# lh3/bfc

Hardware: AMD Instinct MI355X
Metric: M k-mers/s counted (bloom+htab) on 150 bp reads (higher is better)
Workload: dtype u64

## Files before the change

### bfc_amd/_lib.py

```python
import ctypes as C
import os

HERE = os.path.dirname(os.path.abspath(__file__))
SO = os.environ.get("BFC_GPU_LIB") or os.path.join(HERE, "libbfc_gpu.so")

u64p = C.POINTER(C.c_uint64)
u32p = C.POINTER(C.c_uint32)
f32p = C.POINTER(C.c_float)


class BfcOpt(C.Structure):
    _fields_ = [("chunk_size", C.c_int), ("n_threads", C.c_int), ("no_mt_io", C.c_int), ("q", C.c_int), ("k", C.c_int),
                ("filter_mode", C.c_int), ("refine_ec", C.c_int), ("no_qual", C.c_int), ("min_frac", C.c_float),
                ("l_pre", C.c_int), ("bf_shift", C.c_int), ("n_hashes", C.c_int), ("discard", C.c_int),
                ("max_end_ext", C.c_int), ("win_multi_ec", C.c_int), ("min_cov", C.c_int),
                ("w_ec", C.c_int), ("w_ec_high", C.c_int), ("w_absent", C.c_int), ("w_absent_high", C.c_int),
                ("max_path_diff", C.c_int), ("max_heap", C.c_int)]


class BfcBf(C.Structure):
    _fields_ = [("n_shift", C.c_int), ("n_hashes", C.c_int), ("b", C.POINTER(C.c_uint8))]


class BfcKmer(C.Structure):
# ... 5 lines not shown
                ("filter_mode", C.c_int), ("device", C.c_int), ("max_batch_pos", C.c_uint64),
                ("region_shift", C.c_int), ("tab_cshift", C.c_int), ("debug_seen", C.c_int), ("track_order", C.c_int), ("rank", C.c_int), ("n_ranks", C.c_int), ("table_layout", C.c_int)]


SYMBOLS = {
    "bfc_bf_init": (C.POINTER(BfcBf), [C.c_int, C.c_int]),
    "bfc_bf_destroy": (None, [C.POINTER(BfcBf)]),
    "bfc_bf_insert": (C.c_int, [C.POINTER(BfcBf), C.c_uint64]),
    "bfc_bf_get": (C.c_int, [C.POINTER(BfcBf), C.c_uint64]),
    "bfc_ch_init": (C.c_void_p, [C.c_int, C.c_int]),
    "bfc_ch_destroy": (None, [C.c_void_p]),
    "bfc_ch_insert": (C.c_int, [C.c_void_p, u64p, C.c_int, C.c_int]),
    "bfc_ch_get": (C.c_int, [C.c_void_p, u64p]),
    "bfc_ch_count": (C.c_uint64, [C.c_void_p]),
    "bfc_ch_hist": (C.c_int, [C.c_void_p, u64p, u64p]),
    "bfc_ch_dump": (C.c_int, [C.c_void_p, C.c_char_p]),
    "bfc_ch_restore": (C.c_void_p, [C.c_char_p]),
    "bfc_ch_get_k": (C.c_int, [C.c_void_p]),
    "bfc_ch_kmer_occ": (C.c_int, [C.c_void_p, C.POINTER(BfcKmer)]),
    "bfc_count": (C.c_void_p, [C.c_char_p, C.POINTER(BfcOpt)]),
    "bfc_correct": (None, [C.c_char_p, C.POINTER(BfcOpt), C.c_void_p]),
    "bfcg_params_default": (None, [C.POINTER(BfcgParams)]),
    "bfcg_create": (C.c_void_p, [C.POINTER(BfcgParams)]),
    "bfcg_destroy": (None, [C.c_void_p]),
    "bfcg_last_error": (C.c_char_p, []),
    "bfcg_build_id": (C.c_char_p, []),
    "bfcg_device_count": (C.c_int, []),
    "bfcg_reset": (C.c_int, [C.c_void_p]),
    "bfcg_count_batch_dev": (C.c_int, [C.c_void_p, C.c_void_p, C.c_void_p, C.c_uint64]),
    "bfcg_count_batch_host": (C.c_int, [C.c_void_p, C.c_void_p, C.c_void_p, C.c_uint64]),
    "bfcg_plane_words": (C.c_uint64, [C.c_uint64]),
    "bfcg_pack_planes": (None, [C.c_void_p, C.c_void_p, C.c_uint64, C.c_uint64, C.c_uint64, C.c_int, C.c_void_p, C.c_uint64]),
    "bfcg_count_batch_planes": (C.c_int, [C.c_void_p, C.c_void_p, C.c_uint64, C.c_uint64, C.c_uint64, C.c_int]),
    "bfcg_sync": (C.c_int, [C.c_void_p]),
    "bfcg_mg_info": (C.c_int, [C.c_void_p, C.POINTER(C.c_int)]),
    "bfcg_batch_limit": (C.c_uint64, [C.c_void_p]),
    "bfcg_mg_scatter": (C.c_int, [C.c_void_p, C.c_void_p, C.c_void_p, C.c_uint64, C.c_void_p, u32p]),
    "bfcg_mg_process": (C.c_int, [C.c_void_p, C.c_void_p, u32p]),
    "bfcg_mg_allow_onepass": (None, [C.c_void_p, C.c_int]),
    "bfcg_group_unique_id": (C.c_int, [C.c_void_p]),
    "bfcg_group_create": (C.c_void_p, [C.POINTER(BfcgParams), C.c_int, C.c_int, C.c_int, C.POINTER(C.c_int), C.c_void_p, C.c_int]),
    "bfcg_group_destroy": (None, [C.c_void_p]),
    "bfcg_group_info": (C.c_int, [C.c_void_p, C.POINTER(C.c_int)]),
    "bfcg_group_slab_mode": (C.c_int, [C.c_void_p]),
    "bfcg_group_lazy_batches": (C.c_uint64, [C.c_void_p]),
    "bfcg_group_exchange_bytes": (C.c_int, [C.c_void_p, u64p]),
    "bfcg_group_ctx": (C.c_void_p, [C.c_void_p, C.c_int]),
    "bfcg_group_reset": (C.c_int, [C.c_void_p]),
    "bfcg_group_count_batch_dev": (C.c_int, [C.c_void_p, C.POINTER(C.c_void_p), C.POINTER(C.c_void_p), u64p]),
    "bfcg_group_count_batch_host": (C.c_int, [C.c_void_p, C.c_void_p, C.c_void_p, C.c_uint64]),
    "bfcg_group_sync": (C.c_int, [C.c_void_p]),
    "bfcg_group_stats": (C.c_int, [C.c_void_p, u64p]),
    "bfcg_group_progress": (C.c_int, [C.c_void_p, u64p, u64p, u64p, C.c_int]),
    "bfcg_group_export_table": (C.c_void_p, [C.c_void_p]),
    "bfcg_group_export_bloom": (C.POINTER(BfcBf), [C.c_void_p, C.c_int]),
    "bfcg_group_export_bloom_resident": (C.POINTER(BfcBf), [C.c_void_p, C.c_int]),
    "bfcg_trim_create": (C.c_void_p, [C.c_int, C.POINTER(BfcBf), C.c_int, C.c_uint64, C.c_uint64]),
    "bfcg_trim_destroy": (None, [C.c_void_p]),
    "bfcg_trim_batch": (C.c_int, [C.c_void_p, C.c_void_p, C.c_void_p, C.c_uint64, u64p, C.c_uint64, C.c_float, C.POINTER(C.c_int32), C.POINTER(C.c_int32)]),
    "bfcg_trim_last_ms": (C.c_float, [C.c_void_p]),
    "bfcg_trim_adopted": (C.c_int, [C.c_void_p]),
    "bfcg_trim_dev_seq": (C.c_void_p, [C.c_void_p]),
    "bfcg_stream_batches": (C.c_uint64, [C.c_void_p]),
    "bfc_ch_union": (C.c_void_p, [C.POINTER(C.c_void_p), C.c_int]),
    "bfc_ingest_digest": (C.c_int, [C.c_char_p, C.c_uint64, C.c_uint64, C.c_int, u64p]),
    "bfc_ingest_planes_digest": (C.c_int, [C.c_char_p, C.c_uint64, C.c_uint64, C.c_int, C.c_int, C.c_int, u64p]),
    "bfc_pgz_digest": (C.c_int, [C.c_char_p, C.c_int, C.c_uint64, C.c_uint64, u64p]),
    "bfcg_kcov_create": (C.c_void_p, [C.c_void_p, C.c_int, C.c_uint64]),
    "bfcg_kcov_attach": (C.c_void_p, [C.c_void_p, C.c_uint64]),
    "bfcg_kcov_destroy": (None, [C.c_void_p]),
    "bfcg_kcov_batch": (C.c_int, [C.c_void_p, C.c_void_p, C.c_void_p, C.c_uint64, C.c_int, C.c_void_p]),
    "bfcg_kcov_last_ms": (C.c_float, [C.c_void_p]),
    "bfcg_kcov_dev_seq": (C.c_void_p, [C.c_void_p]),
    "bfcg_kcov_dev_out": (C.c_void_p, [C.c_void_p]),
    "bfcg_dev_alloc": (C.c_void_p, [C.c_void_p, C.c_uint64]),
    "bfcg_dev_free": (None, [C.c_void_p, C.c_void_p]),
    "bfcg_h2d": (C.c_int, [C.c_void_p, C.c_void_p, C.c_void_p, C.c_uint64]),
    "bfcg_d2h": (C.c_int, [C.c_void_p, C.c_void_p, C.c_void_p, C.c_uint64]),
    "bfcg_host_alloc": (C.c_void_p, [C.c_uint64]),
    "bfcg_host_free": (None, [C.c_void_p]),
    "bfcg_stats": (C.c_int, [C.c_void_p, u64p]),
    "bfcg_progress": (C.c_int, [C.c_void_p, u64p, u64p, u64p, C.c_int]),
    "bfcg_partition_info": (C.c_int, [C.c_void_p, u64p]),
    "bfcg_s1wc_launches": (C.c_uint64, []),
    "bfcg_table_info": (C.c_int, [C.c_void_p, C.POINTER(C.c_int)]),
    "bfcg_last_batch_ms": (C.c_int, [C.c_void_p, f32p]),
    "bfcg_stage_ms": (C.c_int, [C.c_void_p, C.POINTER(C.c_double), u64p, C.c_int]),
    "bfcg_bloom_to_host": (C.c_int, [C.c_void_p, C.c_int, C.c_void_p]),
    "bfcg_export_bloom": (C.POINTER(BfcBf), [C.c_void_p, C.c_int]),
    "bfcg_export_bloom_resident": (C.POINTER(BfcBf), [C.c_void_p, C.c_int]),
    "bfcg_resident_drop": (None, [C.c_void_p]),
    "bfcg_export_table": (C.c_void_p, [C.c_void_p]),
    "bfcg_export_table_resident": (C.c_void_p, [C.c_void_p]),
    "bfc_ch_get_lpre": (C.c_int, [C.c_void_p]),
    "bfc_ch_export_sorted": (C.c_uint64, [C.c_void_p, u32p, u64p]),
    "bfcg_ec_create": (C.c_void_p, [C.c_void_p, C.POINTER(BfcOpt), C.c_int, C.c_uint64, C.c_uint64]),
    "bfcg_ec_attach": (C.c_void_p, [C.c_void_p, C.POINTER(BfcOpt), C.c_uint64, C.c_uint64]),
    "bfcg_ec_batch": (C.c_int, [C.c_void_p, C.c_void_p, C.c_void_p, C.c_uint64, u64p, C.c_uint64, u32p, u32p]),
    "bfcg_ec_destroy": (None, [C.c_void_p]),
    "bfcg_ec_last_ms": (C.c_float, [C.c_void_p]),
    "bfcg_ec_host_reads": (C.c_uint64, [C.c_void_p]),
    "bfcg_ec_last_lookups": (C.c_uint64, [C.c_void_p]),
    "bfcg_ec_retry_reads": (C.c_uint64, [C.c_void_p]),
    "bfcg_ec_adopted": (C.c_int, [C.c_void_p]),
    "bfcg_ec1_host": (C.c_int, [C.c_void_p, C.POINTER(BfcOpt), C.c_int, C.c_void_p, C.c_void_p, u32p, u32p]),
    "bfcg_ec_batch_refine": (C.c_int, [C.c_void_p, C.c_void_p, C.c_void_p, C.c_uint64, u64p, C.c_uint64, u32p, u32p, u32p, u32p]),
    "bfcg_ec1_host_refine": (C.c_int, [C.c_void_p, C.POINTER(BfcOpt), C.c_int, C.c_void_p, C.c_void_p, C.c_uint32, C.c_uint32, u32p, u32p]),
    "bfcg_ec_parse_stats": (C.c_int, [C.c_char_p, u32p, u32p]),
    "bfcg_kmers_create": (C.c_void_p, [C.c_void_p, C.c_int]),
    "bfcg_kmers_attach": (C.c_void_p, [C.c_void_p]),
    "bfcg_kmers_destroy": (None, [C.c_void_p]),
    "bfcg_kmers_info": (C.c_int, [C.c_void_p, C.POINTER(C.c_int)]),
    "bfcg_kmers_hist": (C.c_int, [C.c_void_p, u64p, u64p]),
    "bfcg_kmers_sub_sizes": (C.c_int, [C.c_void_p, u32p]),
    "bfcg_kmers_hist_sizes": (C.c_int, [C.c_void_p, u64p, u64p, u32p]),
    "bfcg_kmers_list": (C.c_int, [C.c_void_p, C.c_int, C.c_int, C.c_uint32, C.c_uint32, C.c_void_p, C.c_void_p, C.c_uint64, u64p]),
    "bfcg_kmers_last_ms": (C.c_float, [C.c_void_p]),
    "bfcg_kmer_decode_host": (C.c_int, [C.c_int, C.c_int, C.c_uint32, C.c_uint64, u64p]),
    "bfcg_kmer_2str": (None, [C.c_int, u64p, C.c_char_p]),
    "bfcg_kmers_format": (C.c_uint64, [C.c_int, C.c_void_p, C.c_void_p, C.c_uint64, C.c_void_p]),
    "bfcg_kmers_format_sizes": (C.c_uint64, [C.c_void_p, C.c_uint64, C.c_void_p]),
    "bfcg_kmers_lookup": (C.c_int, [C.c_void_p, C.c_void_p, C.c_uint64, C.c_void_p, u64p]),
    "bfcg_kmers_profile": (C.c_int, [C.c_void_p, C.c_void_p, C.c_void_p, C.c_uint64, C.c_void_p]),
    "bfcg_kmer_from_str": (C.c_int, [C.c_int, C.c_char_p, u64p]),
    "bfcg_kmer_occ_host": (C.c_int, [C.c_void_p, u64p]),
    "bfcg_kmers_occ_host": (None, [C.c_void_p, C.c_void_p, C.c_uint64, C.c_void_p]),
    "bfcg_kmers_parse": (C.c_uint64, [C.c_int, C.c_char_p, C.c_uint64, C.c_void_p, C.c_uint64, u64p]),
    "bfcg_lookup_format": (C.c_uint64, [C.c_char_p, C.c_uint64, C.c_void_p, C.c_uint64, C.c_void_p]),
    "bfcg_profile_format": (C.c_uint64, [C.c_void_p, C.c_uint64, C.c_void_p]),
    "bfcg_kmers_read_stats": (C.c_int, [C.c_void_p, C.c_void_p, C.c_void_p, C.c_uint64, C.c_void_p, C.c_uint64, C.c_int, C.c_void_p]),
    "bfcg_read_stats_host": (C.c_int, [C.c_void_p, C.c_void_p, C.c_uint64, C.c_void_p, C.c_uint64, C.c_int, C.c_void_p]),
    "bfcg_read_stats_format": (C.c_uint64, [C.c_void_p, C.c_uint64, C.c_void_p]),
    "bfcg_kmers_joint_hist": (C.c_int, [C.c_void_p, C.c_void_p, u64p, u64p]),
    "bfcg_kmers_list_vs": (C.c_int, [C.c_void_p, C.c_void_p, C.c_int, C.c_int, C.c_int, C.c_int, C.c_uint32, C.c_uint32, C.c_void_p, C.c_void_p, C.c_void_p, C.c_uint64, u64p]),
    "bfcg_kmers_union": (C.c_void_p, [C.c_void_p, C.c_void_p]),
    "bfcg_kmers_export": (C.c_void_p, [C.c_void_p, u64p]),
    "bfcg_kmers_format_vs": (C.c_uint64, [C.c_int, C.c_void_p, C.c_void_p, C.c_void_p, C.c_uint64, C.c_void_p]),
    "bfcg_kmers_neighbors": (C.c_int, [C.c_void_p, C.c_void_p, C.c_uint64, C.c_void_p]),
    "bfcg_kmers_graph_census": (C.c_int, [C.c_void_p, C.c_int, u64p]),
    "bfcg_kmers_list_graph": (C.c_int, [C.c_void_p, C.c_int, C.c_uint32, C.c_uint32, C.c_uint32, C.c_void_p, C.c_void_p, C.c_void_p, C.c_uint64, u64p]),
    "bfcg_kmers_extend": (C.c_int, [C.c_void_p, C.c_void_p, C.c_uint64, C.c_int, C.c_int, C.c_void_p, C.c_void_p]),
    "bfcg_kmer_revcomp": (C.c_int, [C.c_int, u64p, u64p]),
    "bfcg_neighbors_host": (C.c_int, [C.c_void_p, C.c_void_p, C.c_uint64, C.c_void_p]),
    "bfcg_graph_census_host": (C.c_int, [C.c_void_p, C.c_int, u64p]),
    "bfcg_graph_nb_host": (C.c_int64, [C.c_void_p, C.c_int, C.c_void_p, C.c_void_p]),
    "bfcg_extend_host": (C.c_int, [C.c_void_p, C.c_void_p, C.c_uint64, C.c_int, C.c_int, C.c_void_p, C.c_void_p]),
    "bfcg_kmers_unitigs": (C.c_int, [C.c_void_p, C.c_int, C.c_void_p, C.c_uint64, C.c_void_p, C.c_void_p, C.c_void_p, C.c_void_p, C.c_uint64, u64p]),
    "bfcg_unitigs_host": (C.c_int, [C.c_void_p, C.c_int, C.c_void_p, C.c_uint64, C.c_void_p, C.c_void_p, C.c_void_p, C.c_void_p, C.c_uint64, u64p]),
    "bfcg_kmers_clip": (C.c_void_p, [C.c_void_p, C.c_int, C.c_int, C.c_int, C.c_int, C.c_int, C.c_void_p, C.POINTER(C.c_int)]),
    "bfcg_clip_host": (C.c_void_p, [C.c_void_p, C.c_int, C.c_int, C.c_int, C.c_int, C.c_int, C.c_void_p, C.POINTER(C.c_int)]),
    "bfcg_kmers_pop": (C.c_void_p, [C.c_void_p, C.c_int, C.c_int, C.c_int, C.c_int, C.c_int, C.c_void_p, C.POINTER(C.c_int)]),
    "bfcg_pop_host": (C.c_void_p, [C.c_void_p, C.c_int, C.c_int, C.c_int, C.c_int, C.c_int, C.c_void_p, C.POINTER(C.c_int)]),
    "bfcg_hash_positions": (C.c_int, [C.c_void_p, C.c_void_p, C.c_void_p, C.c_uint64, u64p]),
    "bfcg_seen_flags": (C.c_int, [C.c_void_p, C.c_void_p, C.c_uint64]),
}

HOST_SYMBOLS = {
    "bfc_ch_alloc_raw": (C.c_void_p, [C.c_int, C.c_int, C.c_int]),
    "bfc_ch_raw_slots": (u64p, [C.c_void_p]),
    "bfc_ch_raw_cshift": (C.c_int, [C.c_void_p]),
    "bfc_ch_raw_recount": (None, [C.c_void_p]),
}

_lib = None


# ... 25 lines not shown
```

### bfc_amd/api.py

```python
import ctypes as C
import math

import numpy as np

from . import _lib
from ._lib import BfcOpt, BfcgParams, BfcKmer, u64p, u32p, f32p

STAT_NAMES = {0: "n_kmers", 1: "n_high", 2: "n_seen", 3: "n_keys", 4: "tab_ovf", 5: "err_pool", 6: "slow_buckets", 7: "crowded_regions", 8: "tab_cshift", 9: "n_batches"}


class BfcGpuError(RuntimeError):
    pass


def bfc_opt_init():
    o = BfcOpt()
    o.chunk_size = 100000000
    o.n_threads = 1
    o.q = 20
    o.k = 33
    o.l_pre = 20
    o.bf_shift = 33
    o.n_hashes = 4
    o.min_frac = 0.9
# ... 354 lines not shown
        return self

    def _ck(self, rc):
        if rc != 0:
            raise BfcGpuError(self.L.bfcg_last_error().decode())

    def close(self):
        if self.ctx and not getattr(self, "_borrowed", False):
            self.L.bfcg_destroy(self.ctx)
        self.ctx = None

    def __del__(self):
        try:
            self.close()
        except Exception:
            pass

    def reset(self):
        self._ck(self.L.bfcg_reset(self.ctx))

    def count_host(self, seq_stream, qual_stream=None):
        seq_stream = np.ascontiguousarray(seq_stream, dtype=np.uint8)
        q = np.ascontiguousarray(qual_stream, dtype=np.uint8) if qual_stream is not None else None
        self._ck(self.L.bfcg_count_batch_host(self.ctx, seq_stream.ctypes.data, q.ctypes.data if q is not None else None, len(seq_stream)))

    def count_planes(self, planes, first_pos, n_pos, has_qual=True):
        planes = np.ascontiguousarray(planes, dtype=np.uint32)
        assert planes.ndim == 2 and planes.shape[0] == 4
        self._ck(self.L.bfcg_count_batch_planes(self.ctx, planes.ctypes.data, planes.shape[1], first_pos, n_pos, 1 if has_qual else 0))

    def count_dev(self, d_seq, d_qual, n_pos):
        self._ck(self.L.bfcg_count_batch_dev(self.ctx, d_seq, d_qual, n_pos))

    def mg_info(self):
        out = (C.c_int * 4)()
        self.L.bfcg_mg_info(self.ctx, out)
        return dict(nb1=out[0], nb_loc=out[1], rec_bytes=out[2], n_ranks=out[3])

    def batch_limit(self):
        return int(self.L.bfcg_batch_limit(self.ctx))

    def mg_scatter(self, d_seq, d_qual, n_pos, d_send):
        counts = np.zeros(self.mg_info()["nb1"], dtype=np.uint32)
        self._ck(self.L.bfcg_mg_scatter(self.ctx, d_seq, d_qual, n_pos, d_send, counts.ctypes.data_as(u32p)))
        return counts

    def mg_process(self, d_recv, seg_cnt):
        seg_cnt = np.ascontiguousarray(seg_cnt, dtype=np.uint32)
        self._ck(self.L.bfcg_mg_process(self.ctx, d_recv, seg_cnt.ctypes.data_as(u32p)))

    def dev_alloc(self, nbytes):
        p = self.L.bfcg_dev_alloc(self.ctx, nbytes)
        if not p:
            raise BfcGpuError(self.L.bfcg_last_error().decode())
        return p

    def dev_free(self, p):
        self.L.bfcg_dev_free(self.ctx, p)

    def h2d(self, dptr, arr):
        arr = np.ascontiguousarray(arr)
        self._ck(self.L.bfcg_h2d(self.ctx, dptr, arr.ctypes.data, arr.nbytes))

    def sync(self):
        self._ck(self.L.bfcg_sync(self.ctx))

    def stats(self):
        out = np.zeros(16, dtype=np.uint64)
        self._ck(self.L.bfcg_stats(self.ctx, out.ctypes.data_as(u64p)))
        d = {STAT_NAMES[i]: int(out[i]) for i in STAT_NAMES}
        d["stream_batches"] = int(self.L.bfcg_stream_batches(self.ctx))
        d["phase_cycles"] = [int(out[i]) for i in range(10, 16)]
        return d

    def table_info(self):
        out = (C.c_int * 4)()
        self.L.bfcg_table_info(self.ctx, out)
        return dict(segments=bool(out[0]), seg_shift=out[1], tab_cshift=out[2], seg_growths=out[3])

    def partition_info(self):
        out = (C.c_uint64 * 2)()
        self.L.bfcg_partition_info(self.ctx, out)
        return dict(one_pass=bool(out[0] & 1), level2_one_pass=bool(out[0] & 2), replayed_batches=int(out[1]))

    def s1wc_launches(self):
        return int(self.L.bfcg_s1wc_launches())

    def last_batch_ms(self):
        out = np.zeros(6, dtype=np.float32)
        self.L.bfcg_last_batch_ms(self.ctx, out.ctypes.data_as(f32p))
        return dict(hist1=float(out[0]), scatter1=float(out[1]), level2=float(out[2]), bloom=float(out[3]), commit=float(out[4]), total=float(out[5]))

    def stage_ms(self, reset=False):
        out = (C.c_double * 6)()
        n = C.c_uint64()
        self._ck(self.L.bfcg_stage_ms(self.ctx, out, C.byref(n), int(reset)))
        return dict(hist1=out[0], scatter1=out[1], level2=out[2], bloom=out[3], commit=out[4], total=out[5]), int(n.value)

    def bloom_bytes(self, which=0):
        out = np.empty((1 << (self.bf_shift - 3)) // self.n_ranks, dtype=np.uint8)
        self._ck(self.L.bfcg_bloom_to_host(self.ctx, which, out.ctypes.data))
        return out

    def export_bloom(self, which=0, resident=False):
        p = (self.L.bfcg_export_bloom_resident if resident else self.L.bfcg_export_bloom)(self.ctx, which)
        if not p:
            raise BfcGpuError(self.L.bfcg_last_error().decode())
        return HostBloom(p)

    def export_table(self):
        p = self.L.bfcg_export_table(self.ctx)
        if not p:
            raise BfcGpuError(self.L.bfcg_last_error().decode())
        return HostTable(p)

    def hash_positions(self, seq_stream, qual_stream=None):
        seq_stream = np.ascontiguousarray(seq_stream, dtype=np.uint8)
        q = np.ascontiguousarray(qual_stream, dtype=np.uint8) if qual_stream is not None else None
        out = np.zeros((len(seq_stream), 3), dtype=np.uint64)
        self._ck(self.L.bfcg_hash_positions(self.ctx, seq_stream.ctypes.data, q.ctypes.data if q is not None else None, len(seq_stream), out.ctypes.data_as(u64p)))
        return out

    def seen_flags(self, n_pos):
        out = np.zeros(n_pos, dtype=np.uint8)
        self._ck(self.L.bfcg_seen_flags(self.ctx, out.ctypes.data, n_pos))
        return out


class GpuGroup:

    def __init__(self, k, bf_shift, devices, max_batch_pos, n_ranks=None, first_rank=0, uid=None, transport=0, q=20, n_hashes=4, l_pre=20,
                 filter_mode=0, track_order=False, table_layout=0, region_shift=0, tab_cshift=0):
        self.L = _lib.load()
        p = BfcgParams()
        self.L.bfcg_params_default(C.byref(p))
        p.k, p.q, p.bf_shift, p.n_hashes, p.l_pre, p.filter_mode = k, q, bf_shift, n_hashes, l_pre, filter_mode
        p.max_batch_pos, p.region_shift, p.tab_cshift, p.track_order, p.table_layout = int(max_batch_pos), region_shift, tab_cshift, int(track_order), int(table_layout)
        self.params, self.k, self.bf_shift = p, k, bf_shift
        self.devices = list(devices)
        self.n_local = len(self.devices)
        self.n_ranks = n_ranks if n_ranks is not None else self.n_local
        dv = (C.c_int * self.n_local)(*self.devices)
        self._uid = (C.c_uint8 * 128).from_buffer_copy(bytes(uid)) if uid is not None else None
        self.g = self.L.bfcg_group_create(C.byref(p), self.n_ranks, first_rank, self.n_local, dv, self._uid, transport)
        if not self.g:
            raise BfcGpuError("bfcg_group_create failed: " + self.L.bfcg_last_error().decode())

    @staticmethod
    def unique_id():
        L = _lib.load()
        buf = (C.c_uint8 * 128)()
        if L.bfcg_group_unique_id(buf) != 0:
            raise BfcGpuError(L.bfcg_last_error().decode())
        return bytes(buf)

    def _ck(self, rc):
        if rc != 0:
            raise BfcGpuError(self.L.bfcg_last_error().decode())

    def close(self):
        if self.g:
            self.L.bfcg_group_destroy(self.g)
            self.g = None

    def __del__(self):
        try:
# ... 522 lines not shown
```

### bfc_amd/csrc/bfcg_bloom3.hip

```cpp
#include <hip/hip_runtime.h>
#include <stdint.h>
#include <stdlib.h>
#include "kmer_dev.h"
#include "bfcg_internal.h"
#include "bfcg_dev.h"

using namespace bfcg;

#define B3_UND 0x40000000u
#define B3_SEEN16 0x8000u
#define B3_COLD_NR 8
#define B3_WALK_U 4
template <int BT, int PF, bool COLD>
__global__ __launch_bounds__(BT, PF <= 2 ? 8 : 6) void k_bloom3(KParams P, BloomArgs A)
{
	extern __shared__ __attribute__((aligned(16))) unsigned char smem[];
	__shared__ uint32_t s_list_n, s_ovf, s_pool_off, s_emit_n, s_fs_used, s_wb_n, s_pad3[2];
	const uint32_t f = blockIdx.x;
	const bool ho_log = A.ho_stride != 0;
	if (batch_poisoned(A)) { if (ho_log && threadIdx.x == 0) A.ho_mark[f] = A.ho_cur[f]; return; }
	uint32_t rs, n;
	region_list(A, f, rs, n);
	if (n == 0) { if (threadIdx.x == 0) { if (ho_log) A.ho_mark[f] = A.ho_cur[f]; else if (A.agg_cnt) A.agg_cnt[f] = 0; } return; }
	uint32_t ho_cur0 = 0;
	unsigned long long *ho_base;
	if (ho_log) {
		ho_cur0 = A.ho_cur[f];
		if (ho_cur0 + n > A.ho_stride) {
			if (threadIdx.x == 0) { atomicAdd(&A.stats[(size_t)(f & (ST_SLOTS - 1)) * ST_N + ST_ERR_POOL], 1ULL); A.ho_mark[f] = ho_cur0; }
			return;
		}
		ho_base = A.ho + (uint64_t)f * A.ho_stride + ho_cur0;
	} else ho_base = reinterpret_cast<unsigned long long *>(A.stream_out) + rs;
	A.stats += (size_t)(f & (ST_SLOTS - 1)) * ST_N;
	const uint32_t region_dw = 16u << P.R;
	unsigned char *sp = smem;
	unsigned int *region = reinterpret_cast<unsigned int *>(sp); sp += (size_t)region_dw * 4;
	const uint32_t nblk = 1u << P.R;
	unsigned int *bcnt = reinterpret_cast<unsigned int *>(sp), *boff = bcnt + nblk;
	if (COLD) sp += (size_t)(2 * nblk + 4) * 4;
	unsigned int *fs = reinterpret_cast<unsigned int *>(sp); if (!COLD) sp += (size_t)P.fs_cap * 4;
	unsigned int *la = reinterpret_cast<unsigned int *>(sp); sp += (size_t)P.list_cap * 4;
	unsigned int *lb = reinterpret_cast<unsigned int *>(sp); sp += (size_t)P.list_cap * 4;
	unsigned short *lc = reinterpret_cast<unsigned short *>(sp); sp += (size_t)P.list_cap * 2;
	unsigned short *ord = reinterpret_cast<unsigned short *>(sp);
	const uint32_t fs_mask = P.fs_cap - 1;
	const uint32_t *recs = A.recs + (uint64_t)rs * 3;
	unsigned int *g_region = reinterpret_cast<unsigned int *>(A.bloom) + (uint64_t)f * region_dw;
	const uint32_t imp = (P.f_base + f) >> P.F2;
	const Dec3 D = dec3_geom(P);
	const int tid = threadIdx.x, lane = tid & 63;
	const uint32_t mask_a = (1u << D.a) - 1u, imp_sh = D.n ? imp << D.lo : 0u, sh_up = D.lo + D.n;
#ifdef BFCG_MEASURE
	const bool timing = BFCG_ABL(P, 64) && tid == 0;
	long long tq[7] = {0, 0, 0, 0, 0, 0, 0};
	long long tc[7] = {0, 0, 0, 0, 0, 0, 0};
	if (timing) tq[0] = clock64();
#define B3_TC(i) do { if (timing) tc[i] = clock64(); } while (0)
#else
#define B3_TC(i) do { } while (0)
#endif
	auto addr3 = [&](uint32_t d0, uint32_t d1) -> uint32_t {
		const uint32_t y0d = d0 & mask_a, upper = y0d >> D.up;
		const uint32_t y0lo = D.n ? (y0d & D.lowmask) | imp_sh | (upper << sh_up) : y0d;
		const uint32_t y1lo = __builtin_amdgcn_alignbit(d1, d0, D.a) & D.mk32;
		const uint32_t hh = upper | (((y0lo - y1lo) ^ y1lo) << D.sh_x);
		uint32_t h2 = (hh >> 9) & 511u;
		h2 |= (uint32_t)((h2 & 31u) == 0);
		return (y0d & D.rmask) | ((hh & 511u) << 8) | (h2 << 17);
	};
	auto entry3 = [&](uint32_t d0, uint32_t d1) -> unsigned long long {
		const unsigned long long AA = d0 | ((unsigned long long)d1 << 32);
		const unsigned long long y1 = (AA >> D.a) & ((1ULL << P.k) - 1);
		const uint32_t y0d = d0 & mask_a;
		const unsigned long long id = (unsigned long long)((y0d & D.rmask) | ((y0d >> D.up) << D.R)) | (y1 << D.sh_y1);
		return (id << 1) | (unsigned long long)((d1 >> D.sh_flag) & 1u);
	};
	RecW<3> cur[PF], nxt[PF];
#pragma unroll
	for (int u = 0; u < PF; ++u) {
		const uint32_t i = tid + u * BT;
		cur[u].d[0] = cur[u].d[1] = cur[u].d[2] = 0; nxt[u] = cur[u];
		if (i < n) cur[u] = rec_load<3>(recs + (uint64_t)i * 3);
		if (i + BT * PF < n) nxt[u] = rec_load<3>(recs + (uint64_t)(i + BT * PF) * 3);
	}
	{
		const uint4 *src = reinterpret_cast<const uint4 *>(g_region);
		uint4 *dst = reinterpret_cast<uint4 *>(region);
		for (uint32_t i = tid; i < region_dw / 4; i += BT) dst[i] = src[i];
		if constexpr (COLD) { for (uint32_t i = tid; i < 2 * nblk + 4; i += BT) bcnt[i] = 0; }
		else {
			uint4 *f4 = reinterpret_cast<uint4 *>(fs);
			for (uint32_t i = tid; i < P.fs_cap / 4; i += BT) f4[i] = make_uint4(FS32_EMPTY, FS32_EMPTY, FS32_EMPTY, FS32_EMPTY);
		}
		if (tid == 0) { s_list_n = 0; s_emit_n = 0; s_ovf = 0; s_fs_used = 0; s_wb_n = 0; }
	}
	__syncthreads();
#ifdef BFCG_MEASURE
	if (timing) tq[1] = clock64();
#endif
	volatile uint32_t *v_ovf = &s_ovf;

	for (uint32_t base = 0; base < n; base += BT * PF) {
		uint32_t pk[PF], um[PF];
#pragma unroll
		for (int u = 0; u < PF; ++u) {
			pk[u] = 0; um[u] = 0;
			if (base + u * BT + (uint32_t)(tid & ~63) < n) {
				pk[u] = addr3(cur[u].d[0], cur[u].d[1]);
				const B3Pos b = b3_positions((pk[u] >> 8) & 511u, pk[u] >> 17);
				const uint32_t bl64 = (pk[u] & 255u) << 6;
// ... 621 lines not shown
```

### bfc_amd/csrc/bfcg_ctx.hip

```cpp
#include <hip/hip_runtime.h>
#include <stdint.h>
#include <stdio.h>
#include <stdlib.h>
#include <string.h>
#include <stdarg.h>
#include <sys/mman.h>
#include <time.h>
#include <vector>
#include <thread>
#include "bfc_gpu.h"
#include "bfcg_internal.h"
#include "bfc_host.h"

using namespace bfcg;

static thread_local char g_err[512] = "";
enum { HO_MAX_PAGES = BFCG_HO_MAX_PAGES };
enum { OP_FLAG_WORDS = 12, OP_STICKY = 8 };
static double dbg_now(void) { struct timespec ts; clock_gettime(CLOCK_MONOTONIC, &ts); return ts.tv_sec + 1e-9 * ts.tv_nsec; }
static inline void set_seg_shift(KParams &P, int s, int blk_max) { P.seg_shift = s; P.seg_blk = s < blk_max ? s : blk_max; }
int bfcg::fail(const char *fmt, ...)
{
	va_list ap; va_start(ap, fmt); vsnprintf(g_err, sizeof(g_err), fmt, ap); va_end(ap);
	fprintf(stderr, "[E::bfcg] %s\n", g_err);
	return -1;
}

struct bfcg_ctx {
	bfcg_params_t prm;
	KParams P;
	BatchBufs B;
	hipStream_t st;
	hipStream_t stA;
	hipStream_t stC;
	hipEvent_t evt[2][7];
	hipEvent_t evA[2], evB[2], evCopy;
	uint32_t *rows1[2], *chunk1[2], *start1[2]; uint64_t *recs1[2];
	uint8_t *d_seq2[2], *d_qual2[2];
	uint32_t *d_planes[2];
	uint64_t plane_cap;
	int cur, pend;
	int used[2];
	uint8_t *d_seq, *d_qual;
	unsigned long long *h_stats;
	unsigned long long *h_snap[2];
	uint64_t call_no, slot_call[2];
	int call_depth;
	uint64_t final_call, call_keys[64];
	uint64_t n_batches;
	float last_ms[6];
	double sum_ms[6]; uint64_t n_timed;
	int rw;
	uint64_t bloom_bytes;
	int n_ranks, rank, log2n;
	uint32_t *d_seg, *h_seg;
	size_t seg_words;
	uint64_t recv_cap;
	uint64_t keys_last, grow[2];
	uint64_t crowded_last;
	int stream_mode;
	uint32_t *stream_out; uint64_t n_stream_batches;
	double seen_per_pos;
	int cold;
	uint64_t seen_last, pos_final, slot_pos[2];
	int pipeline;
	int seg_ok;
	int seg_total_max;
	int seg_blk_max;
	int b3_ok;
	uint32_t fs_cap_w, list_cap_w;
	uint32_t list_cap_cw;
	uint32_t list_cap_c;
	int seg_init_shift;
	int seg_escaped;
	uint64_t n_seg_grow;
	int onepass_ok, onepass;
	uint32_t *op_cursor[2], *op_seg[2], *op_flags, *h_flags[2];
	int unfinished, unfinished_mg;
	uint32_t *h_rows[2]; int rows_slot;
	uint32_t op_cap; uint64_t op_min_pos;
	uint32_t *cnt2; uint32_t cap2; uint64_t recs2_n;
	struct opq_t { const uint8_t *seq, *qual; uint64_t n_pos; int slot; const void *recv; int mg; } opq[4]; int n_opq;
	int mg_op2_ok, mg_op2, mg_op2_allowed; uint32_t *mg_seg[4];
	int mg_slab_ok; int mg_seg_slab[4];
	uint64_t n_replayed;
	int reused;
	int seg_no_grow;
	int seg_cap_shift;
	unsigned long long *ho, *ho_keys, *h_ho_keys[2]; uint32_t *ho_cur, *ho_mark; uint32_t ho_stride; int ho_K;
	int ho_pending;
	uint64_t ho_page_call[HO_MAX_PAGES];
	int slot_commit[2]; uint64_t slot_page_call[2][HO_MAX_PAGES];
	int slot_all_committed[2];
	uint64_t keys_known;
	int commit_absorbed;
	uint64_t keys_per_batch; int n_commits, ho_window;
	unsigned long long *seg_spare; int seg_spare_shift;
};

extern "C" const char *bfcg_last_error(void) { return g_err; }
extern "C" void bfcg_set_error(const char *msg) { fail("%s", msg); }

extern "C" int bfcg_device_count(void)
{
	int ndev = 0;
	if (hipGetDeviceCount(&ndev) != hipSuccess) { (void)hipGetLastError(); return 0; }
	return ndev;
}

extern "C" void bfcg_params_default(bfcg_params_t *p)
{
	memset(p, 0, sizeof(*p));
	p->k = 33; p->q = 20; p->bf_shift = 33; p->n_hashes = 4; p->l_pre = 20;
	p->max_batch_pos = 1ULL << 27;
}

static int clamp_lpre(int k, int l_pre)
{
	if (k * 2 - l_pre > BFC_CH_KEYBITS) l_pre = k * 2 - BFC_CH_KEYBITS;
	if (l_pre > BFC_CH_MAXPRE) l_pre = BFC_CH_MAXPRE;
	return l_pre;
}

extern "C" bfcg_ctx_t *bfcg_create(const bfcg_params_t *prm)
{
	int ndev = 0;
	const bool timing = getenv("BFC_GPU_TIMING") != 0;
	const double t_c0 = dbg_now();
	if (hipGetDeviceCount(&ndev) != hipSuccess || ndev == 0) { fail("no HIP device available: the counting path has no CPU fallback"); return NULL; }
	const double t_c1 = dbg_now();
	if (prm->device < 0 || prm->device >= ndev) { fail("device %d out of range (%d devices)", prm->device, ndev); return NULL; }
	if (prm->k < 1 || prm->k > 63) { fail("k=%d outside [1,63] (bfc.h:8, htab.c:23)", prm->k); return NULL; }
	if (prm->bf_shift < 9 + 0 || prm->bf_shift > 37) { fail("bf_shift=%d outside [9,37] (bbf.c:9, bfc.h:9)", prm->bf_shift); return NULL; }
	if (prm->n_hashes < 1 || prm->n_hashes > 12) { fail("n_hashes=%d outside [1,12]", prm->n_hashes); return NULL; }
	if (prm->max_batch_pos == 0 || prm->max_batch_pos >= (1ULL << 32)) { fail("max_batch_pos must be in [1, 2^32)"); return NULL; }
	const int n_ranks = prm->n_ranks > 0 ? prm->n_ranks : 1;
	int log2n = 0; while ((1 << log2n) < n_ranks) ++log2n;
	if ((1 << log2n) != n_ranks || n_ranks > 64 || prm->rank < 0 || prm->rank >= n_ranks) { fail("n_ranks=%d must be a power of two <= 64 and 0 <= rank=%d < n_ranks", n_ranks, prm->rank); return NULL; }
	if (n_ranks > 1 && prm->max_batch_pos >= (1ULL << (32 - log2n))) { fail("with %d ranks a batch holds < 2^%d positions", n_ranks, 32 - log2n); return NULL; }
	BFCG_CKN((void)0, hipSetDevice(prm->device));

	bfcg_ctx_t *c = (bfcg_ctx_t *)calloc(1, sizeof(bfcg_ctx_t));
	if (!c) { fail("out of host memory"); return NULL; }
	c->prm = *prm;
	KParams &P = c->P;
	P.k = prm->k; P.q = prm->q; P.bf_shift = prm->bf_shift; P.n_hashes = prm->n_hashes; P.filter_mode = prm->filter_mode;
	P.l_pre = clamp_lpre(prm->k, prm->l_pre);
	if (!prm->filter_mode && 2 * prm->k < P.l_pre) {
		fail("k=%d is too small for l_pre=%d: the count table needs 2k >= l_pre (htab.c:45-58)", prm->k, P.l_pre); bfcg_destroy(c); return NULL;
	}
	{
		const char *e;
		P.R = prm->region_shift > 0 ? prm->region_shift : ((e = getenv("BFCG_R")) ? atoi(e) : 8);
		if (P.R > 10) P.R = 10;
		if (P.R < 4) P.R = 4;
		if (P.R > P.bf_shift - 9) P.R = P.bf_shift - 9;
		while (P.bf_shift - 9 - P.R > 20 && P.R < 10) ++P.R;
		P.F = P.bf_shift - 9 - P.R;
		if (P.F <= 8) { P.F1 = P.F; P.F2 = 0; }
		else { P.F2 = (P.F + 1) / 2; if (P.F2 > 10) P.F2 = 10; P.F1 = P.F - P.F2; }
		if (P.F2 > 0 && (e = getenv("BFCG_F1"))) {
			const int f1 = atoi(e);
			if (f1 >= 1 && f1 <= 10 && P.F - f1 >= 1 && P.F - f1 <= 10 && f1 >= log2n) { P.F1 = f1; P.F2 = P.F - f1; }
		}
		if (P.F1 > 10) { fail("bf_shift=%d needs more than two scatter levels at region_shift=%d", P.bf_shift, P.R); bfcg_destroy(c); return NULL; }
		if (n_ranks > 1 && P.F2 == 0) {
			if (P.F <= log2n) { fail("bf_shift=%d gives %d bloom regions: too few for %d ranks", P.bf_shift, 1 << P.F, n_ranks); bfcg_destroy(c); return NULL; }
			P.F1 = (P.F + 1) / 2 > log2n ? (P.F + 1) / 2 : log2n; P.F2 = P.F - P.F1;
		}
#ifdef BFCG_MEASURE
		P.ablate = (e = getenv("BFCG_ABLATE")) ? atoi(e) : 0;
#else
		P.ablate = 0;
		if ((e = getenv("BFCG_ABLATE")) && atoi(e)) fprintf(stderr, "[W::bfcg] BFCG_ABLATE=%s ignored: this library was built without -DBFCG_MEASURE\n", e);
#endif
// ... 87 lines not shown
	c->recv_cap = n_ranks > 1 ? B.max_kmers + B.max_kmers / 4 + (1u << 20) : B.max_kmers;
	BFCG_CKN(bfcg_destroy(c), hipStreamCreate(&c->st)); BFCG_CKN(bfcg_destroy(c), hipStreamCreate(&c->stA)); BFCG_CKN(bfcg_destroy(c), hipStreamCreate(&c->stC));
	for (int b = 0; b < 2; ++b) {
		for (int i = 0; i < 7; ++i) BFCG_CKN(bfcg_destroy(c), hipEventCreate(&c->evt[b][i]));
		BFCG_CKN(bfcg_destroy(c), hipEventCreateWithFlags(&c->evA[b], hipEventDisableTiming)); BFCG_CKN(bfcg_destroy(c), hipEventCreateWithFlags(&c->evB[b], hipEventDisableTiming));
	}
	BFCG_CKN(bfcg_destroy(c), hipEventCreateWithFlags(&c->evCopy, hipEventDisableTiming));
	{
		const uint64_t tile = (uint64_t)bfcg_tile_of_rw(c->rw / 4), tile1 = (uint64_t)bfcg_tile1_of_rw(c->rw / 4);
		const uint64_t tiles1 = (prm->max_batch_pos + tile1 - 1) / tile1, chunks1 = (tiles1 + BFCG_SCAN_CH - 1) / BFCG_SCAN_CH;
		const uint64_t rows2 = (c->recv_cap + c->recv_cap / 8) / tile + (uint64_t)nb1 * 16 + 8;
		for (int b = 0; b < 2; ++b) {
			BFCG_CKN(bfcg_destroy(c), hipMalloc(&c->rows1[b], sizeof(uint32_t) * tiles1 * nb1));
			BFCG_CKN(bfcg_destroy(c), hipMalloc(&c->chunk1[b], sizeof(uint32_t) * chunks1 * nb1));
			BFCG_CKN(bfcg_destroy(c), hipMalloc(&c->start1[b], sizeof(uint32_t) * (nb1 + 1) * 2));
		}
		B.rows1 = c->rows1[0]; B.chunk1 = c->chunk1[0]; B.start1 = c->start1[0]; B.row_base = B.start1 + nb1 + 1;
		if (P.F2 > 0) {
			BFCG_CKN(bfcg_destroy(c), hipMalloc(&B.rows2, sizeof(uint32_t) * rows2 * (1u << P.F2)));
			BFCG_CKN(bfcg_destroy(c), hipMalloc(&B.start2, sizeof(uint32_t) * (nfine + 1)));
		}
	}
	{
		const char *e = getenv("BFCG_ONEPASS");
		c->onepass_ok = n_ranks == 1 && P.F2 > 0 && !(e && atoi(e) == 0);
		uint64_t cap = (B.max_kmers + B.max_kmers / 8) / ((uint64_t)nb1 * 8) + 1;
		while (cap * nb1 * 8 > 0xffffffffULL) --cap;
		if (cap >= 1024) cap &= ~31ULL;
		else if (cap >= 8) cap &= ~3ULL;
		c->op_cap = (uint32_t)cap;
		c->op_min_pos = (e = getenv("BFCG_ONEPASS_MIN_TILES")) ? (uint64_t)atoi(e) * 4096 : (uint64_t)nb1 * 8 * 1024;
	}
	const uint64_t recs1_n = c->onepass_ok ? (uint64_t)c->op_cap * nb1 * 8 + (uint64_t)bfcg_tile1_of_rw(c->rw / 4) + 64 : B.max_kmers;
	BFCG_CKN(bfcg_destroy(c), hipMalloc(&c->recs1[0], recs1_n * c->rw));
	if (n_ranks == 1 && !c->pipeline) c->recs1[1] = c->recs1[0];
	else BFCG_CKN(bfcg_destroy(c), hipMalloc(&c->recs1[1], recs1_n * c->rw));
	{
		const char *e = getenv("BFCG_ONEPASS");
		c->mg_op2_ok = P.F2 > 0 && !(e && atoi(e) == 0);
	}
	{ const char *e = getenv("BFCG_MG_SLABS"); c->mg_slab_ok = P.F2 > 0 && !(e && atoi(e) == 0); }
	if (c->onepass_ok || c->mg_slab_ok) {
		for (int b = 0; b < 2; ++b) {
			BFCG_CKN(bfcg_destroy(c), hipMalloc(&c->op_cursor[b], sizeof(uint32_t) * (8 * nb1 * 32 + 32)));
			BFCG_CKN(bfcg_destroy(c), hipMalloc(&c->op_seg[b], sizeof(uint32_t) * ((size_t)25 * nb1 + 8)));
		}
	}
	if (c->mg_slab_ok) for (int b = 0; b < 2; ++b) BFCG_CKN(bfcg_destroy(c), hipHostMalloc(&c->h_rows[b], sizeof(uint32_t) * ((size_t)8 * nb1 + 2 * (size_t)n_ranks)));
	if (c->onepass_ok || c->mg_op2_ok || c->mg_slab_ok) {
		for (int b = 0; b < 2; ++b) BFCG_CKN(bfcg_destroy(c), hipHostMalloc(&c->h_flags[b], 4 * sizeof(uint32_t)));
		BFCG_CKN(bfcg_destroy(c), hipMalloc(&c->op_flags, OP_FLAG_WORDS * sizeof(uint32_t)));
		BFCG_CKN(bfcg_destroy(c), hipMemset(c->op_flags, 0, OP_FLAG_WORDS * sizeof(uint32_t)));
	}
	if (c->mg_op2_ok) for (int i = 0; i < 4; ++i) c->mg_seg[i] = (uint32_t *)malloc(sizeof(uint32_t) * (size_t)n_ranks * (size_t)(nb1 >> log2n) * 8);
	B.recs1 = c->recs1[0];
	c->recs2_n = c->recv_cap;
	if (c->onepass_ok || c->mg_op2_ok || c->mg_slab_ok) {
		const char *e = getenv("BFCG_ONEPASS2");
		const uint64_t cap2 = (B.max_kmers + B.max_kmers / 8) / (uint64_t)nfine + 64, n2 = cap2 * (uint64_t)nfine + 8192;
		if (!(e && atoi(e) == 0) && n2 < 0xffffffffULL) {
			c->cap2 = (uint32_t)cap2; c->recs2_n = n2 > c->recv_cap ? n2 : c->recv_cap;
			BFCG_CKN(bfcg_destroy(c), hipMalloc(&c->cnt2, sizeof(uint32_t) * (size_t)nfine));
		} else { c->mg_op2_ok = 0; BFCG_CKN(bfcg_destroy(c), hipMalloc(&c->cnt2, sizeof(uint32_t) * (size_t)nfine)); }
		B.cnt_live = c->cnt2;
	}
	if (P.F2 > 0) BFCG_CKN(bfcg_destroy(c), hipMalloc(&B.recs2, c->recs2_n * c->rw));
	c->seg_words = (size_t)25 * nb1 + 8;
	{ BFCG_CKN(bfcg_destroy(c), hipMalloc(&c->d_seg, sizeof(uint32_t) * 2 * c->seg_words)); BFCG_CKN(bfcg_destroy(c), hipHostMalloc(&c->h_seg, sizeof(uint32_t) * 2 * c->seg_words)); }
	BFCG_CKN(bfcg_destroy(c), hipMalloc(&B.bloom, c->bloom_bytes));
	P.f_base = (uint32_t)c->rank * (uint32_t)nfine;
	if (c->seg_ok) {
		int sh = prm->tab_cshift > 0 ? prm->tab_cshift + 3 : 6;
		if (prm->tab_cshift <= 0) while (((uint64_t)nfine << sh) < prm->max_batch_pos / 4 && sh < BFCG_SEG_MAX_SHIFT) ++sh;
		if (sh > BFCG_SEG_MAX_SHIFT) sh = BFCG_SEG_MAX_SHIFT;
		c->seg_init_shift = sh;
		{ const char *e = getenv("BFCG_SEG_BLOCK"); c->seg_blk_max = e && atoi(e) >= 3 && atoi(e) <= BFCG_SEG_MAX_SHIFT ? atoi(e) : 12; }
		{ const char *e = getenv("BFCG_SEG_TOTAL"); c->seg_total_max = e && atoi(e) >= c->seg_blk_max && atoi(e) <= BFCG_SEG_TOTAL_MAX ? atoi(e) : BFCG_SEG_TOTAL_MAX; }
		if (c->seg_total_max > c->seg_blk_max + 15) c->seg_total_max = c->seg_blk_max + 15;
		P.seg = 1; set_seg_shift(P, sh, c->seg_blk_max); c->seg_cap_shift = sh;
		BFCG_CKN(bfcg_destroy(c), set_seg_lds_attr());
		BFCG_CKN(bfcg_destroy(c), hipMalloc(&B.seg_tab, ((uint64_t)nfine << sh) * 8));
		{
			const char *e = getenv("BFCG_COMMIT_K");
			int K = e ? atoi(e) : 4;
			if (K < 1) K = 1;
			if (K > HO_MAX_PAGES) K = HO_MAX_PAGES;
			if (!c->cap2) K = 1;
			size_t free_b = 0, total_b = 0;
			const uint64_t page = (uint64_t)nfine * (c->cap2 ? c->cap2 : 1) * 8;
			if (hipMemGetInfo(&free_b, &total_b) == hipSuccess) while (K > 1 && page * (uint64_t)K > (uint64_t)free_b / 3) --K;
			c->ho_K = K;
			c->ho_stride = c->cap2 ? (uint32_t)K * c->cap2 : 0u;
			uint64_t entries = (uint64_t)nfine * c->ho_stride;
			if (entries < c->recs2_n) entries = c->recs2_n;
			BFCG_CKN(bfcg_destroy(c), hipMalloc(&c->ho, (entries + 4096) * 8));
			BFCG_CKN(bfcg_destroy(c), hipMalloc(&c->ho_cur, sizeof(uint32_t) * (size_t)nfine));
			BFCG_CKN(bfcg_destroy(c), hipMalloc(&c->ho_mark, sizeof(uint32_t) * (size_t)nfine * HO_MAX_PAGES));
			BFCG_CKN(bfcg_destroy(c), hipMalloc(&c->ho_keys, sizeof(unsigned long long) * ST_SLOTS * HO_MAX_PAGES));
			for (int b = 0; b < 2; ++b) BFCG_CKN(bfcg_destroy(c), hipHostMalloc(&c->h_ho_keys[b], sizeof(unsigned long long) * ST_SLOTS * HO_MAX_PAGES));
		}
	}
	if (P.filter_mode) BFCG_CKN(bfcg_destroy(c), hipMalloc(&B.bloom_hi, c->bloom_bytes));
	else if (!c->seg_ok) BFCG_CKN(bfcg_destroy(c), hipMalloc(&B.table, 8ULL << (P.l_pre + P.tab_cshift)));
	if (P.track) { BFCG_CKN(bfcg_destroy(c), hipMalloc(&B.tab_first, 8ULL << (P.l_pre + P.tab_cshift))); BFCG_CKN(bfcg_destroy(c), hipMalloc(&B.sub_last, 8ULL << P.l_pre)); }
	BFCG_CKN(bfcg_destroy(c), hipMalloc(&B.stats, sizeof(unsigned long long) * ST_N * (ST_SLOTS + 1)));
	{ uint64_t cap = prm->max_batch_pos / 2; if (cap < (1u << 20)) cap = 1u << 20; if (cap > (1u << 28)) cap = 1u << 28; B.tab_ovf_cap = (uint32_t)cap; }
	BFCG_CKN(bfcg_destroy(c), hipMalloc(&B.tab_ovf, (uint64_t)B.tab_ovf_cap * 40));
	B.pool_slices = 256;
	{
		const uint64_t pool_words = (uint64_t)B.pool_slices + (uint64_t)B.pool_slices * ((uint64_t)1024 << P.R);
		BFCG_CKN(bfcg_destroy(c), hipMalloc(&B.pool, pool_words * 8));
		BFCG_CKN(bfcg_destroy(c), hipMemset(B.pool, 0, (size_t)B.pool_slices * 8));
	}
	if (prm->debug_seen) BFCG_CKN(bfcg_destroy(c), hipMalloc(&B.seen_out, prm->max_batch_pos));
	if (!P.filter_mode) {
		if (!c->seg_ok) BFCG_CKN(bfcg_destroy(c), hipMalloc(&B.agg_out, (uint64_t)nfine * P.ag_cap * (P.track ? 32 : 24)));
		BFCG_CKN(bfcg_destroy(c), hipMalloc(&B.agg_cnt, sizeof(uint32_t) * nfine));
	}
	for (int b = 0; b < 2; ++b) { BFCG_CKN(bfcg_destroy(c), hipMalloc(&c->d_seq2[b], prm->max_batch_pos)); BFCG_CKN(bfcg_destroy(c), hipMalloc(&c->d_qual2[b], prm->max_batch_pos + 64)); }
	c->d_seq = c->d_seq2[0]; c->d_qual = c->d_qual2[0];
	BFCG_CKN(bfcg_destroy(c), hipHostMalloc(&c->h_stats, sizeof(unsigned long long) * ST_N * (ST_SLOTS + 2)));
	for (int b = 0; b < 2; ++b) BFCG_CKN(bfcg_destroy(c), hipHostMalloc(&c->h_snap[b], sizeof(unsigned long long) * ST_N * (ST_SLOTS + 1)));
	const double t_c2 = dbg_now();
	BFCG_CKN(bfcg_destroy(c), set_bloom_lds_attr(P));
	BFCG_CKN(bfcg_destroy(c), set_scatter1wc_lds_attr());
	const double t_c3 = dbg_now();
	if (bfcg_reset(c) != 0) { bfcg_destroy(c); return NULL; }
	if (timing) fprintf(stderr, "[T::bfcg_create] HIP runtime up %.3f s, device buffers %.3f s, kernel attributes %.3f s, filter and table cleared %.3f s\n", t_c1 - t_c0, t_c2 - t_c1, t_c3 - t_c2, dbg_now() - t_c3);
	return c;
}

extern "C" void bfcg_destroy(bfcg_ctx_t *c)
{
	if (!c) return;
	(void)hipSetDevice(c->prm.device);
	(void)hipDeviceSynchronize();
	for (int b = 0; b < 2; ++b) { (void)hipFree(c->rows1[b]); (void)hipFree(c->chunk1[b]); (void)hipFree(c->start1[b]); if (b == 0 || c->recs1[1] != c->recs1[0]) (void)hipFree(c->recs1[b]); (void)hipFree(c->d_seq2[b]); (void)hipFree(c->d_qual2[b]); (void)hipFree(c->d_planes[b]); }
	(void)hipFree(c->B.rows2); (void)hipFree(c->B.start2); (void)hipFree(c->B.recs2);
	(void)hipFree(c->B.bloom); (void)hipFree(c->B.bloom_hi); (void)hipFree(c->B.table); (void)hipFree(c->B.stats); (void)hipFree(c->B.tab_first); (void)hipFree(c->B.sub_last);
	(void)hipFree(c->stream_out); (void)hipFree(c->B.seg_tab); (void)hipFree(c->seg_spare);
	(void)hipFree(c->ho); (void)hipFree(c->ho_cur); (void)hipFree(c->ho_mark); (void)hipFree(c->ho_keys);
	for (int b = 0; b < 2; ++b) if (c->h_ho_keys[b]) (void)hipHostFree(c->h_ho_keys[b]);
	for (int b = 0; b < 2; ++b) { (void)hipFree(c->op_cursor[b]); (void)hipFree(c->op_seg[b]); if (c->h_flags[b]) (void)hipHostFree(c->h_flags[b]); if (c->h_rows[b]) (void)hipHostFree(c->h_rows[b]); }
	(void)hipFree(c->op_flags); (void)hipFree(c->cnt2); for (int i = 0; i < 4; ++i) free(c->mg_seg[i]);
	(void)hipFree(c->B.tab_ovf); (void)hipFree(c->B.pool); (void)hipFree(c->B.seen_out); (void)hipFree(c->B.agg_out); (void)hipFree(c->B.agg_cnt);
	for (void *h : {(void *)c->h_stats, (void *)c->h_snap[0], (void *)c->h_snap[1]}) if (h) (void)hipHostFree(h); (void)hipFree(c->d_seg); if (c->h_seg) (void)hipHostFree(c->h_seg);
	for (int b = 0; b < 2; ++b) for (hipEvent_t e : {c->evt[b][0], c->evt[b][1], c->evt[b][2], c->evt[b][3], c->evt[b][4], c->evt[b][5], c->evt[b][6], c->evA[b], c->evB[b]}) if (e) (void)hipEventDestroy(e);
	if (c->evCopy) (void)hipEventDestroy(c->evCopy);
	for (hipStream_t st : {c->st, c->stA, c->stC}) if (st) (void)hipStreamDestroy(st);
	free(c);
}

static inline uint64_t nfine(const bfcg_ctx_t *c) { return ((uint64_t)1 << c->P.F) >> c->log2n; }
static int batch_fits(const bfcg_ctx_t *c, uint64_t n_pos)
{
	if (n_pos > c->prm.max_batch_pos) return fail("batch of %llu positions exceeds max_batch_pos=%llu", (unsigned long long)n_pos, (unsigned long long)c->prm.max_batch_pos);
	return 0;
}

static int drain(bfcg_ctx_t *c);
static int replay_poisoned(bfcg_ctx_t *c);
static int enqueue_batch(bfcg_ctx_t *c, const uint8_t *d_seq, const uint8_t *d_qual, uint64_t n_pos, int wait_copy, int no_kstats);
static int ensure_agg(bfcg_ctx_t *c);
static int same_block_offset(bfcg_ctx_t *c, int b, const uint8_t *d_seq, const uint8_t **d_qual, uint64_t n_pos, hipStream_t s);
static int commit_pending_pages(bfcg_ctx_t *c, int b);
static void absorb_pages(bfcg_ctx_t *c, int b);
static int handover_begin(bfcg_ctx_t *c, BatchBufs &Bt, int b, int slabs, uint64_t call);
static int handover_end(bfcg_ctx_t *c, const BatchBufs &Bt, int b);

static void warm_tables(const bfcg_ctx_t *c, KParams &Pt)
{
	Pt.b3_warm = 0; Pt.b3_cold = 0;
	if (Pt.b3 && c->cold && c->list_cap_c) { Pt.list_cap = c->list_cap_c; Pt.b3_cold = 1; Pt.dedupe = 0; }
	else if (Pt.b3 && !Pt.dedupe && !c->cold && c->list_cap_cw && c->list_cap_cw >= c->list_cap_w) { Pt.list_cap = c->list_cap_cw; Pt.b3_warm = 1; Pt.b3_cold = 1; }
	else if (Pt.b3 && !Pt.dedupe && !c->cold && c->list_cap_w) { Pt.fs_cap = c->fs_cap_w; Pt.list_cap = c->list_cap_w; Pt.b3_warm = 1; }
}
static int dedupe_hint(const bfcg_ctx_t *c) { return (c->n_batches == 0 || (c->cold && c->seen_per_pos < 0.15)) && !getenv("BFCG_NO_DEDUPE"); }

extern "C" int bfcg_reset(bfcg_ctx_t *c)
{
	const double t_dbg = dbg_now();
	struct dbg_guard { double t; ~dbg_guard() { if (getenv("BFCG_DEBUG")) fprintf(stderr, "[D::reset] %.3f ms\n", (dbg_now() - t) * 1e3); } } dg{t_dbg};
	BFCG_CK(hipSetDevice(c->prm.device));
	if (c->pend && drain(c) != 0) return -1;
	BFCG_CK(hipMemsetAsync(c->B.stats, 0, sizeof(unsigned long long) * ST_N * (ST_SLOTS + 1), c->st));
	if (c->op_flags) BFCG_CK(hipMemsetAsync(c->op_flags, 0, OP_FLAG_WORDS * sizeof(uint32_t), c->st));
	BFCG_CK(hipEventRecord(c->evCopy, c->st));
	BFCG_CK(hipStreamWaitEvent(c->stA, c->evCopy, 0));
	BFCG_CK(hipMemsetAsync(c->B.bloom, 0, c->bloom_bytes, c->st));
	if (c->B.bloom_hi) BFCG_CK(hipMemsetAsync(c->B.bloom_hi, 0, c->bloom_bytes, c->st));
	if (c->seg_ok) {
		const uint64_t nf = nfine(c);
		if (c->seg_escaped || !c->B.seg_tab) {
			BFCG_CK(hipStreamSynchronize(c->st));
			if (c->B.table) { BFCG_CK(hipFree(c->B.table)); c->B.table = 0; }
			if (c->B.seg_tab) { BFCG_CK(hipFree(c->B.seg_tab)); c->B.seg_tab = 0; }
			set_seg_shift(c->P, c->seg_init_shift, c->seg_blk_max); c->seg_cap_shift = c->seg_init_shift;
			BFCG_CK(hipMalloc(&c->B.seg_tab, (nf << c->P.seg_shift) * 8));
		} else {
			set_seg_shift(c->P, c->seg_init_shift, c->seg_blk_max);
			if (c->n_batches && c->seg_spare && c->seg_spare_shift < c->seg_cap_shift && ((nf << c->seg_cap_shift) * 8) <= (16ULL << 30)) {
				BFCG_CK(hipStreamSynchronize(c->st));
				BFCG_CK(hipFree(c->seg_spare)); c->seg_spare = 0;
				if (hipMalloc(&c->seg_spare, (nf << c->seg_cap_shift) * 8) != hipSuccess) { (void)hipGetLastError(); c->seg_spare = 0; }
				c->seg_spare_shift = c->seg_cap_shift;
			}
		}
		if (c->n_batches) c->reused = 1;
		c->P.seg = 1; c->P.b3 = c->b3_ok; c->seg_escaped = 0;
		BFCG_CK(hipMemsetAsync(c->ho_cur, 0, sizeof(uint32_t) * (size_t)nf, c->st));
		c->ho_pending = 0; c->slot_commit[0] = c->slot_commit[1] = 0; c->slot_all_committed[0] = c->slot_all_committed[1] = 0; c->keys_known = 0; c->commit_absorbed = 0;
		c->keys_per_batch = 0; c->n_commits = 0; c->ho_window = 1;
		BFCG_CK(hipMemsetAsync(c->B.seg_tab, 0, (nf << c->P.seg_shift) * 8, c->st));
	}
	if (c->B.table) BFCG_CK(hipMemsetAsync(c->B.table, 0, 8ULL << (c->P.l_pre + c->P.tab_cshift), c->st));
	if (c->B.tab_first) { BFCG_CK(hipMemsetAsync(c->B.tab_first, 0xff, 8ULL << (c->P.l_pre + c->P.tab_cshift), c->st)); BFCG_CK(hipMemsetAsync(c->B.sub_last, 0, 8ULL << c->P.l_pre, c->st)); }
	c->n_batches = 0;
	c->keys_last = 0; c->grow[0] = c->grow[1] = 0;
	c->crowded_last = 0; c->stream_mode = c->P.seg ? 1 : 0;
	c->cold = 1; c->seen_last = c->pos_final = 0; c->seg_no_grow = 0;
	c->onepass = c->onepass_ok; c->mg_op2 = c->mg_op2_ok; c->n_opq = 0;
	c->call_no = c->final_call = 0; c->call_depth = 0; memset(c->call_keys, 0, sizeof(c->call_keys));
	return 0;
}

static void fold_slots(bfcg_ctx_t *c, const unsigned long long *raw)
{
	for (int i = 0; i < ST_N; ++i) {
		unsigned long long s = 0;
		for (int j = 0; j < ST_SLOTS; ++j) s += raw[(size_t)j * ST_N + i];
		c->h_stats[i] = s;
	}
	c->h_stats[ST_TAB_OVF] = raw[(size_t)ST_SLOTS * ST_N];
}
static int fetch_stats(bfcg_ctx_t *c)
{
	unsigned long long *raw = c->h_stats + ST_N;
	BFCG_CK(hipMemcpyAsync(raw, c->B.stats, sizeof(unsigned long long) * ST_N * (ST_SLOTS + 1), hipMemcpyDeviceToHost, c->st));
	BFCG_CK(hipStreamSynchronize(c->st));
	fold_slots(c, raw);
	return 0;
}
static void fold_snapshot(bfcg_ctx_t *c, int b)
{
	fold_slots(c, c->h_snap[b]);
	absorb_pages(c, b);
	if (c->slot_all_committed[b]) {
		c->final_call = c->slot_call[b]; c->call_keys[c->slot_call[b] & 63] = c->h_stats[ST_KEYS];
		if (c->h_stats[ST_KEYS] > c->keys_known && c->h_stats[ST_KEYS] - c->keys_known > c->keys_per_batch) c->keys_per_batch = c->h_stats[ST_KEYS] - c->keys_known;
		c->keys_known = c->h_stats[ST_KEYS]; c->commit_absorbed = 1;
	}
	c->pos_final += c->slot_pos[b]; c->slot_pos[b] = 0;
}

static int table_maintain(bfcg_ctx_t *c);
static int seg_maintain(bfcg_ctx_t *c);
static int seg_target_shift(const bfcg_ctx_t *c);
static int seg_to_legacy(bfcg_ctx_t *c, int for_export = 0);
static void note_growth(bfcg_ctx_t *c);
static int finalise_previous(bfcg_ctx_t *c, int b);
static int table_target_cshift(const bfcg_ctx_t *c);
static int use_stream(bfcg_ctx_t *c);

static int batch_times(bfcg_ctx_t *c, int b)
{
	for (int i = 0; i < 3; ++i) BFCG_CK(hipEventSynchronize(c->evt[b][i]));
	for (int i = 0; i < 5; ++i) BFCG_CK(hipEventElapsedTime(&c->last_ms[i], c->evt[b][i == 2 ? 6 : i], c->evt[b][i + 1]));
	c->last_ms[5] = c->last_ms[0] + c->last_ms[1] + c->last_ms[2] + c->last_ms[3] + c->last_ms[4];
	for (int i = 0; i < 6; ++i) c->sum_ms[i] += c->last_ms[i];
	++c->n_timed;
	return 0;
}
static int check_health(bfcg_ctx_t *c)
{
	if (c->h_stats[ST_ERR_POOL]) return fail("first-setter pool exhausted in %llu bloom regions: batch too large for max_batch_pos", (unsigned long long)c->h_stats[ST_ERR_POOL]);
	if (c->P.seg) return seg_maintain(c);
	if (c->B.table) return table_maintain(c);
	return 0;
}
static int drain(bfcg_ctx_t *c)
{
	if (!c->pend) return 0;
	BFCG_CK(hipStreamSynchronize(c->stA));
	BFCG_CK(hipStreamSynchronize(c->st));
	BFCG_CK(hipGetLastError());
	c->pend = 0;
	if (batch_times(c, c->cur ^ 1) != 0) return -1;
	absorb_pages(c, c->cur); absorb_pages(c, c->cur ^ 1);
	if (c->n_opq) {
		uint32_t sticky = 0;
		BFCG_CK(hipMemcpy(&sticky, c->op_flags + OP_STICKY, sizeof(sticky), hipMemcpyDeviceToHost));
		if (sticky) return replay_poisoned(c);
		c->n_opq = 0;
	}
	if (c->P.seg && c->ho_pending) {
		if (commit_pending_pages(c, 0) != 0) return -1;
		BFCG_CK(hipStreamSynchronize(c->st));
		BFCG_CK(hipGetLastError());
		absorb_pages(c, 0);
	}
	if (fetch_stats(c) != 0) return -1;
	c->keys_known = c->h_stats[ST_KEYS]; c->commit_absorbed = 1;
	c->final_call = c->call_no; c->call_keys[c->call_no & 63] = c->h_stats[ST_KEYS];
	c->pos_final += c->slot_pos[0] + c->slot_pos[1]; c->slot_pos[0] = c->slot_pos[1] = 0;
	note_growth(c);
	return check_health(c);
}

extern "C" int bfcg_sync(bfcg_ctx_t *c) { return drain(c); }

static int replay_poisoned(bfcg_ctx_t *c)
{
	const int n = c->n_opq;
	bfcg_ctx::opq_t q[4];
	for (int i = 0; i < n; ++i) q[i] = c->opq[i];
	c->n_opq = 0; c->onepass = 0; c->mg_op2 = 0;
	if (getenv("BFCG_DEBUG")) {
		uint32_t fl[OP_FLAG_WORDS];
		BFCG_CK(hipMemcpy(fl, c->op_flags, sizeof(fl), hipMemcpyDeviceToHost));
		fprintf(stderr, "[D::replay] %d batches; flags (level-1 slab, -, region slab, -) of slot 0: %u %u %u %u, slot 1: %u %u %u %u, sticky %u\n", n, fl[0], fl[1], fl[2], fl[3], fl[4], fl[5], fl[6], fl[7], fl[OP_STICKY]);
	}
	BFCG_CK(hipMemset(c->op_flags, 0, OP_FLAG_WORDS * sizeof(uint32_t)));
	if (fetch_stats(c) != 0) return -1;
	c->n_batches -= (uint64_t)n;
	std::vector<uint32_t> seg;
	for (int i = 0; i < n; ++i) if (q[i].mg) --c->call_no;
	for (int i = 0; i < n; ++i) {
		if (q[i].mg) {
			const int slab = c->mg_seg_slab[q[i].mg - 1];
			const size_t w = (size_t)c->n_ranks * (size_t)((1 << c->P.F1) >> c->log2n) * (slab ? 8 : 1);
			seg.assign(c->mg_seg[q[i].mg - 1], c->mg_seg[q[i].mg - 1] + w);
			if (mg_process(c, q[i].recv, seg.data(), slab ? c->op_cap : 0u, 0, 0) != 0) return -1;
		} else if (enqueue_batch(c, q[i].seq, q[i].qual, q[i].n_pos, 0, 1) != 0) return -1;
		if (drain(c) != 0) return -1;
		++c->n_replayed;
	}
	return 0;
}

static uint64_t growth_forecast(const bfcg_ctx_t *c) { return c->grow[0] < c->grow[1] ? c->grow[0] : c->grow[1]; }
static void note_growth(bfcg_ctx_t *c)
{
	const uint64_t keys = c->h_stats[ST_KEYS];
	{
		const uint64_t ds = c->h_stats[ST_SEEN] - c->seen_last, np = c->pos_final;
		if (np) { c->cold = ds * 5 < np * 2; c->seen_per_pos = (double)ds / (double)np; }
		c->seen_last = c->h_stats[ST_SEEN]; c->pos_final = 0;
	}
	if (!c->P.seg || c->commit_absorbed) {
		c->grow[1] = c->grow[0]; c->grow[0] = keys > c->keys_last ? keys - c->keys_last : 0; c->keys_last = keys;
		c->commit_absorbed = 0;
	}
	const uint64_t crowded = c->h_stats[ST_CROWDED];
	if (!c->stream_mode && c->B.table && !c->P.track && c->P.n_hashes == 4 && c->P.bloom_bt == 512 && !getenv("BFCG_NO_STREAM") && (crowded - c->crowded_last) * 2 > nfine(c)) c->stream_mode = 1;
	c->crowded_last = crowded;
}
static int table_target_cshift(const bfcg_ctx_t *c)
{
	const KParams &P = c->P;
	const uint64_t need = c->h_stats[ST_KEYS] + c->h_stats[ST_TAB_OVF], g = growth_forecast(c);
	int t = P.tab_cshift;
	if ((need + g) * 2 > (1ULL << (P.l_pre + t)))
		while ((need + 2 * g) * 2 > (1ULL << (P.l_pre + t)) && P.l_pre + t < 36) ++t;
	if (c->h_stats[ST_TAB_OVF] && t == P.tab_cshift) ++t;
	if (t > P.tab_cshift) {
		size_t free_b = 0, total_b = 0;
		if (hipMemGetInfo(&free_b, &total_b) == hipSuccess) {
			const uint64_t margin = 2ULL << 30;
			while (t > P.tab_cshift && (8ULL << (P.l_pre + t)) + margin > (uint64_t)free_b) --t;
			if (t == P.tab_cshift && !c->h_stats[ST_TAB_OVF] && need * 5 <= (4ULL << (P.l_pre + t))) return t;
			if (t == P.tab_cshift) return t + 1;
		}
	}
	return t;
}

static int table_maintain(bfcg_ctx_t *c)
{
	KParams &P = c->P; BatchBufs &B = c->B;
	for (;;) {
		const uint64_t ovf = c->h_stats[ST_TAB_OVF];
		const int target = table_target_cshift(c);
		if (ovf == 0 && target == P.tab_cshift) return 0;
		if (ovf > B.tab_ovf_cap) return fail("count table overflow list exhausted (%llu parked k-mers)", (unsigned long long)ovf);
		if (P.l_pre + target > 36) return fail("count table cannot grow beyond 2^36 slots");
		{
			size_t free_b = 0, total_b = 0;
			if (hipMemGetInfo(&free_b, &total_b) == hipSuccess && (8ULL << (P.l_pre + target)) + (1ULL << 30) > (uint64_t)free_b)
				return fail("count table of %llu keys cannot grow to 2^%d slots: %.1f GiB of device memory free", (unsigned long long)c->h_stats[ST_KEYS], P.l_pre + target, free_b / 1073741824.0);
		}
		int old_cshift = P.tab_cshift;
		unsigned long long *nt = 0;
		P.tab_cshift = target;
		unsigned long long *nf = 0;
		BFCG_CK(hipMalloc(&nt, 8ULL << (P.l_pre + P.tab_cshift)));
		BFCG_CK(hipMemsetAsync(nt, 0, 8ULL << (P.l_pre + P.tab_cshift), c->st));
		if (B.tab_first) { BFCG_CK(hipMalloc(&nf, 8ULL << (P.l_pre + P.tab_cshift))); BFCG_CK(hipMemsetAsync(nf, 0xff, 8ULL << (P.l_pre + P.tab_cshift), c->st)); }
		run_table_rehash(P, B.table, old_cshift, nt, B.tab_first, nf, c->st);
		BFCG_CK(hipStreamSynchronize(c->st));
		BFCG_CK(hipFree(B.table));
		B.table = nt;
		if (B.tab_first) { BFCG_CK(hipFree(B.tab_first)); B.tab_first = nf; }
		if (ovf) {
			uint64_t *tmp = 0;
			BFCG_CK(hipMalloc(&tmp, ovf * 40));
			BFCG_CK(hipMemcpyAsync(tmp, B.tab_ovf, ovf * 40, hipMemcpyDeviceToDevice, c->st));
			BFCG_CK(hipMemsetAsync(&B.stats[(size_t)ST_SLOTS * ST_N], 0, 8, c->st));
			run_table_replay(P, B.table, tmp, ovf, B.stats, B.tab_ovf, B.tab_ovf_cap, B.tab_first, B.sub_last, c->st);
			if (fetch_stats(c) != 0) return -1;
			BFCG_CK(hipFree(tmp));
		} else c->h_stats[ST_TAB_OVF] = 0;
	}
}


static int seg_target_shift(const bfcg_ctx_t *c)
{
	const KParams &P = c->P;
	const uint64_t nf = nfine(c);
	const uint64_t need = c->h_stats[ST_KEYS] + c->h_stats[ST_TAB_OVF], g = c->ho_K > 1 ? c->keys_per_batch : c->grow[0] > c->grow[1] ? c->grow[0] : c->grow[1];
	int t = P.seg_shift;
	const double full = c->seg_no_grow ? 0.85 : 0.62;
	while ((double)(need + (c->seg_no_grow ? 0 : g)) > full * (double)(nf << t)) ++t;
	if (c->h_stats[ST_TAB_OVF] && t == P.seg_shift) ++t;
	if (t != P.seg_shift && getenv("BFCG_DEBUG")) fprintf(stderr, "[D::seg_target] shift %d -> %d: keys %llu parked %llu forecast %llu slots %llu\n", P.seg_shift, t,
		(unsigned long long)c->h_stats[ST_KEYS], (unsigned long long)c->h_stats[ST_TAB_OVF], (unsigned long long)g, (unsigned long long)(nf << P.seg_shift));
	return t;
}

static int seg_maintain(bfcg_ctx_t *c)
{
	KParams &P = c->P; BatchBufs &B = c->B;
	const uint64_t nf = nfine(c);
	const double t_dbg = dbg_now();
	struct dbg_guard { double t; int s0; const int *s1; ~dbg_guard() { if (getenv("BFCG_DEBUG") && *s1 != s0) fprintf(stderr, "[D::seg_maintain] shift %d -> %d: %.3f ms\n", s0, *s1, (dbg_now() - t) * 1e3); } } dg{t_dbg, P.seg_shift, &P.seg_shift};
	for (;;) {
		const uint64_t ovf = c->h_stats[ST_TAB_OVF];
		const int target = seg_target_shift(c);
		if (ovf == 0 && target == P.seg_shift) return 0;
		if (ovf > B.tab_ovf_cap) return fail("count table overflow list exhausted (%llu parked k-mers)", (unsigned long long)ovf);
		{
			size_t free_b = 0, total_b = 0;
			const bool no_room = hipMemGetInfo(&free_b, &total_b) == hipSuccess && ((nf << target) * 8) + (1ULL << 30) > (uint64_t)free_b + (c->seg_spare && c->seg_spare_shift >= target ? (nf << c->seg_spare_shift) * 8 : 0);
			if (no_room || target > c->seg_total_max) {
				if (ovf == 0 && (double)c->h_stats[ST_KEYS] < 0.85 * (double)(nf << P.seg_shift)) { c->seg_no_grow = 1; return 0; }
				if (target > c->seg_total_max) return seg_to_legacy(c);
				if (seg_to_legacy(c) == 0) return 0;
				return fail("count table of %llu keys cannot grow to 2^%d slots per region: %.1f GiB of device memory free", (unsigned long long)c->h_stats[ST_KEYS], target, free_b / 1073741824.0);
			}
		}
		const int old_shift = P.seg_shift, old_blk = P.seg_blk;
		unsigned long long *nt = 0;
		int nt_shift = target;
		set_seg_shift(P, target, c->seg_blk_max);
		if (c->seg_spare && c->seg_spare_shift >= target) { nt = c->seg_spare; nt_shift = c->seg_spare_shift; c->seg_spare = 0; }
		else {
			if (c->seg_spare) { BFCG_CK(hipFree(c->seg_spare)); c->seg_spare = 0; }
			BFCG_CK(hipMalloc(&nt, (nf << target) * 8));
		}
		run_seg_rehash(P, B.seg_tab, old_shift, old_blk, nt, (uint32_t)nf, c->st);
		BFCG_CK(hipStreamSynchronize(c->st));
		BFCG_CK(hipGetLastError());
		if (((nf << nt_shift) * 8) <= (16ULL << 30)) {
			if (c->seg_cap_shift < nt_shift && c->reused) { BFCG_CK(hipFree(B.seg_tab)); c->seg_spare = 0; if (hipMalloc(&c->seg_spare, (nf << nt_shift) * 8) != hipSuccess) { (void)hipGetLastError(); c->seg_spare = 0; } c->seg_spare_shift = nt_shift; }
			else { c->seg_spare = B.seg_tab; c->seg_spare_shift = c->seg_cap_shift; }
		} else BFCG_CK(hipFree(B.seg_tab));
		B.seg_tab = nt; c->seg_cap_shift = nt_shift;
		++c->n_seg_grow;
		if (ovf) {
			uint64_t *tmp = 0;
			BFCG_CK(hipMalloc(&tmp, ovf * 40));
			BFCG_CK(hipMemcpyAsync(tmp, B.tab_ovf, ovf * 40, hipMemcpyDeviceToDevice, c->st));
			BFCG_CK(hipMemsetAsync(&B.stats[(size_t)ST_SLOTS * ST_N], 0, 8, c->st));
			run_seg_replay(P, B.seg_tab, tmp, ovf, B.stats, B.tab_ovf, B.tab_ovf_cap, c->st);
			if (fetch_stats(c) != 0) return -1;
			BFCG_CK(hipFree(tmp));
		} else c->h_stats[ST_TAB_OVF] = 0;
	}
}

static int seg_to_legacy(bfcg_ctx_t *c, int for_export)
{
	KParams &P = c->P; BatchBufs &B = c->B;
	const uint64_t nf = nfine(c);
	const uint64_t keys = c->h_stats[ST_KEYS];
	if (c->seg_spare) { BFCG_CK(hipFree(c->seg_spare)); c->seg_spare = 0; }
	if (!for_export && !P.filter_mode && !B.agg_out) BFCG_CK(hipMalloc(&B.agg_out, nf * P.ag_cap * (P.track ? 32 : 24)));
	int cs = c->prm.tab_cshift > 0 ? c->prm.tab_cshift : 2;
	const uint64_t want = for_export ? keys + keys * 3 / 4 : 2 * keys + (c->prm.max_batch_pos / 4);
	while ((1ULL << (P.l_pre + cs)) < want && P.l_pre + cs < 36) ++cs;
	{
		size_t free_b = 0, total_b = 0;
		if (hipMemGetInfo(&free_b, &total_b) == hipSuccess)
			while (cs > 1 && (8ULL << (P.l_pre + cs)) + (2ULL << 30) > (uint64_t)free_b) --cs;
	}
	P.tab_cshift = cs;
	BFCG_CK(hipMalloc(&B.table, 8ULL << (P.l_pre + cs)));
	BFCG_CK(hipMemsetAsync(B.table, 0, 8ULL << (P.l_pre + cs), c->st));
	BFCG_CK(hipMemset2DAsync(B.stats + ST_KEYS, sizeof(unsigned long long) * ST_N, 0, sizeof(unsigned long long), ST_SLOTS, c->st));
	run_seg_to_table(P, B.seg_tab, (uint32_t)nf, B.table, B.stats, B.tab_ovf, B.tab_ovf_cap, c->st);
	BFCG_CK(hipStreamSynchronize(c->st));
	BFCG_CK(hipGetLastError());
	BFCG_CK(hipFree(B.seg_tab));
	B.seg_tab = 0;
	P.seg = 0; P.b3 = 0; c->seg_escaped = 1;
	BFCG_CK(set_bloom_lds_attr(P));
	if (fetch_stats(c) != 0) return -1;
	c->keys_last = c->h_stats[ST_KEYS];
	if (for_export && c->h_stats[ST_TAB_OVF] == 0) return 0;
	return table_maintain(c);
}

extern "C" int bfcg_partition_info(bfcg_ctx_t *c, uint64_t out[2]) { out[0] = (uint64_t)((c->onepass ? 1 : 0) | ((c->onepass || (c->mg_op2 && c->mg_op2_allowed)) && c->cap2 ? 2 : 0)); out[1] = c->n_replayed; return 0; }
extern "C" void bfcg_mg_allow_onepass(bfcg_ctx_t *c, int on) { c->mg_op2_allowed = on != 0; }

extern "C" int bfcg_table_info(bfcg_ctx_t *c, int out[4])
{
	out[0] = c->P.seg; out[1] = c->P.seg ? c->P.seg_shift : 0; out[2] = c->P.seg ? 0 : c->P.tab_cshift; out[3] = (int)c->n_seg_grow;
	return 0;
}


static KParams batch_params(const bfcg_ctx_t *c, int no_kstats, int onepass1)
{
	KParams Pt = c->P;
	Pt.no_kstats = no_kstats;
	Pt.dedupe = dedupe_hint(c);
	warm_tables(c, Pt);
	if (onepass1) {
		const char *e = getenv("BFCG_L2_BIG");
		const int want = e ? atoi(e) : 0;
		Pt.l2_big = c->cap2 && want > 0 && Pt.F2 >= (want == 1 ? 9 : 10) && scatter2_big_ok(Pt);
	}
	return Pt;
}

static int batch_bufs(bfcg_ctx_t *c, BatchBufs &Bt)
{
	if (ensure_agg(c) != 0 || use_stream(c) != 0) return -1;
	Bt = c->B;
	Bt.batch_hi = (unsigned long long)(c->n_batches + 1) << 32;
	Bt.stream = c->stream_mode; Bt.stream_out = c->stream_out;
	return 0;
}

struct StageB {
	const uint64_t *in1; const uint32_t *seg_beg, *seg_end; int n_seg, segs_per_bucket; const uint32_t *row_base, *bucket_start; uint64_t rec_bound;
	int slabs;
	int queued;
	uint64_t call, pos;
	const uint8_t *seq, *qual;
	const void *recv; const uint32_t *sizes; int sizes_slab;
	int finalise;
};

static int opq_push(bfcg_ctx_t *c, int b, const StageB &w)
{
	if (c->n_opq == 4) return fail("internal: one-pass queue overflow");
	int mg = 0;
	if (w.recv) {
		const size_t words = (size_t)c->n_ranks * (size_t)((1 << c->P.F1) >> c->log2n) * (w.sizes_slab ? 8 : 1);
		for (;; ++mg) { int used = 0; for (int i = 0; i < c->n_opq; ++i) used |= c->opq[i].mg == mg + 1; if (!used) break; }
		if (w.sizes) memcpy(c->mg_seg[mg], w.sizes, sizeof(uint32_t) * words); else memset(c->mg_seg[mg], 0, sizeof(uint32_t) * words);
		c->mg_seg_slab[mg++] = w.sizes_slab;
	}
	c->opq[c->n_opq++] = bfcg_ctx::opq_t{w.seq, w.qual, w.pos, b, w.recv, mg};
	return 0;
}

static int enqueue_stage_b(bfcg_ctx_t *c, int b, BatchBufs &Bt, const KParams &Pt, const StageB &w)
{
	if (handover_begin(c, Bt, b, w.slabs, w.call) != 0) return -1;
	run_stage_b(Pt, Bt, w.in1, w.seg_beg, w.seg_end, w.n_seg, w.segs_per_bucket, w.row_base, w.bucket_start, w.rec_bound, c->st, c->evt[b]);
	if (handover_end(c, Bt, b) != 0) return -1;
	if (w.queued) {
		BFCG_CK(hipMemcpyAsync(c->h_flags[b] + 1, c->op_flags + OP_STICKY, sizeof(uint32_t), hipMemcpyDeviceToHost, c->st));
		if (opq_push(c, b, w) != 0) return -1;
	}
	BFCG_CK(hipMemcpyAsync(c->h_snap[b], c->B.stats, sizeof(unsigned long long) * ST_N * (ST_SLOTS + 1), hipMemcpyDeviceToHost, c->st));
	c->slot_call[b] = c->call_no = w.call; c->slot_pos[b] = w.pos;
	BFCG_CK(hipEventRecord(c->evB[b], c->st));
	BFCG_CK(hipGetLastError());
	c->used[b] = 1;
	++c->n_batches;
	return w.finalise ? finalise_previous(c, b) : 0;
}

static int mg_stage_b(bfcg_ctx_t *c, int b, const void *d_recv, const uint32_t *d, int n_seg, int spb, uint64_t rec_bound, const uint32_t *sizes, int sizes_slab, int finalise)
{
	BatchBufs Bt;
	if (batch_bufs(c, Bt) != 0) return -1;
	const int op2_run = c->mg_op2 && c->mg_op2_allowed && c->cap2;
	const int op2 = op2_run && rec_bound >= 8 * nfine(c);
	if (op2_run) Bt.op_sticky = c->op_flags + OP_STICKY;
	if (op2) {
		Bt.cnt2 = c->cnt2; Bt.cap2 = c->cap2; Bt.op_flags = c->op_flags + 4 * b;
		BFCG_CK(hipMemsetAsync(Bt.op_flags, 0, 4 * sizeof(uint32_t), c->st));
	}
	const StageB w = {(const uint64_t *)d_recv, d, d + n_seg, n_seg, spb, d + 2 * n_seg, d + 3 * n_seg + 1, rec_bound, op2, op2_run, c->call_no + 1, rec_bound, nullptr, nullptr, d_recv, sizes, sizes_slab, finalise};
	return enqueue_stage_b(c, b, Bt, batch_params(c, 0, 0), w);
}


extern "C" int bfcg_mg_info(bfcg_ctx_t *c, int out[4])
{
	out[0] = 1 << c->P.F1; out[1] = (1 << c->P.F1) >> c->log2n; out[2] = c->rw; out[3] = c->n_ranks;
	return 0;
}

static int mg_scatter2(bfcg_ctx_t *c, const uint8_t *d_seq, const uint8_t *d_qual, uint64_t n_pos, void *d_send, uint32_t *counts, int no_kstats);
extern "C" int bfcg_mg_scatter(bfcg_ctx_t *c, const uint8_t *d_seq, const uint8_t *d_qual, uint64_t n_pos, void *d_send, uint32_t *counts) { return mg_scatter2(c, d_seq, d_qual, n_pos, d_send, counts, 0); }
int bfcg::mg_scatter_again(bfcg_ctx_t *c, const uint8_t *d_seq, const uint8_t *d_qual, uint64_t n_pos, void *d_send, uint32_t *counts) { return mg_scatter2(c, d_seq, d_qual, n_pos, d_send, counts, 1); }
static inline hipStream_t mg_stage_a_stream(bfcg_ctx_t *c) { return c->n_ranks == 1 && !c->pipeline ? c->st : c->stA; }
static int mg_stage_a_begin(bfcg_ctx_t *c, int b, hipStream_t sA, const uint8_t *d_seq, const uint8_t **d_qual, uint64_t n_pos)
{
	if (batch_fits(c, n_pos) != 0) return -1;
	BFCG_CK(hipSetDevice(c->prm.device));
	if (n_pos == 0) {
		for (int i = 0; i < 3; ++i) BFCG_CK(hipEventRecord(c->evt[b][i], sA));
		return 1;
	}
	return same_block_offset(c, b, d_seq, d_qual, n_pos, sA);
}
static BatchBufs mg_slab_bufs(const bfcg_ctx_t *c, int b, uint32_t own_delta)
{
	const uint32_t nb_loc = (1u << c->P.F1) >> c->log2n;
	BatchBufs Bt = c->B;
	Bt.op_cursor = c->op_cursor[b]; Bt.op_seg = c->op_seg[b]; Bt.op_flags = c->op_flags + 4 * b; Bt.op_cap = c->op_cap; Bt.cap2 = c->cap2;
	Bt.op_own_lo = (uint32_t)c->rank * nb_loc; Bt.op_own_n = nb_loc; Bt.op_own_delta = own_delta;
	return Bt;
}
static int mg_scatter2(bfcg_ctx_t *c, const uint8_t *d_seq, const uint8_t *d_qual, uint64_t n_pos, void *d_send, uint32_t *counts, int no_kstats)
{
	const int nb1 = 1 << c->P.F1, b = c->cur;
	const hipStream_t sA = mg_stage_a_stream(c);
	const int begun = mg_stage_a_begin(c, b, sA, d_seq, &d_qual, n_pos);
	if (begun == 1) memset(counts, 0, sizeof(uint32_t) * nb1);
	if (begun) return begun < 0 ? -1 : 0;
	BatchBufs Bt = c->B;
	Bt.rows1 = c->rows1[b]; Bt.chunk1 = c->chunk1[b]; Bt.start1 = c->start1[b]; Bt.row_base = Bt.start1 + nb1 + 1;
	KParams Pa = c->P;
	Pa.no_kstats = no_kstats;
	run_stage_a(Pa, Bt, d_seq, d_qual, (int64_t)n_pos, (uint64_t *)d_send, sA, c->evt[b]);
	BFCG_CK(hipGetLastError());
	uint32_t *tmp = (uint32_t *)malloc(sizeof(uint32_t) * (nb1 + 1));
	hipError_t e = hipMemcpyAsync(tmp, Bt.start1, sizeof(uint32_t) * (nb1 + 1), hipMemcpyDeviceToHost, sA);
	if (e == hipSuccess) e = hipStreamSynchronize(sA);
	if (e != hipSuccess) { free(tmp); return fail("reading the level-1 bucket starts failed: %s", hipGetErrorString(e)); }
	for (int i = 0; i < nb1; ++i) counts[i] = tmp[i + 1] - tmp[i];
	free(tmp);
	return 0;
}

int bfcg::mg_slab_info(bfcg_ctx_t *c, uint32_t out[2]) { out[0] = c->op_cap; out[1] = (uint32_t)(c->mg_slab_ok && c->op_cursor[0] != 0); return 0; }
int bfcg::mg_scatter_slabs(bfcg_ctx_t *c, const uint8_t *d_seq, const uint8_t *d_qual, uint64_t n_pos, void *d_send, uint32_t own_delta, uint32_t *fills, int *overflow)
{
	const int nb1 = 1 << c->P.F1, b = c->cur;
// ... 68 lines not shown
					const uint64_t at = ((uint64_t)((size_t)s * nb_loc + k) * 8 + x) * slab_cap;
					const uint32_t fill = seg_cnt[((size_t)s * nb_loc + k) * 8 + x];
					if (fill > slab_cap || at + fill > 0xffffffffULL) return fail("slab of %u records holds %u", slab_cap, fill);
					seg_beg[seg] = (uint32_t)at; seg_end[seg] = (uint32_t)at + fill; off += fill;
				}
	} else
	for (int s = 0; s < N; ++s)
		for (int k = 0; k < nb_loc; ++k) {
			int seg = k * N + s;
			seg_beg[seg] = (uint32_t)off; off += seg_cnt[s * nb_loc + k]; seg_end[seg] = (uint32_t)off;
		}
	if (off > c->recv_cap) return fail("received %llu records for this rank's buckets, capacity %llu", (unsigned long long)off, (unsigned long long)c->recv_cap);
	const uint32_t tile2 = (uint32_t)bfcg_tile_of_rw(c->rw / 4);
	for (int seg = 0; seg < n_seg; ++seg) { row_base[seg] = (uint32_t)rows; rows += (seg_end[seg] - seg_beg[seg] + tile2 - 1) / tile2; }
	row_base[n_seg] = (uint32_t)rows;
	for (int k = 0; k < nb_loc; ++k) {
		bucket_start[k] = (uint32_t)tot;
		for (int s = 0; s < spb; ++s) tot += seg_end[k * spb + s] - seg_beg[k * spb + s];
	}
	bucket_start[nb_loc] = (uint32_t)tot;
	uint32_t *d = c->d_seg + (size_t)b * c->seg_words;
	for (int i = 0; i < n_wait; ++i) BFCG_CK(hipStreamWaitEvent(c->st, wait[i], 0));
	BFCG_CK(hipEventRecord(c->evt[b][6], c->st));
	BFCG_CK(hipMemcpyAsync(d, seg_beg, sizeof(uint32_t) * words, hipMemcpyHostToDevice, c->st));
	if (c->B.seen_out) BFCG_CK(hipMemsetAsync(c->B.seen_out, 0, c->prm.max_batch_pos, c->st));
	return mg_stage_b(c, b, d_recv, d, n_seg, spb, off, seg_cnt, slab_cap != 0, 1);
}

int bfcg::mg_async_ok(bfcg_ctx_t *c) { return c->mg_slab_ok && !c->B.seen_out && !c->P.track && c->h_rows[0] != 0 && (c->n_ranks == 1 || (uint64_t)8 * (1u << c->P.F1) * c->op_cap <= c->recv_cap); }
int bfcg::mg_process_slabs_dev(bfcg_ctx_t *c, const void *d_recv, const uint32_t *d_rows_in, uint32_t slab_cap, uint64_t rec_bound, int s_lo, int s_hi, hipEvent_t *wait, int n_wait)
{
	const int N = c->n_ranks, nb_loc = (1 << c->P.F1) >> c->log2n, spb = N * 8, n_seg = nb_loc * spb, b = c->cur;
	BFCG_CK(hipSetDevice(c->prm.device));
	const size_t words = (size_t)3 * n_seg + 1 + nb_loc + 1;
	if (words > c->seg_words) return fail("internal: %zu segment words, room for %zu", words, c->seg_words);
	if (!slab_cap || !mg_async_ok(c)) return fail("internal: mg_process_slabs_dev needs slabs and no debug_seen");
	if (rec_bound > c->recv_cap) rec_bound = c->recv_cap;
	uint32_t *d = c->d_seg + (size_t)b * c->seg_words;
	for (int i = 0; i < n_wait; ++i) BFCG_CK(hipStreamWaitEvent(c->st, wait[i], 0));
	BFCG_CK(hipEventRecord(c->evt[b][6], c->st));
	run_seg_setup_mg(c->P, c->rw / 4, d_rows_in, (uint32_t)(nb_loc * 8 + 2), N, s_lo, s_hi, slab_cap, d, nullptr, c->st);
	const int n_q = c->n_opq;
	if (mg_stage_b(c, b, d_recv, d, n_seg, spb, rec_bound, nullptr, 1, 0) != 0) return -1;
	c->unfinished_mg = c->n_opq > n_q ? c->opq[n_q].mg : 0;
	c->unfinished = 1;
	return 0;
}
int bfcg::mg_process_finish(bfcg_ctx_t *c, const uint32_t *fills)
{
	if (!c->unfinished) return fail("internal: no stage B waits for its sizes");
	const int N = c->n_ranks, nb_loc = (1 << c->P.F1) >> c->log2n, b = c->cur;
	c->unfinished = 0;
	uint64_t tot = 0;
	for (size_t i = 0; i < (size_t)N * nb_loc * 8; ++i) tot += fills[i];
	c->slot_pos[b] = tot;
	if (c->unfinished_mg) {
		memcpy(c->mg_seg[c->unfinished_mg - 1], fills, sizeof(uint32_t) * (size_t)N * nb_loc * 8);
		for (int i = 0; i < c->n_opq; ++i) if (c->opq[i].mg == c->unfinished_mg) c->opq[i].n_pos = tot;
		c->unfinished_mg = 0;
	}
	return finalise_previous(c, b);
}

static int use_stream(bfcg_ctx_t *c)
{
	if (c->stream_mode) {
		if (!c->P.seg && !c->stream_out) BFCG_CK(hipMalloc(&c->stream_out, c->recs2_n * (uint64_t)c->rw));
		++c->n_stream_batches;
	}
	return 0;
}

static int finalise_previous(bfcg_ctx_t *c, int b)
{
	if (c->pend) {
		const int pb = b ^ 1;
		BFCG_CK(hipEventSynchronize(c->evB[pb]));
		if (batch_times(c, pb) != 0) return -1;
		if (c->n_opq && c->opq[0].slot == pb) {
			if (c->h_flags[pb][1]) { c->pend = 1; c->cur = b ^ 1; return drain(c); }
			for (int i = 1; i < c->n_opq; ++i) c->opq[i - 1] = c->opq[i];
			--c->n_opq;
		}
		fold_snapshot(c, pb);
		note_growth(c);
		if (c->h_stats[ST_ERR_POOL] || c->h_stats[ST_TAB_OVF] || (c->P.seg ? seg_target_shift(c) != c->P.seg_shift : (c->B.table && table_target_cshift(c) != c->P.tab_cshift))) {
			c->pend = 1; c->cur = b ^ 1;
			return drain(c);
		}
	}
	c->pend = 1; c->cur = b ^ 1;
	return 0;
}


static int commit_pending_pages(bfcg_ctx_t *c, int b)
{
	if (!c->ho_pending) return 0;
	const uint32_t nf = (uint32_t)nfine(c);
	BatchBufs Bt = c->B;
	Bt.ho = c->ho; Bt.ho_stride = c->ho_stride; Bt.ho_cur = c->ho_cur; Bt.ho_mark = c->ho_mark; Bt.ho_mark_stride = nf; Bt.ho_keys = c->ho_keys;
	BFCG_CK(hipMemsetAsync(c->ho_keys, 0, sizeof(unsigned long long) * ST_SLOTS * (size_t)c->ho_pending, c->st));
	run_commit_pages(c->P, Bt, nf, (uint32_t)c->ho_pending, c->st);
	BFCG_CK(hipMemcpyAsync(c->h_ho_keys[b], c->ho_keys, sizeof(unsigned long long) * ST_SLOTS * (size_t)c->ho_pending, hipMemcpyDeviceToHost, c->st));
	c->slot_commit[b] = c->ho_pending;
	memcpy(c->slot_page_call[b], c->ho_page_call, sizeof(uint64_t) * (size_t)c->ho_pending);
	c->ho_pending = 0;
	return 0;
}
static int handover_begin(bfcg_ctx_t *c, BatchBufs &Bt, int b, int slabs, uint64_t call)
{
	c->slot_commit[b] = 0; c->slot_all_committed[b] = 1;
	if (!c->P.seg) return 0;
	const uint32_t nf = (uint32_t)nfine(c);
	Bt.stream_out = (uint32_t *)c->ho;
	Bt.ho = c->ho; Bt.ho_cur = c->ho_cur; Bt.ho_mark = c->ho_mark; Bt.ho_mark_stride = nf; Bt.ho_keys = c->ho_keys;
	if (!slabs || c->ho_stride == 0 || Bt.seen_out) {
		if (commit_pending_pages(c, b) != 0) return -1;
		Bt.ho_stride = 0; Bt.ho_page = 0; Bt.ho_commit = 1; Bt.ho_keys = nullptr;
		return 0;
	}
	if (c->ho_pending == 0) {
		int w = 1;
		if (c->ho_K > 1 && c->n_commits > 0) {
			const double room = 0.85 * (double)((uint64_t)nf << c->P.seg_shift) - (double)c->keys_known, g = 1.1 * (double)(c->keys_per_batch ? c->keys_per_batch : 1);
			w = room <= g ? 1 : room / g >= (double)c->ho_K ? c->ho_K : (int)(room / g);
		}
		c->ho_window = w;
		if (getenv("BFCG_DEBUG")) fprintf(stderr, "[D::window] %d batches: keys %llu, largest page of the last commit %llu, slots %llu, commits so far %d\n", w,
			(unsigned long long)c->keys_known, (unsigned long long)c->keys_per_batch, (unsigned long long)((uint64_t)nf << c->P.seg_shift), c->n_commits);
	}
	Bt.ho_stride = c->ho_stride; Bt.ho_page = (uint32_t)c->ho_pending;
	c->ho_page_call[c->ho_pending++] = call;
	Bt.ho_commit = c->ho_pending >= c->ho_window;
	if (Bt.ho_commit) BFCG_CK(hipMemsetAsync(c->ho_keys, 0, sizeof(unsigned long long) * ST_SLOTS * (size_t)c->ho_pending, c->st));
	else c->slot_all_committed[b] = 0;
	return 0;
}
static int handover_end(bfcg_ctx_t *c, const BatchBufs &Bt, int b)
{
	if (!c->P.seg || Bt.ho_stride == 0 || !Bt.ho_commit) return 0;
	BFCG_CK(hipMemcpyAsync(c->h_ho_keys[b], c->ho_keys, sizeof(unsigned long long) * ST_SLOTS * (size_t)c->ho_pending, hipMemcpyDeviceToHost, c->st));
	c->slot_commit[b] = c->ho_pending;
	memcpy(c->slot_page_call[b], c->ho_page_call, sizeof(uint64_t) * (size_t)c->ho_pending);
	c->ho_pending = 0;
	return 0;
}
static void absorb_pages(bfcg_ctx_t *c, int b)
{
	const int J = c->slot_commit[b];
	if (!J) return;
	uint64_t run = c->keys_known, most = 0;
	for (int j = 0; j < J; ++j) {
		const unsigned long long *row = c->h_ho_keys[b] + (size_t)j * ST_SLOTS;
		uint64_t d = 0;
		for (int i = 0; i < ST_SLOTS; ++i) d += row[i];
		run += d;
		if (d > most) most = d;
		c->call_keys[c->slot_page_call[b][j] & 63] = run;
	}
	c->keys_per_batch = most; ++c->n_commits;
	c->final_call = c->slot_page_call[b][J - 1];
	c->keys_known = run;
	c->slot_commit[b] = 0;
	c->commit_absorbed = 1;
}

static int same_block_offset(bfcg_ctx_t *c, int b, const uint8_t *d_seq, const uint8_t **d_qual, uint64_t n_pos, hipStream_t s)
{
	if (!*d_qual || ((((uintptr_t)d_seq) ^ ((uintptr_t)*d_qual)) & 15) == 0) return 0;
	uint8_t *dst = c->d_qual2[b] + (((uintptr_t)d_seq) & 15);
	BFCG_CK(hipMemcpyAsync(dst, *d_qual, n_pos, hipMemcpyDeviceToDevice, s));
	*d_qual = dst;
	return 0;
}

static int ensure_agg(bfcg_ctx_t *c)
{
	if (c->P.filter_mode || c->P.seg || c->B.agg_out) return 0;
	BFCG_CK(hipMalloc(&c->B.agg_out, nfine(c) * c->P.ag_cap * (c->P.track ? 32 : 24)));
	return 0;
}

static int enqueue_batch(bfcg_ctx_t *c, const uint8_t *d_seq, const uint8_t *d_qual, uint64_t n_pos, int wait_copy, int no_kstats)
{
	const int b = c->cur, nb1 = 1 << c->P.F1;
	BatchBufs Bt;
	if (batch_bufs(c, Bt) != 0) return -1;
	Bt.rows1 = c->rows1[b]; Bt.chunk1 = c->chunk1[b]; Bt.start1 = c->start1[b]; Bt.row_base = Bt.start1 + nb1 + 1; Bt.recs1 = c->recs1[b];
	hipStream_t sA = c->pipeline ? c->stA : c->st;
	if (c->used[b]) BFCG_CK(hipStreamWaitEvent(sA, c->evB[b], 0));
	if (!c->pipeline && wait_copy) BFCG_CK(hipStreamWaitEvent(sA, c->evCopy, 0));
	const int op_run = c->onepass && !no_kstats;
	const int op = op_run && n_pos >= c->op_min_pos;
	const KParams Pt = batch_params(c, no_kstats, op);
	StageB w = {};
	w.seq = d_seq; w.qual = d_qual;
	if (same_block_offset(c, b, d_seq, &d_qual, n_pos, sA) != 0) return -1;
	if (op_run) Bt.op_sticky = c->op_flags + OP_STICKY;
	if (op) {
		Bt.op_cursor = c->op_cursor[b]; Bt.op_seg = c->op_seg[b]; Bt.op_flags = c->op_flags + 4 * b; Bt.op_cap = c->op_cap;
		Bt.cnt2 = c->cnt2; Bt.cap2 = c->cap2;
		run_stage_a_onepass(Pt, Bt, d_seq, d_qual, (int64_t)n_pos, Bt.recs1, sA, c->evt[b]);
	} else run_stage_a(Pt, Bt, d_seq, d_qual, (int64_t)n_pos, Bt.recs1, sA, c->evt[b]);
	BFCG_CK(hipEventRecord(c->evA[b], sA));
	BFCG_CK(hipStreamWaitEvent(c->st, c->evA[b], 0));
	BFCG_CK(hipEventRecord(c->evt[b][6], c->st));
	if (c->B.seen_out) BFCG_CK(hipMemsetAsync(c->B.seen_out, 0, n_pos, c->st));
	w.in1 = Bt.recs1; w.segs_per_bucket = op ? 8 : 1; w.n_seg = nb1 * w.segs_per_bucket;
	if (op) {
		const uint32_t *sg = c->op_seg[b];
		w.seg_beg = sg; w.seg_end = sg + 8 * nb1; w.row_base = sg + 16 * nb1; w.bucket_start = sg + 24 * nb1 + 1; w.rec_bound = (uint64_t)8 * nb1 * c->op_cap;
	} else { w.seg_beg = Bt.start1; w.seg_end = Bt.start1 + 1; w.row_base = Bt.row_base; w.bucket_start = Bt.start1; w.rec_bound = n_pos; }
	w.slabs = op && Bt.cap2; w.queued = op_run; w.call = c->call_no; w.pos = n_pos; w.finalise = 1;
	return enqueue_stage_b(c, b, Bt, Pt, w);
}

static uint64_t split_limit(const bfcg_ctx_t *c);
static void split_rule(const bfcg_ctx_t *c, uint64_t *from, uint64_t *target_max)
{
	const uint64_t lim = split_limit(c);
	if (c->cold) { const char *e = getenv("BFCG_COLD_FRAC"); *target_max = e ? (uint64_t)((double)lim * atof(e)) : lim - lim / 10; *from = *target_max; }
	else {
		double unseen = 0.79 - c->seen_per_pos;
		if (unseen < 0.2) unseen = 0.2;
		double w = getenv("BFCG_NO_WARM_BATCHES") ? 1.0 : 0.6 / 0.95 / unseen;
		if (w < 1.0) w = 1.0;
		*target_max = (uint64_t)((double)lim * w); *from = *target_max + *target_max / 6;
	}
}
static uint64_t split_limit(const bfcg_ctx_t *c)
{
	const uint64_t nf = nfine(c);
	const uint32_t cap = c->P.b3 && c->cold && c->list_cap_c ? c->list_cap_c : c->P.list_cap;
	if (c->P.b3fm) return (uint64_t)((double)nf * (double)cap * 0.95 * 1.6);
	return (uint64_t)((double)nf * (double)cap * 0.95);
}
static uint64_t find_cut(const uint8_t *seq, int on_device, uint64_t lo, uint64_t hi)
{
	const uint64_t win = hi - lo < (1u << 20) ? hi - lo : (1u << 20);
	const uint8_t *p = seq + hi - win;
	uint8_t *tmp = 0;
	if (on_device) {
		tmp = (uint8_t *)malloc(win);
		if (hipMemcpy(tmp, p, win, hipMemcpyDeviceToHost) != hipSuccess) { free(tmp); return 0; }
		p = tmp;
	}
	uint64_t cut = 0;
	for (uint64_t i = win; i > 0; --i) if (!is_acgt(p[i - 1])) { cut = hi - win + i; break; }
	free(tmp);
	return cut > lo ? cut : 0;
}

extern "C" uint64_t bfcg_batch_limit(bfcg_ctx_t *c) { return split_limit(c); }
double bfcg::mg_warm_factor(bfcg_ctx_t *c)
{
	if (c->cold || getenv("BFCG_NO_WARM_BATCHES")) return 1.0;
	double unseen = 1.0 - c->seen_per_pos;
	if (unseen < 0.2) unseen = 0.2;
	const double w = 0.6 / unseen;
	return w < 1.0 ? 1.0 : w;
}



__global__ __launch_bounds__(256) void k_expand_planes(const uint32_t *__restrict__ pl, uint64_t pw, uint32_t bit_off, uint64_t n_pos, int has_qual,
                                                        uint8_t *__restrict__ seq, uint8_t *__restrict__ qual)
{
	const uint64_t i0 = ((uint64_t)blockIdx.x * 256 + threadIdx.x) * 16;
	if (i0 >= n_pos) return;
	const uint64_t s = i0 + bit_off, k = s >> 5;
	const uint32_t sh = (uint32_t)s & 31u;
	auto take = [&](int p) -> uint32_t {
		const uint32_t *w = pl + (uint64_t)p * pw + k;
		const unsigned long long v = (unsigned long long)w[0] | ((unsigned long long)w[1] << 32);
		return (uint32_t)(v >> sh) & 0xffffu;
	};
	const uint32_t m0 = take(0), m1 = take(1), mn = take(2), mq = has_qual ? take(3) : 0u;
	auto spread = [](uint32_t nib) -> uint32_t { return ((nib & 0xFu) * 0x00204081u) & 0x01010101u; };
	uint32_t sw[4], qw[4];
#pragma unroll
	for (int d = 0; d < 4; ++d) {
		const uint32_t c0 = spread(m0 >> (4 * d)), c1 = spread(m1 >> (4 * d)), nn = spread(mn >> (4 * d)) * 0xFFu, hq = spread(mq >> (4 * d));
		const uint32_t base = 0x41414141u + c0 * 2u + c1 * 6u + (c0 & c1) * 0x0bu;
		sw[d] = (base & ~nn) | (0x0a0a0a0au & nn);
		qw[d] = 0x80808080u - hq;
	}
	if (i0 + 16 <= n_pos) {
		*reinterpret_cast<uint4 *>(seq + i0) = make_uint4(sw[0], sw[1], sw[2], sw[3]);
		if (has_qual) *reinterpret_cast<uint4 *>(qual + i0) = make_uint4(qw[0], qw[1], qw[2], qw[3]);
	} else {
		for (uint64_t i = i0; i < n_pos; ++i) {
			const int j = (int)(i - i0);
			seq[i] = (uint8_t)(sw[j >> 2] >> (8 * (j & 3)));
			if (has_qual) qual[i] = (uint8_t)(qw[j >> 2] >> (8 * (j & 3)));
		}
	}
// ... 278 lines not shown
```

### bfc_amd/csrc/bfcg_dev.h

```cpp
#pragma once
#include <hip/hip_runtime.h>
#include <stdint.h>
#include "kmer_dev.h"
#include "bfcg_internal.h"

using namespace bfcg;

template <int RD> struct RecW { uint32_t d[RD]; };

template <int RD> __device__ __forceinline__ RecW<RD> rec_load(const uint32_t *p);
template <> __device__ __forceinline__ RecW<3> rec_load<3>(const uint32_t *p)
{ const uint3 v = *reinterpret_cast<const uint3 *>(p); RecW<3> r; r.d[0] = v.x; r.d[1] = v.y; r.d[2] = v.z; return r; }
template <> __device__ __forceinline__ RecW<4> rec_load<4>(const uint32_t *p)
{ const uint4 v = *reinterpret_cast<const uint4 *>(p); RecW<4> r; r.d[0] = v.x; r.d[1] = v.y; r.d[2] = v.z; r.d[3] = v.w; return r; }
template <> __device__ __forceinline__ RecW<5> rec_load<5>(const uint32_t *p)
{ RecW<5> r; r.d[0] = p[0]; r.d[1] = p[1]; r.d[2] = p[2]; r.d[3] = p[3]; r.d[4] = p[4]; return r; }
template <int RD> __device__ __forceinline__ void rec_store(uint32_t *p, const RecW<RD> &r);
template <> __device__ __forceinline__ void rec_store<3>(uint32_t *p, const RecW<3> &r)
{ *reinterpret_cast<uint3 *>(p) = make_uint3(r.d[0], r.d[1], r.d[2]); }
template <> __device__ __forceinline__ void rec_store<4>(uint32_t *p, const RecW<4> &r)
{ *reinterpret_cast<uint4 *>(p) = make_uint4(r.d[0], r.d[1], r.d[2], r.d[3]); }
template <> __device__ __forceinline__ void rec_store<5>(uint32_t *p, const RecW<5> &r)
{ p[0] = r.d[0]; p[1] = r.d[1]; p[2] = r.d[2]; p[3] = r.d[3]; p[4] = r.d[4]; }


struct TabOrder {
	unsigned long long *first, *sub_last;
	__device__ __forceinline__ void note(uint32_t sub, uint64_t slot, unsigned long long sf, unsigned long long sl) const
	{
		if (first) { atomicMin(&first[slot], sf); atomicMax(&sub_last[sub], sl); }
	}
};


#define FS_EMPTY 0xffffffffffffffffULL

template <bool GLOBAL>
__device__ __forceinline__ bool fs_insert(unsigned long long *tab, uint32_t cap_mask, uint32_t bitoff, uint32_t idx, uint32_t max_probe)
{
	const unsigned long long e = ((unsigned long long)bitoff << 32) | idx;
	uint32_t p = ((bitoff * 0x9E3779B1u) >> 12 ^ bitoff) & cap_mask;
	for (uint32_t probe = 0; probe <= max_probe; ++probe, p = (p + 1) & cap_mask) {
		unsigned long long cur = GLOBAL ? __hip_atomic_load(&tab[p], __ATOMIC_RELAXED, __HIP_MEMORY_SCOPE_AGENT) : tab[p];
		if (cur == FS_EMPTY) {
			cur = atomicCAS(&tab[p], FS_EMPTY, e);
			if (cur == FS_EMPTY) return true;
		}
		if ((uint32_t)(cur >> 32) == bitoff) { if (e < cur) atomicMin(&tab[p], e); return true; }
	}
	return false;
}
template <bool GLOBAL>
__device__ __forceinline__ bool fs_lookup(const unsigned long long *tab, uint32_t cap_mask, uint32_t bitoff, uint32_t &first)
{
	uint32_t p = ((bitoff * 0x9E3779B1u) >> 12 ^ bitoff) & cap_mask;
	for (uint32_t probe = 0; probe <= cap_mask; ++probe, p = (p + 1) & cap_mask) {
		unsigned long long cur = GLOBAL ? __hip_atomic_load((unsigned long long *)&tab[p], __ATOMIC_RELAXED, __HIP_MEMORY_SCOPE_AGENT) : tab[p];
		if (cur == FS_EMPTY) return false;
		if ((uint32_t)(cur >> 32) == bitoff) { first = (uint32_t)cur; return true; }
	}
	return false;
}

struct BloomArgs {
	const uint32_t *recs;
	const uint32_t *start;
	unsigned long long *bloom;
	unsigned long long *bloom_hi;
	unsigned long long *table;
	unsigned long long *stats;
	uint64_t *tab_ovf; uint32_t tab_ovf_cap; unsigned long long *ovf_cnt;
	unsigned long long *pool; uint32_t pool_slices;
	uint8_t *seen_out;
	uint64_t *agg_out;
	uint32_t *agg_cnt;
	uint32_t *stream_out;
	unsigned long long *seg_tab;
	uint32_t n_fine;
	TabOrder ord;
	unsigned long long batch_hi;
	const uint32_t *cnt2; uint32_t cap2;
	unsigned long long *ho; uint32_t ho_stride; uint32_t *ho_cur; uint32_t *ho_mark;
	uint32_t ho_pages, ho_mark_stride;
	unsigned long long *ho_keys;
	const uint32_t *flags;
	const uint32_t *sticky;
};

__device__ __forceinline__ void region_list(const BloomArgs &A, uint32_t f, uint32_t &rs, uint32_t &n)
{
	if (A.cap2) { const uint32_t c = A.cnt2[f]; rs = f * A.cap2; n = c < A.cap2 ? c : A.cap2; }
	else if (A.cnt2) { rs = A.start[f]; n = A.cnt2[f]; }
	else { rs = A.start[f]; n = A.start[f + 1] - rs; }
}
__device__ __forceinline__ bool batch_poisoned(const BloomArgs &A) { return (A.sticky && *A.sticky) || (A.flags && (A.flags[0] | A.flags[2])); }


struct Dec3 { int ok, a, lo, n, up, sh_x, R, sh_flag, sh_y1; uint32_t lowmask, rmask, mk32; };
__device__ __forceinline__ Dec3 dec3_geom(const KParams &P)
{
	Dec3 g;
	g.a = P.k - P.rec_n; g.lo = P.rec_lo; g.n = P.rec_n; g.up = P.rec_n ? P.rec_lo : P.bf_shift - 9; g.sh_x = P.k - (P.bf_shift - 9);
	g.R = P.R; g.sh_flag = g.a + P.k - 32; g.sh_y1 = P.k - P.F;
	g.lowmask = P.rec_n ? (1u << (P.rec_lo & 31)) - 1u : 0xffffffffu; g.rmask = (1u << P.R) - 1u; g.mk32 = P.k >= 32 ? 0xffffffffu : (1u << P.k) - 1u;
	g.ok = P.k >= P.bf_shift - 9 && P.bf_shift + 9 <= 2 * P.k && g.a >= 1 && g.a <= 31 && g.a + P.k >= 32 && (P.rec_n == 0 || P.rec_lo + P.rec_n <= 31)
	       && g.up <= g.a && g.sh_x >= 0 && g.sh_x <= 31 && g.sh_y1 >= 0 && g.sh_y1 <= 32 && (P.rec_n == 0 || P.rec_lo + P.rec_n == P.bf_shift - 9) && P.R <= g.up;
	return g;
}

#define FS32_EMPTY 0xffffffffu
__device__ __forceinline__ uint32_t fs32_slot(uint32_t bitoff, uint32_t mask) { return ((bitoff * 0x9E3779B1u) >> 12 ^ bitoff) & mask; }

__device__ __forceinline__ bool fs32_insert(unsigned int *fs, uint32_t mask, uint32_t bitoff, uint32_t li, uint32_t idx, const unsigned int *list_idx)
{
	const uint32_t e = (bitoff << 13) | li;
	uint32_t p = fs32_slot(bitoff, mask);
	for (int probe = 0; probe < 1024; ++probe, p = (p + 1) & mask) {
		uint32_t cur = fs[p];
		if (cur == FS32_EMPTY) {
			cur = atomicCAS(&fs[p], FS32_EMPTY, e);
			if (cur == FS32_EMPTY) return true;
		}
		if ((cur >> 13) == bitoff) {
			while (list_idx[cur & 0x1fffu] > idx) {
				uint32_t old = atomicCAS(&fs[p], cur, e);
				if (old == cur) break;
				cur = old;
			}
			return true;
		}
	}
	return false;
}
__device__ __forceinline__ bool fs32_compete(unsigned int *fs, uint32_t mask, uint32_t bitoff, uint32_t li, uint32_t idx, const unsigned int *list_idx)
{
	const uint32_t e = (bitoff << 13) | li;
	uint32_t p = fs32_slot(bitoff, mask);
	for (uint32_t probe = 0; probe <= mask; ++probe, p = (p + 1) & mask) {
		uint32_t cur = fs[p];
		if (cur == FS32_EMPTY) return false;
		if ((cur >> 13) == bitoff) {
			while (list_idx[cur & 0x1fffu] > idx) {
				uint32_t old = atomicCAS(&fs[p], cur, e);
				if (old == cur) break;
				cur = old;
			}
			return true;
		}
	}
	return false;
}
__device__ __forceinline__ uint32_t fs32_lookup(const unsigned int *fs, uint32_t mask, uint32_t bitoff)
{
	uint32_t p = fs32_slot(bitoff, mask);
	for (uint32_t probe = 0; probe <= mask; ++probe, p = (p + 1) & mask) {
		uint32_t cur = fs[p];
		if (cur == FS32_EMPTY) return FS32_EMPTY;
		if ((cur >> 13) == bitoff) return cur & 0x1fffu;
	}
	return FS32_EMPTY;
}


struct B3Pos { uint32_t b0, b1, b2, b3; };
__device__ __forceinline__ B3Pos b3_positions(uint32_t h1, uint32_t h2)
// ... 25 lines not shown
```

### bfc_amd/csrc/bfcg_internal.h

```cpp
#pragma once
#include <hip/hip_runtime.h>
#define BFCG_TILE1 4096
#define BFCG_BT1 256
#define BFCG_SCAN_CH 64
static inline int bfcg_rec_dwords(int k, int rec_n) { const int bits = 2 * k - rec_n + 33; return bits <= 96 ? 3 : bits <= 128 ? 4 : 5; }
static constexpr int bfcg_tile_of_rw(int rw) { return rw == 5 ? 2048 : rw == 4 ? 3072 : 4096; }
static constexpr int bfcg_tile1_of_rw(int rw) { return rw == 3 ? 4096 : 3072; }
#define BFCG_MAXB 1024
#define BFCG_HO_MAX_PAGES 8
#ifdef BFCG_MEASURE
#define BFCG_ABL(P, bits) ((P).ablate & (bits))
#else
#define BFCG_ABL(P, bits) 0
#endif
#include <stdint.h>
struct bfcg_ctx; struct bfcg_kcov;

extern "C" void bfcg_set_error(const char *msg);
extern "C" void *bfcg_bloom_slice(struct bfcg_ctx *c, int which, uint64_t *bytes);
extern "C" int bfcg_resident_register(const void *bf, void *dev, int device, int n_shift);

#define BFCG_UT_NBUF 20
struct bfcg_kmers {
	int k, l_pre, cshift, device, owns_table;
	hipStream_t st;
	hipEvent_t e0, e1;
	const unsigned long long *table;
	unsigned long long *d_hist;
	uint32_t *d_sizes;
	uint32_t *d_cnt; unsigned long long *d_off; uint64_t blk_cap;
	ulonglong2 *d_y; uint16_t *d_ch; uint64_t out_cap;
	ulonglong2 *d_qy; int16_t *d_qout; uint64_t q_cap;
	uint8_t *d_pseq; uint64_t pseq_cap; int16_t *d_pout; uint64_t pout_cap;
	unsigned long long *d_roff; uint64_t roff_cap; int32_t *d_rout; uint64_t rout_cap;
	int16_t *d_oth; uint64_t oth_cap;
	uint32_t *d_jpart; uint64_t jpart_cap;
	unsigned long long *d_joint;
	uint8_t *d_gout; uint64_t gout_cap;
	int32_t *d_gls; uint64_t gls_cap;
	void *d_ut[BFCG_UT_NBUF]; uint64_t ut_bytes[BFCG_UT_NBUF];
	uint64_t ut_cap;
	uint64_t n_keys; int has_keys;
	float last_ms;
};

namespace bfcg {
#define BFCG_LOCAL __attribute__((visibility("hidden")))

enum { ST_KMERS = 0, ST_HIGH, ST_SEEN, ST_KEYS, ST_TAB_OVF, ST_ERR_POOL, ST_SLOW_BUCKETS, ST_CROWDED , ST_N = 16 };
enum { ST_SLOTS = 256 };

struct KParams {
	int k, q, bf_shift, n_hashes, l_pre, filter_mode;
	int R;
	int F, F1, F2;
	int tab_cshift;
	uint32_t fs_cap, list_cap;
	uint32_t ag_cap;
	uint32_t idx_rank;
	int track;
	int ablate;
	int bloom_bt;
	int seg;
	int seg_shift;
	int seg_blk;
	int seg_lo, seg_hi;
	uint32_t f_base;
	int no_kstats;
	int dedupe;
	uint32_t ct_cap;
	int rec_lo, rec_n;
	int b3;
	int b3_warm;
	int b3fm;
	int l2_big;
	int b3_cold;
};

struct BatchBufs {
	uint32_t *rows1, *chunk1;
	uint32_t *start1, *row_base;
	uint32_t *rows2, *start2;
	uint64_t *recs1, *recs2;
	uint64_t max_kmers;
	unsigned long long *bloom, *bloom_hi, *table;
	unsigned long long *stats;
	uint64_t *tab_ovf; uint32_t tab_ovf_cap;
	unsigned long long *pool; uint32_t pool_slices;
	uint8_t *seen_out;
	uint64_t *agg_out; uint32_t *agg_cnt;
	uint32_t *stream_out; int stream;
	uint32_t *op_cursor, *op_flags, *op_sticky, *op_seg; uint32_t op_cap;
	uint32_t op_own_lo, op_own_n, op_own_delta;
	uint32_t *cnt2; uint32_t cap2;
	uint32_t *cnt_live;
	unsigned long long *ho; uint32_t ho_stride; uint32_t *ho_cur, *ho_mark; uint32_t ho_mark_stride, ho_page; int ho_commit; unsigned long long *ho_keys;
	unsigned long long *seg_tab;
	unsigned long long *tab_first, *sub_last;
	unsigned long long batch_hi;
};

void run_stage_a(const KParams &P, const BatchBufs &B, const uint8_t *seq, const uint8_t *qual, int64_t n_pos, uint64_t *out1, hipStream_t st, hipEvent_t *ev);
void run_stage_a_onepass(const KParams &P, const BatchBufs &B, const uint8_t *seq, const uint8_t *qual, int64_t n_pos, uint64_t *out1, hipStream_t st, hipEvent_t *ev);
void run_stage_b(const KParams &P, const BatchBufs &B, const uint64_t *in1, const uint32_t *seg_beg, const uint32_t *seg_end, int n_seg, int segs_per_bucket,
                 const uint32_t *row_base, const uint32_t *bucket_start, uint64_t n_rec_bound, hipStream_t st, hipEvent_t *ev);
void run_pack_rows(const KParams &P, const BatchBufs &B, int n_ranks, uint32_t row_w, uint32_t *rows, hipStream_t st);
void run_seg_setup_mg(const KParams &P, int rw_dwords, const uint32_t *rows, uint32_t row_w, int n_ranks, int s_lo, int s_hi, uint32_t cap, uint32_t *seg, unsigned long long *total, hipStream_t st);
void run_batch(const KParams &P, const BatchBufs &B, const uint8_t *seq, const uint8_t *qual, int64_t n_pos, hipStream_t st, hipEvent_t *ev);
int bloom_lds_bytes(const KParams &P);
bool bloom3fm_geometry_ok(const KParams &P);
bool bloom3_geometry_ok(const KParams &P);
BFCG_LOCAL bool scatter2_big_ok(const KParams &P);
hipError_t set_bloom_lds_attr(const KParams &P);
void run_query(const KParams &P, const uint8_t *seq, int64_t n_pos, const void *bloom, uint8_t *flags, hipStream_t st);
void run_kcov(const KParams &P, const uint8_t *seq, int64_t n_pos, int min_occ, const void *tab, uint8_t *flags, uint16_t *out, hipStream_t st);
void run_streak(int k, float min_frac, const uint8_t *flags, const uint64_t *off, uint64_t n_reads, int32_t *out_start, int32_t *out_end, hipStream_t st);
void run_hash_only(const KParams &P, const uint8_t *seq, const uint8_t *qual, int64_t n_pos, uint64_t *out, hipStream_t st);
void run_table_replay(const KParams &P, unsigned long long *tab, const uint64_t *src, uint64_t n, unsigned long long *stats, uint64_t *ovf, uint32_t ovf_cap,
                      unsigned long long *first, unsigned long long *sub_last, hipStream_t st);
void run_seg_rehash(const KParams &P, const unsigned long long *old_tab, int old_shift, int old_blk, unsigned long long *new_tab, uint32_t n_fine, hipStream_t st);
void run_seg_replay(const KParams &P, unsigned long long *seg_tab, const uint64_t *src, uint64_t n, unsigned long long *stats, uint64_t *ovf, uint32_t ovf_cap, hipStream_t st);
void run_seg_to_table(const KParams &P, const unsigned long long *seg_tab, uint32_t n_fine, unsigned long long *tab, unsigned long long *stats, uint64_t *ovf, uint32_t ovf_cap, hipStream_t st);
hipError_t set_seg_lds_attr(void);
hipError_t set_scatter1wc_lds_attr(void);
void run_commit_pages(const KParams &P, const BatchBufs &B, uint32_t n_fine, uint32_t pages, hipStream_t st);
#define BFCG_SEG_MAX_SHIFT 14
#define BFCG_SEG_TOTAL_MAX 24
void run_table_rehash(const KParams &P, const unsigned long long *old_tab, int cshift_old, unsigned long long *new_tab,
                      const unsigned long long *old_first, unsigned long long *new_first, hipStream_t st);

BFCG_LOCAL int fail(const char *fmt, ...) __attribute__((format(printf, 1, 2)));
#define BFCG_CK(call) do { hipError_t e_ = (call); if (e_ != hipSuccess) return bfcg::fail("%s failed: %s (%s:%d)", #call, hipGetErrorString(e_), __FILE__, __LINE__); } while (0)
#define BFCG_CKN(cleanup, call) do { hipError_t e_ = (call); if (e_ != hipSuccess) { bfcg::fail("%s failed: %s (%s:%d)", #call, hipGetErrorString(e_), __FILE__, __LINE__); cleanup; (void)hipGetLastError(); return NULL; } } while (0)

static inline int is_acgt(uint8_t ch) { ch &= 0xDF; return ch == 'A' || ch == 'C' || ch == 'G' || ch == 'T'; }

struct resident_t { const void *host; void *dev; int device, n_shift, k, l_pre, cshift; };
BFCG_LOCAL int resident_put(const resident_t &r);
BFCG_LOCAL void *resident_take(const void *host, int device, int n_shift, int k, int l_pre, int cshift);

const unsigned long long *ctx_borrow_table(::bfcg_ctx *c, KParams *P, int *device);
int ctx_table_k(::bfcg_ctx *c);
BFCG_LOCAL int mg_scatter_again(::bfcg_ctx *c, const uint8_t *d_seq, const uint8_t *d_qual, uint64_t n_pos, void *d_send, uint32_t *counts);
BFCG_LOCAL int mg_slab_info(::bfcg_ctx *c, uint32_t out[2]);
BFCG_LOCAL int mg_scatter_slabs(::bfcg_ctx *c, const uint8_t *d_seq, const uint8_t *d_qual, uint64_t n_pos, void *d_send, uint32_t own_delta, uint32_t *fills, int *overflow);
BFCG_LOCAL int mg_row_words(::bfcg_ctx *c);
BFCG_LOCAL int mg_async_ok(::bfcg_ctx *c);
BFCG_LOCAL int mg_scatter_slabs_async(::bfcg_ctx *c, const uint8_t *d_seq, const uint8_t *d_qual, uint64_t n_pos, void *d_send, uint32_t own_delta, uint32_t *d_rows_out, hipEvent_t *done);
BFCG_LOCAL int mg_scatter_slabs_wait(::bfcg_ctx *c, uint32_t *fills, int *overflow);
BFCG_LOCAL int mg_process(::bfcg_ctx *c, const void *d_recv, const uint32_t *sizes, uint32_t slab_cap, hipEvent_t *wait, int n_wait);
BFCG_LOCAL int mg_process_slabs_dev(::bfcg_ctx *c, const void *d_recv, const uint32_t *d_rows_in, uint32_t slab_cap, uint64_t rec_bound, int s_lo, int s_hi, hipEvent_t *wait, int n_wait);
BFCG_LOCAL int mg_process_finish(::bfcg_ctx *c, const uint32_t *fills);
BFCG_LOCAL double mg_warm_factor(::bfcg_ctx *c);
const unsigned long long *kcov_table(::bfcg_kcov *t, KParams *P, int *device);
int kcov_adopted(::bfcg_kcov *t);
BFCG_LOCAL ::bfcg_kmers *kmers_new(int k, int l_pre, int cshift, int device);
BFCG_LOCAL uint64_t lookup_cap();
BFCG_LOCAL uint64_t unitig_cap();
BFCG_LOCAL int lookup_stage(::bfcg_kmers *t);
BFCG_LOCAL int profile_launch(::bfcg_kmers *t, const uint8_t *h_seq, const uint8_t *d_seq, uint64_t n_pos);
template <typename T> int grow(T *&buf, uint64_t &cap, uint64_t need, const char *what)
{
	if (need <= cap) return 0;
	(void)hipFree(buf); buf = NULL; cap = 0;
	hipError_t e = hipMalloc(&buf, need);
	if (e != hipSuccess) { buf = NULL; (void)hipGetLastError(); return fail("no room for %s of %llu bytes: %s", what, (unsigned long long)need, hipGetErrorString(e)); }
	cap = need;
	return 0;
}

}
```

### bfc_amd/csrc/bfcg_kernels.hip

```cpp
#include <hip/hip_runtime.h>
#include <stdint.h>
#include <stdlib.h>
#include <string.h>
#include <stdio.h>
#include "kmer_dev.h"
#include "bfcg_internal.h"
#include "bfcg_dev.h"
#include "bfcg_k1.h"

using namespace bfcg;

#define WAVE 64








template <typename W> __device__ __forceinline__ uint32_t fine_id(const KParams &P, uint64_t y0, uint64_t y1)
{
	W m = kmask<W>(P.k);
	uint64_t hash = bloom_hash<W>(P.k, (W)y0, (W)y1, m);
// ... 729 lines not shown
	}
	return false;
}

template <typename W, bool TRACK>
__device__ __forceinline__ void emit_seen(const KParams &P, const BloomArgs &A, const AggView &G, uint64_t y0, uint64_t y1, bool hi, uint32_t idx)
{
	if (BFCG_ABL(P, 2)) return;
	if (!agg_add<W, TRACK>(P, G, y0, y1, hi, idx)) commit_seen<W, TRACK>(P, A, y0, y1, 1u, (uint32_t)hi, TRACK ? idx : 0u, TRACK ? idx : 0u);
}

struct KRec { uint64_t y0, y1; uint32_t idx, bl, h1, h2; bool hi; uint32_t d0, d1; };

__device__ __forceinline__ KRec decode_fast3(const Dec3 g, const RecW<3> &w, uint32_t imp)
{
	KRec r;
	r.d0 = w.d[0]; r.d1 = w.d[1]; r.idx = w.d[2];
	const uint32_t y0d = w.d[0] & ((1u << g.a) - 1u), upper = y0d >> g.up;
	const uint32_t y0lo = g.n ? (y0d & g.lowmask) | (imp << g.lo) | (upper << (g.lo + g.n)) : y0d;
	const uint32_t y1lo = __builtin_amdgcn_alignbit(w.d[1], w.d[0], g.a) & g.mk32;
	const uint32_t x = (y0lo - y1lo) ^ y1lo;
	const uint32_t hh = upper | (x << g.sh_x);
	r.bl = y0d & g.rmask; r.h1 = hh & 511u; r.h2 = (hh >> 9) & 511u;
	if ((r.h2 & 31u) == 0) r.h2 = (r.h2 + 1) & 511u;
	r.hi = (w.d[1] >> g.sh_flag) & 1u;
	r.y0 = r.y1 = 0;
	return r;
}
__device__ __forceinline__ unsigned long long entry_fast3(const Dec3 g, const KRec &r, int k)
{
	const unsigned long long A = r.d0 | ((unsigned long long)r.d1 << 32);
	const unsigned long long y1 = (A >> g.a) & (k >= 64 ? ~0ULL : (1ULL << k) - 1);
	const uint32_t y0d = r.d0 & ((1u << g.a) - 1u);
	const unsigned long long id = (unsigned long long)((y0d & g.rmask) | ((y0d >> g.up) << g.R)) | (y1 << g.sh_y1);
	return (id << 1) | (unsigned long long)r.hi;
}

template <typename W, int RW>
__device__ __forceinline__ KRec decode_rec(const KParams &P, const RecW<RW> &w, W m, uint32_t rmask, uint32_t imp)
{
	KRec r;
	Rec<RW>::unpack(w, rec_geom(P), imp, r.y0, r.y1, r.idx, r.hi);
	BloomAddr a = bloom_addr(bloom_hash<W>(P.k, (W)r.y0, (W)r.y1, m), P.bf_shift);
	r.bl = (uint32_t)a.blk & rmask; r.h1 = a.h1; r.h2 = a.h2;
	r.d0 = r.d1 = 0;
	return r;
}

__device__ __forceinline__ uint32_t ct_home(uint32_t cls, uint32_t mask) { return ((cls * 0x9E3779B1u) >> 9 ^ cls) & mask; }
__device__ __forceinline__ void ct_insert(unsigned long long *ct, uint32_t mask, uint32_t cls, uint32_t idx)
{
	const unsigned long long e = ((unsigned long long)cls << 32) | idx;
	for (uint32_t p = ct_home(cls, mask);; p = (p + 1) & mask) {
		unsigned long long cur = ct[p];
		if (cur == FS_EMPTY) { cur = atomicCAS(&ct[p], FS_EMPTY, e); if (cur == FS_EMPTY) return; }
		if ((uint32_t)(cur >> 32) == cls) { if (e < cur) atomicMin(&ct[p], e); return; }
	}
}
__device__ __forceinline__ uint32_t ct_first(const unsigned long long *ct, uint32_t mask, uint32_t cls)
{
	for (uint32_t p = ct_home(cls, mask);; p = (p + 1) & mask) {
		const unsigned long long cur = ct[p];
		if ((uint32_t)(cur >> 32) == cls) return (uint32_t)cur;
	}
}

template <typename W, int RW, int BT, int PF, int NH, bool TRACK, bool FM = false, bool STREAM = false, bool SEGOUT = false, bool F3 = false>
__global__ __launch_bounds__(BT, BT == 512 ? 6 : 8) void k_bloom(KParams P, BloomArgs A)
{
	if (BFCG_ABL(P, 8)) return;
	extern __shared__ __attribute__((aligned(16))) unsigned char smem[];
	__shared__ uint32_t s_list_n, s_ovf, s_pool_off, s_seen, s_agg_n, s_fs_used, s_pad[2];
	const uint32_t f = blockIdx.x;
	const bool ho_log = SEGOUT && A.ho_stride != 0;
	if (batch_poisoned(A)) { if (ho_log && threadIdx.x == 0) A.ho_mark[f] = A.ho_cur[f]; return; }
	uint32_t rs, n;
	region_list(A, f, rs, n);
	if (n == 0) { if (threadIdx.x == 0) { if (ho_log) A.ho_mark[f] = A.ho_cur[f]; else if (A.agg_cnt) A.agg_cnt[f] = 0; } return; }
	uint32_t ho_cur0 = 0;
	unsigned long long *ho_base = nullptr;
	if (SEGOUT) {
		if (ho_log) {
			ho_cur0 = A.ho_cur[f];
			if (ho_cur0 + n > A.ho_stride) {
				if (threadIdx.x == 0) { atomicAdd(&A.stats[(size_t)(f & (ST_SLOTS - 1)) * ST_N + ST_ERR_POOL], 1ULL); A.ho_mark[f] = ho_cur0; }
				return;
			}
			ho_base = A.ho + (uint64_t)f * A.ho_stride + ho_cur0;
		} else ho_base = reinterpret_cast<unsigned long long *>(A.stream_out) + rs;
	}
	A.stats += (size_t)(f & (ST_SLOTS - 1)) * ST_N;
	const int region_blocks = 1 << P.R;
	const uint32_t region_dw = region_blocks * 16;
	constexpr bool two = sizeof(W) == 8;
	unsigned char *sp = smem;
	unsigned int *region = reinterpret_cast<unsigned int *>(sp); sp += (size_t)region_dw * 4;
	AggView G;
	unsigned int *region_hi = nullptr;
	if (FM) { region_hi = reinterpret_cast<unsigned int *>(sp); sp += (size_t)region_dw * 4; G.id0 = G.id1 = nullptr; G.cnt = G.imin = G.imax = nullptr; G.mask = 0; }
	else if (STREAM) { G.id0 = G.id1 = nullptr; G.cnt = G.imin = G.imax = nullptr; G.mask = 0; }
	else {
		G.id0 = reinterpret_cast<unsigned long long *>(sp); sp += (size_t)P.ag_cap * 8;
		G.id1 = G.id0;
		if (two) { G.id1 = reinterpret_cast<unsigned long long *>(sp); sp += (size_t)P.ag_cap * 8; }
		G.cnt = reinterpret_cast<unsigned int *>(sp); sp += (size_t)P.ag_cap * 8;
		G.imin = G.imax = nullptr;
		if (TRACK) { G.imin = reinterpret_cast<unsigned int *>(sp); sp += (size_t)P.ag_cap * 4; G.imax = reinterpret_cast<unsigned int *>(sp); sp += (size_t)P.ag_cap * 4; }
		G.mask = P.ag_cap - 1;
	}
	unsigned int *fs = reinterpret_cast<unsigned int *>(sp); sp += (size_t)P.fs_cap * 4;
	unsigned int *list_a = reinterpret_cast<unsigned int *>(sp); sp += (size_t)P.list_cap * 4;
	unsigned int *list_b = reinterpret_cast<unsigned int *>(sp);
	const uint32_t fs_mask = P.fs_cap - 1;
	const uint32_t *recs = A.recs + (uint64_t)rs * RW;
	unsigned int *g_region = reinterpret_cast<unsigned int *>(A.bloom) + (uint64_t)f * region_dw;
	unsigned int *g_region_hi = FM ? reinterpret_cast<unsigned int *>(A.bloom_hi) + (uint64_t)f * region_dw : nullptr;
	const W m = kmask<W>(P.k);
	const uint32_t rmask = region_blocks - 1;
	const uint32_t imp = (P.f_base + f) >> P.F2;
	const int nh = NH ? NH : P.n_hashes;
	static_assert(!F3 || (RW == 3 && SEGOUT), "the fast decode is for 12-byte records into the hand-over log");
	const Dec3 D3 = dec3_geom(P);
	constexpr bool fast3 = F3;
	auto dec = [&](const RecW<RW> &w) -> KRec {
		if constexpr (F3) return decode_fast3(D3, *reinterpret_cast<const RecW<3> *>(&w), imp);
		else return decode_rec<W, RW>(P, w, m, rmask, imp);
	};
	const bool dd = P.dedupe && P.ct_cap >= 2u * BT * PF && n <= (uint32_t)(BT * PF) && n <= P.list_cap && P.R <= 10;

	const bool timing = BFCG_ABL(P, 64) && threadIdx.x == 0;
	long long tq[7] = {0, 0, 0, 0, 0, 0, 0};
	if (timing) tq[0] = clock64();

	RecW<RW> rw[PF];
#pragma unroll
	for (int u = 0; u < PF; ++u) {
		uint32_t i = threadIdx.x + u * BT;
		if (i < n) {
			rw[u] = rec_load<RW>(recs + (uint64_t)i * RW);
		}
	}
	{
		const uint4 *src = reinterpret_cast<const uint4 *>(g_region);
		uint4 *dst = reinterpret_cast<uint4 *>(region);
		for (uint32_t i = threadIdx.x; i < region_dw / 4; i += BT) dst[i] = src[i];
		for (uint32_t i = threadIdx.x; i < (dd ? 2u * P.ct_cap : P.fs_cap); i += BT) fs[i] = FS32_EMPTY;
		if (FM) {
			const uint4 *src2 = reinterpret_cast<const uint4 *>(g_region_hi);
			uint4 *dst2 = reinterpret_cast<uint4 *>(region_hi);
			for (uint32_t i = threadIdx.x; i < region_dw / 4; i += BT) dst2[i] = src2[i];
		} else if (!STREAM) {
			for (uint32_t i = threadIdx.x; i < P.ag_cap; i += BT) {
				G.id0[i] = FS_EMPTY; if (two) G.id1[i] = FS_EMPTY; G.cnt[2 * i] = 0; G.cnt[2 * i + 1] = 0;
				if (TRACK) { G.imin[i] = 0xffffffffu; G.imax[i] = 0; }
			}
		}
		if (threadIdx.x == 0) { s_list_n = 0; s_seen = 0; s_agg_n = 0; s_ovf = 0; s_fs_used = 0; }
	}
	__syncthreads();
	if (timing) tq[1] = clock64();

	uint32_t n_seen = 0;
	volatile uint32_t *v_ovf = &s_ovf;
	const int lane = threadIdx.x & 63;

	auto clear_mask = [&](const KRec &r) -> uint32_t {
		uint32_t z = r.h1, um = 0;
// ... 975 lines not shown
}

template <typename W, int RW>
static void run_stage_a_onepass_t(const KParams &P, const BatchBufs &B, const uint8_t *seq, const uint8_t *qual, int64_t n_pos, uint32_t *out1, hipStream_t st, hipEvent_t *ev)
{
	constexpr int T1 = bfcg_tile1_of_rw(RW), T2 = bfcg_tile_of_rw(RW);
	const int nb1 = 1 << P.F1;
	const int64_t tiles1 = (n_pos + T1 - 1) / T1;
	if (ev) hipEventRecord(ev[0], st);
	hipMemsetAsync(B.op_cursor, 0, ((size_t)8 * nb1 * 32 + 32) * sizeof(uint32_t), st);
	hipMemsetAsync(B.op_flags, 0, 4 * sizeof(uint32_t), st);
	if (ev) hipEventRecord(ev[1], st);
	unsigned g1 = (unsigned)(((tiles1 + 7) / 8) * 8);
	const size_t lds1 = scatter1_lds_bytes(RW, nb1, true, P.rec_n);
	OnePass OP{B.op_cursor, B.op_cap, B.op_flags, B.stats, 1u, B.op_own_lo, B.op_own_n, B.op_own_delta};
	{
		static int n_cu = 0;
		if (!n_cu) { hipDeviceProp_t pr; int dev = 0; n_cu = (hipGetDevice(&dev) == hipSuccess && hipGetDeviceProperties(&pr, dev) == hipSuccess) ? pr.multiProcessorCount : 256; }
		int per_cu = (int)((size_t)160 * 1024 / (lds1 + 4400)); if (per_cu > 2) per_cu = 2; if (per_cu < 1) per_cu = 1;
		const char *e = getenv("BFCG_S1_WGS"); if (e && atoi(e) > 0) per_cu = atoi(e);
		const unsigned gp = (unsigned)(n_cu * per_cu) & ~7u;
		if (gp >= 8 && gp < g1) g1 = gp;
	}
	if (B.cnt_live) {
		const char *e = getenv("BFCG_S1_CHUNK");
		const int forced = e ? atoi(e) : 0;
		uint32_t ch = 32;
		while (ch > 1 && (uint64_t)(g1 / 8) * (ch / 2) * 36 > B.op_cap) ch >>= 1;
		OP.chunk = forced > 0 ? (uint32_t)forced : ch;
	}
	WcPlan wc;
	const bool fast = RW == 3 && scatter1_fast(P);
	const int v = !fast ? S1V_ONEPASS : sizeof(W) == 8 && P.k == 33 ? S1V_FAST_K33 : S1V_FAST;
	if ((fast || RW == 4) && B.cnt_live && scatter1_wc_plan(P, OP, RW, n_pos, &wc)) run_scatter1_wc(P, seq, qual, n_pos, out1, OP, wc, st);
	else hipLaunchKernelGGL(have(scatter1_kernel<W, RW>(v), "k_scatter1", v, RW), dim3(g1), dim3(BTS1), lds1, st, P, seq, qual, n_pos, nullptr, out1, OP);
	dbg_sync(st, "k_scatter1 (one pass)");
	uint32_t *sg = B.op_seg;
	hipLaunchKernelGGL(k_seg_setup, dim3(1), dim3(1024), 0, st, P, B.op_cursor, B.op_cap, B.op_flags, (RW == 3 && P.l2_big) ? TILE2_BIG : T2, sg, sg + 8 * nb1, sg + 16 * nb1, sg + 24 * nb1 + 1);
	dbg_sync(st, "k_seg_setup");
	if (ev) hipEventRecord(ev[2], st);
}

static inline bool scatter2_fast(const KParams &P)
{
	const int a = P.k - P.rec_n;
	return P.k >= P.bf_shift - 9 && P.F2 > 0 && P.R + P.F2 <= 31 && a >= P.R + P.F2 && P.rec_lo == P.R + P.F2 && !getenv("BFCG_NO_FAST_S2");
}

static inline bool bloom_fast3(const KParams &P)
{
	const int a = P.k - P.rec_n, up = P.rec_n ? P.rec_lo : P.bf_shift - 9, sh_x = P.k - (P.bf_shift - 9), sh_y1 = P.k - P.F;
	return P.k >= P.bf_shift - 9 && P.bf_shift + 9 <= 2 * P.k && a >= 1 && a <= 31 && a + P.k >= 32 && (P.rec_n == 0 || P.rec_lo + P.rec_n <= 31)
	       && up <= a && sh_x >= 0 && sh_x <= 31 && sh_y1 >= 0 && sh_y1 <= 32 && (P.rec_n == 0 || P.rec_lo + P.rec_n == P.bf_shift - 9) && P.R <= up && !getenv("BFCG_NO_FAST_BLOOM");
}

bool bloom3fm_geometry_ok(const KParams &P)
{
	const int up = P.rec_n ? P.rec_lo : P.bf_shift - 9, a = P.k - P.rec_n, io = a + P.k + 1;
	return bfcg_rec_dwords(P.k, P.rec_n) == 4 && P.n_hashes == 4 && P.R <= 8 && P.k >= P.bf_shift + 9 && (P.rec_n == 0 || P.rec_lo + P.rec_n == P.bf_shift - 9)
	       && P.R <= up && up >= 1 && up <= 31 && a >= up + 18 && io + 32 <= 128;
}
bool bloom3_geometry_ok(const KParams &P) { return bfcg_rec_dwords(P.k, P.rec_n) == 3 && P.n_hashes == 4 && P.R <= 8 && bloom_fast3(P); }
bool scatter2_big_ok(const KParams &P) { return bfcg_rec_dwords(P.k, P.rec_n) == 3 && scatter2_fast(P); }

static dim3 seg_grid(const KParams &P, uint32_t n_fine, uint32_t bt)
{
	const uint32_t ub = (uint32_t)(P.seg_shift - P.seg_blk);
	const uint64_t wgs = (uint64_t)n_fine << ub;
	static const bool force2d = getenv("BFCG_SEG_GRID2D") != nullptr;
	if (wgs * bt < (1ULL << 32) && !force2d) return dim3((unsigned)wgs, 1u);
	return dim3(n_fine, 1u << ub);
}
static void launch_commit_seg(const KParams &P, const BloomArgs &A, int nfine, hipStream_t st)
{
	const BloomK k = commit_seg_kernel(P.seg_blk);
	hipLaunchKernelGGL(k.fn, seg_grid(P, (uint32_t)nfine, (uint32_t)k.bt), dim3(k.bt), commit_seg_lds_bytes(P.seg_blk), st, P, A);
	dbg_sync(st, "k_commit_seg");
}
void run_commit_pages(const KParams &P, const BatchBufs &B, uint32_t n_fine, uint32_t pages, hipStream_t st)
{
	BloomArgs A;
	memset(&A, 0, sizeof(A));
	A.stats = B.stats; A.tab_ovf = B.tab_ovf; A.tab_ovf_cap = B.tab_ovf_cap; A.ovf_cnt = B.stats + (size_t)ST_SLOTS * ST_N; A.seg_tab = B.seg_tab; A.n_fine = n_fine;
	A.ho = B.ho; A.ho_stride = B.ho_stride; A.ho_cur = B.ho_cur; A.ho_mark = B.ho_mark; A.ho_mark_stride = B.ho_mark_stride; A.ho_pages = pages; A.ho_keys = B.ho_keys;
	launch_commit_seg(P, A, (int)n_fine, st);
}

template <typename W, int RW>
static std::pair<const uint32_t *, const uint32_t *> run_level2_t(const KParams &P, const BatchBufs &B, const uint32_t *in1, const uint32_t *seg_beg, const uint32_t *seg_end, int n_seg,
                                                                  int segs_per_bucket, const uint32_t *row_base, const uint32_t *bucket_start, uint64_t n_rec_bound, hipStream_t st)
{
	if (P.F2 == 0) return {in1, bucket_start};
	const int nb_loc = n_seg / segs_per_bucket, nfine = nb_loc << P.F2;
	int v = S2V_TWO_PASS;
	if (B.cap2) {
		const bool fast = (RW == 3 || RW == 4) && scatter2_fast(P);
		v = !fast ? S2V_ONEPASS : RW == 3 && P.l2_big ? S2V_FAST_BIG : S2V_FAST;
		hipMemsetAsync(B.cnt2, 0, sizeof(uint32_t) * (size_t)nfine, st);
	} else {
		hipLaunchKernelGGL((k_hist2<W, RW, bfcg_tile_of_rw(RW), BT2>), dim3(level2_grid(n_rec_bound, bfcg_tile_of_rw(RW), n_seg)), dim3(BT2), 0, st, P, in1, seg_beg, seg_end, n_seg, segs_per_bucket, row_base, B.rows2);
		hipLaunchKernelGGL(k_scan2, dim3(nb_loc), dim3((1 << P.F2) < 64 ? 64 : (1 << P.F2)), 0, st, P, bucket_start, segs_per_bucket, row_base, B.rows2, B.start2, B.cnt_live);
	}
	const Scatter2K k = scatter2_kernel<W, RW>(v);
	hipLaunchKernelGGL(have(k.fn, "k_scatter2", v, RW), dim3(level2_grid(n_rec_bound, k.tile, n_seg)), dim3(k.bt), scatter2_lds_bytes(RW, k.tile, 1 << P.F2), st, P, in1, seg_beg, seg_end, n_seg, segs_per_bucket, row_base,
	                   B.cap2 ? nullptr : B.rows2, (uint32_t *)B.recs2, B.cap2 ? OnePass2{B.cnt2, B.cap2, B.op_flags} : OnePass2{nullptr, 0u, nullptr});
	dbg_sync(st, "level 2");
	return {(const uint32_t *)B.recs2, B.start2};
}

template <typename W, int RW>
static BloomArgs run_bloom_t(const KParams &P, const BatchBufs &B, const uint32_t *fine_recs, const uint32_t *fine_start, int nfine, hipStream_t st)
{
	BloomArgs A;
	memset(&A, 0, sizeof(A));
	A.recs = fine_recs; A.start = fine_start; A.bloom = B.bloom; A.bloom_hi = B.bloom_hi; A.table = B.table; A.stats = B.stats;
	A.tab_ovf = B.tab_ovf; A.tab_ovf_cap = B.tab_ovf_cap; A.ovf_cnt = B.stats + (size_t)ST_SLOTS * ST_N; A.pool = B.pool; A.pool_slices = B.pool_slices; A.seen_out = B.seen_out;
	A.agg_out = B.agg_out; A.agg_cnt = B.agg_cnt; A.n_fine = (uint32_t)nfine; A.stream_out = nullptr; A.seg_tab = nullptr;
	A.ord.first = B.tab_first; A.ord.sub_last = B.sub_last; A.batch_hi = B.batch_hi;
	A.cnt2 = nullptr; A.cap2 = 0; A.flags = B.op_flags; A.sticky = B.op_sticky;
	if (P.F2 > 0 && B.cap2) { A.cnt2 = B.cnt2; A.cap2 = B.cap2; }
	else if (P.F2 > 0 && B.cnt_live) A.cnt2 = B.cnt_live;
	const bool h4 = P.n_hashes == 4;
	if (P.filter_mode && B.bloom_hi) {
		if (RW == 4 && P.b3fm) run_bloom3fm(P, A, nfine, (size_t)bloom_lds_bytes(P), st);
		else launch_bloom<W, RW>(!h4 ? BV_FM_ANYH : P.bloom_bt == 1024 ? BV_FM_1024 : BV_FM, P, A, nfine, st);
	} else if (P.seg && B.seg_tab && (B.stream_out || B.ho)) {
		A.stream_out = B.stream_out; A.seg_tab = B.seg_tab; A.table = nullptr; A.agg_out = nullptr;
		A.ho = B.ho; A.ho_stride = B.ho_stride; A.ho_cur = B.ho_cur; A.ho_mark = B.ho_stride ? B.ho_mark + (size_t)B.ho_page * B.ho_mark_stride : nullptr;
		if (RW == 3 && P.b3 && (P.b3_cold || !P.dedupe)) run_bloom3(P, A, nfine, (size_t)bloom_lds_bytes(P), st);
		else launch_bloom<W, RW>(!h4 ? BV_SEG_ANYH : RW == 3 && bloom_fast3(P) ? BV_SEG_F3 : BV_SEG, P, A, nfine, st);
	} else if (B.stream && B.stream_out && !P.track && h4) {
		A.stream_out = B.stream_out;
		launch_bloom<W, RW>(BV_STREAM, P, A, nfine, st);
	} else if (P.track) launch_bloom<W, RW>(h4 ? BV_TRACK : BV_TRACK_ANYH, P, A, nfine, st);
	else launch_bloom<W, RW>(!h4 ? BV_ANYH : P.bloom_bt == 1024 ? BV_1024 : BV_512, P, A, nfine, st);
	return A;
}

template <typename W, int RW>
static void run_commit_t(const KParams &P, const BatchBufs &B, BloomArgs &A, int nfine, hipStream_t st)
{
	const auto waves = [&] { return dim3((unsigned)((nfine + 4 * COMMIT_RPW - 1) / (4 * COMMIT_RPW))); };
	if (A.seg_tab) {
		if (B.ho_stride == 0 || B.ho_commit) {
			A.ho_mark = B.ho_mark; A.ho_mark_stride = B.ho_mark_stride; A.ho_pages = B.ho_page + 1; A.ho_keys = B.ho_keys;
			launch_commit_seg(P, A, nfine, st);
		}
	} else if (A.stream_out) hipLaunchKernelGGL((k_commit_stream<W, RW>), waves(), dim3(256), 0, st, P, A);
	else if (B.agg_out && nfine > (1 << 18)) hipLaunchKernelGGL((P.track ? k_commit<W, true, true> : k_commit<W, false, true>), waves(), dim3(256), 0, st, P, A);
	else if (B.agg_out) hipLaunchKernelGGL((P.track ? k_commit<W, true, false> : k_commit<W, false, false>), dim3((unsigned)(((uint64_t)nfine * P.ag_cap + 255) / 256)), dim3(256), 0, st, P, A);
}

template <typename W, int RW>
static void run_stage_b_t(const KParams &P, const BatchBufs &B, const uint32_t *in1, const uint32_t *seg_beg, const uint32_t *seg_end, int n_seg,
                          int segs_per_bucket, const uint32_t *row_base, const uint32_t *bucket_start, uint64_t n_rec_bound, hipStream_t st, hipEvent_t *ev)
{
	const int nfine = (n_seg / segs_per_bucket) << P.F2;
	const auto [fine_recs, fine_start] = run_level2_t<W, RW>(P, B, in1, seg_beg, seg_end, n_seg, segs_per_bucket, row_base, bucket_start, n_rec_bound, st);
	if (ev) hipEventRecord(ev[3], st);
	BloomArgs A = run_bloom_t<W, RW>(P, B, fine_recs, fine_start, nfine, st);
	if (ev) hipEventRecord(ev[4], st);
	if (A.seg_tab || A.stream_out) dbg_sync(st, "k_bloom");
	run_commit_t<W, RW>(P, B, A, nfine, st);
	if (A.flags) hipLaunchKernelGGL(k_seal, dim3(1), dim3(1), 0, st, B.op_flags, B.op_sticky);
	if (ev) hipEventRecord(ev[5], st);
}

#define DISPATCH_W(fn, ...) do { const int rw_ = bfcg_rec_dwords(P.k, P.rec_n); \
	if (P.k <= 32) { if (rw_ == 3) fn<uint32_t, 3>(__VA_ARGS__); else fn<uint32_t, 4>(__VA_ARGS__); } \
	else if (rw_ == 3) fn<uint64_t, 3>(__VA_ARGS__); else if (rw_ == 4) fn<uint64_t, 4>(__VA_ARGS__); else fn<uint64_t, 5>(__VA_ARGS__); } while (0)

void run_stage_a(const KParams &P, const BatchBufs &B, const uint8_t *seq, const uint8_t *qual, int64_t n_pos, uint64_t *out1, hipStream_t st, hipEvent_t *ev)
{ DISPATCH_W(run_stage_a_t, P, B, seq, qual, n_pos, (uint32_t *)out1, st, ev); }

void run_stage_a_onepass(const KParams &P, const BatchBufs &B, const uint8_t *seq, const uint8_t *qual, int64_t n_pos, uint64_t *out1, hipStream_t st, hipEvent_t *ev)
{ DISPATCH_W(run_stage_a_onepass_t, P, B, seq, qual, n_pos, (uint32_t *)out1, st, ev); }

void run_pack_rows(const KParams &P, const BatchBufs &B, int n_ranks, uint32_t row_w, uint32_t *rows, hipStream_t st)
{
	const int nb1 = 1 << P.F1;
	hipLaunchKernelGGL(k_pack_rows, dim3((unsigned)n_ranks), dim3(256), 0, st, B.op_seg + (size_t)8 * nb1, B.op_flags, nb1 / n_ranks, B.op_cap, row_w, rows);
}
void run_seg_setup_mg(const KParams &P, int rw_dwords, const uint32_t *rows, uint32_t row_w, int n_ranks, int s_lo, int s_hi, uint32_t cap, uint32_t *seg, unsigned long long *total, hipStream_t st)
{
	const int nb1 = 1 << P.F1, nb_loc = nb1 / n_ranks, n_seg = nb1 * 8;
	hipLaunchKernelGGL(k_seg_setup_mg, dim3(1), dim3(1024), 0, st, rows, row_w, n_ranks, s_lo, s_hi, nb_loc, cap, bfcg_tile_of_rw(rw_dwords), seg, seg + n_seg, seg + 2 * n_seg, seg + 3 * n_seg + 1, total);
}

void run_stage_b(const KParams &P, const BatchBufs &B, const uint64_t *in1, const uint32_t *seg_beg, const uint32_t *seg_end, int n_seg, int segs_per_bucket,
                 const uint32_t *row_base, const uint32_t *bucket_start, uint64_t n_rec_bound, hipStream_t st, hipEvent_t *ev)
{ DISPATCH_W(run_stage_b_t, P, B, (const uint32_t *)in1, seg_beg, seg_end, n_seg, segs_per_bucket, row_base, bucket_start, n_rec_bound, st, ev); }

void run_batch(const KParams &P, const BatchBufs &B, const uint8_t *seq, const uint8_t *qual, int64_t n_pos, hipStream_t st, hipEvent_t *ev)
{
	run_stage_a(P, B, seq, qual, n_pos, B.recs1, st, ev);
	run_stage_b(P, B, B.recs1, B.start1, B.start1 + 1, 1 << P.F1, 1, B.row_base, B.start1, (uint64_t)n_pos, st, ev);
}

int bloom_lds_bytes(const KParams &P)
{
	const size_t second = P.filter_mode ? ((size_t)64 << P.R) : P.seg ? 0 : (size_t)P.ag_cap * ((P.k > 32 ? 24 : 16) + (P.track ? 8 : 0));
	if (P.b3fm) return (int)(((size_t)128 << P.R) + ((size_t)2 << P.R) * 4 + 16 + (size_t)P.list_cap * 10 + 16);
	if (P.b3 && P.b3_cold) return (int)(((size_t)64 << P.R) + ((size_t)2 << P.R) * 4 + 16 + (size_t)P.list_cap * 12 + 16);
	return (int)(((size_t)64 << P.R) + (size_t)P.fs_cap * 4 + second + (size_t)P.list_cap * (P.b3 ? 10 : 8) + 16);
}

template <typename W, int RW> static void register_lds_t(int lds, hipError_t *err)
{
	hipError_t e = hipSuccess;
	for (int v = 0; v < S1V_N && e == hipSuccess; ++v) if (const Scatter1Fn fn = scatter1_kernel<W, RW>(v)) e = set_max_lds((const void *)fn, scatter1_lds_bytes(RW, BFCG_MAXB, v != S1V_TWO_PASS, 1));
	for (int v = 0; v < S2V_N && e == hipSuccess; ++v) if (const Scatter2K k = scatter2_kernel<W, RW>(v); k.fn) e = set_max_lds((const void *)k.fn, scatter2_lds_bytes(RW, k.tile, BFCG_MAXB));
// ... 82 lines not shown
```

### include/bfc_gpu.h

```cpp
#ifndef BFC_GPU_H
#define BFC_GPU_H

#include <stdint.h>

#ifdef __cplusplus
extern "C" {
#endif


typedef struct { uint64_t x[4]; } bfc_kmer_t;

#define BFC_BLK_SHIFT 9
#define BFC_BLK_MASK  ((1 << BFC_BLK_SHIFT) - 1)
typedef struct { int n_shift, n_hashes; uint8_t *b; } bfc_bf_t;

bfc_bf_t *bfc_bf_init(int n_shift, int n_hashes);
void      bfc_bf_destroy(bfc_bf_t *b);
int       bfc_bf_insert(bfc_bf_t *b, uint64_t hash);
int       bfc_bf_get(const bfc_bf_t *b, uint64_t hash);

#define BFC_CH_KEYBITS 50
#define BFC_CH_MAXPRE  24
struct bfc_ch_s;
typedef struct bfc_ch_s bfc_ch_t;
// ... 18 lines not shown
	int l_pre, bf_shift, n_hashes;
	int discard;
	int max_end_ext;
	int win_multi_ec;
	int min_cov;
	int w_ec, w_ec_high, w_absent, w_absent_high;
	int max_path_diff, max_heap;
} bfc_opt_t;

void *bfc_count(const char *fn, const bfc_opt_t *opt);

void bfc_correct(const char *fn, const bfc_opt_t *opt, const void *ptr);


typedef struct bfcg_ctx bfcg_ctx_t;

typedef struct {
	int k, q, bf_shift, n_hashes, l_pre, filter_mode;
	int device;
	uint64_t max_batch_pos;
	int region_shift;
	int tab_cshift;
	int debug_seen;
	int track_order;
	int rank, n_ranks;
	int table_layout;
} bfcg_params_t;

void bfcg_params_default(bfcg_params_t *p);
bfcg_ctx_t *bfcg_create(const bfcg_params_t *p);
void bfcg_destroy(bfcg_ctx_t *c);
const char *bfcg_last_error(void);
const char *bfcg_build_id(void);
int bfcg_device_count(void);
int bfcg_reset(bfcg_ctx_t *c);

int bfcg_count_batch_dev(bfcg_ctx_t *c, const uint8_t *d_seq, const uint8_t *d_qual, uint64_t n_pos);
int bfcg_count_batch_host(bfcg_ctx_t *c, const uint8_t *h_seq, const uint8_t *h_qual, uint64_t n_pos);
uint64_t bfcg_plane_words(uint64_t n_pos);
void bfcg_pack_planes(const uint8_t *seq, const uint8_t *qual, uint64_t lo, uint64_t hi, uint64_t n_pos, int q, uint32_t *planes, uint64_t plane_words);
int bfcg_count_batch_planes(bfcg_ctx_t *c, const uint32_t *h_planes, uint64_t plane_words, uint64_t first_pos, uint64_t n_pos, int has_qual);
int bfcg_sync(bfcg_ctx_t *c);

int bfcg_mg_info(bfcg_ctx_t *c, int out[4]);
uint64_t bfcg_batch_limit(bfcg_ctx_t *c);
int bfcg_mg_scatter(bfcg_ctx_t *c, const uint8_t *d_seq, const uint8_t *d_qual, uint64_t n_pos, void *d_send, uint32_t *counts);
int bfcg_mg_process(bfcg_ctx_t *c, const void *d_recv, const uint32_t *seg_cnt);
void bfcg_mg_allow_onepass(bfcg_ctx_t *c, int on);

enum { BFCG_ST_KMERS = 0, BFCG_ST_HIGH, BFCG_ST_SEEN, BFCG_ST_KEYS, BFCG_ST_TAB_OVF, BFCG_ST_ERR_POOL, BFCG_ST_SLOW_BUCKETS, BFCG_ST_CROWDED,
       BFCG_ST_TAB_CSHIFT = 8, BFCG_ST_BATCHES, BFCG_ST_N = 16 };

typedef struct bfcg_group bfcg_group_t;
#define BFCG_UID_BYTES 128
int bfcg_group_unique_id(uint8_t uid[BFCG_UID_BYTES]);
bfcg_group_t *bfcg_group_create(const bfcg_params_t *prm, int n_ranks, int first_rank, int n_local, const int *devices, const uint8_t *uid, int transport);
void bfcg_group_destroy(bfcg_group_t *g);
int bfcg_group_info(bfcg_group_t *g, int out[6]);
int bfcg_group_exchange_bytes(bfcg_group_t *g, uint64_t out[4]);
bfcg_ctx_t *bfcg_group_ctx(bfcg_group_t *g, int i);
int bfcg_group_slab_mode(bfcg_group_t *g);
uint64_t bfcg_group_lazy_batches(bfcg_group_t *g);
int bfcg_group_reset(bfcg_group_t *g);
int bfcg_group_count_batch_dev(bfcg_group_t *g, const uint8_t *const *d_seq, const uint8_t *const *d_qual, const uint64_t *n_pos);
int bfcg_group_count_batch_host(bfcg_group_t *g, const uint8_t *h_seq, const uint8_t *h_qual, uint64_t n_pos);
int bfcg_group_sync(bfcg_group_t *g);
int bfcg_group_stats(bfcg_group_t *g, uint64_t out[BFCG_ST_N]);
int bfcg_group_progress(bfcg_group_t *g, uint64_t *batches, uint64_t *final, uint64_t *keys_of, int n);
bfc_ch_t *bfcg_group_export_table(bfcg_group_t *g);
bfc_bf_t *bfcg_group_export_bloom(bfcg_group_t *g, int which);
bfc_bf_t *bfcg_group_export_bloom_resident(bfcg_group_t *g, int which);

void *bfcg_dev_alloc(bfcg_ctx_t *c, uint64_t bytes);
void  bfcg_dev_free(bfcg_ctx_t *c, void *p);
int   bfcg_h2d(bfcg_ctx_t *c, void *dst, const void *src, uint64_t bytes);
int   bfcg_d2h(bfcg_ctx_t *c, void *dst, const void *src, uint64_t bytes);
void *bfcg_host_alloc(uint64_t bytes);
void  bfcg_host_free(void *p);

int bfcg_stats(bfcg_ctx_t *c, uint64_t out[BFCG_ST_N]);
int bfcg_progress(bfcg_ctx_t *c, uint64_t *calls, uint64_t *final, uint64_t *keys_of, int n);
int bfcg_table_info(bfcg_ctx_t *c, int out[4]);
int bfcg_partition_info(bfcg_ctx_t *c, uint64_t out[2]);
uint64_t bfcg_s1wc_launches(void);
uint64_t bfcg_stream_batches(bfcg_ctx_t *c);

int bfcg_last_batch_ms(bfcg_ctx_t *c, float out[6]);
int bfcg_stage_ms(bfcg_ctx_t *c, double out[6], uint64_t *n_batches, int reset);

int bfcg_bloom_to_host(bfcg_ctx_t *c, int which , uint8_t *dst);
bfc_bf_t *bfcg_export_bloom(bfcg_ctx_t *c, int which);
bfc_bf_t *bfcg_export_bloom_resident(bfcg_ctx_t *c, int which);
void bfcg_resident_drop(const void *bf);
bfc_ch_t *bfcg_export_table(bfcg_ctx_t *c);
bfc_ch_t *bfcg_export_table_resident(bfcg_ctx_t *c);

int bfc_ingest_digest(const char *fn, uint64_t chunk_size, uint64_t cap, int n_threads, uint64_t out[7]);
int bfc_ingest_planes_digest(const char *fn, uint64_t chunk_size, uint64_t cap, int n_threads, int q, int direct, uint64_t out[7]);
int bfc_pgz_digest(const char *fn, int n_threads, uint64_t chunk, uint64_t window, uint64_t out[5]);

bfc_ch_t *bfc_ch_union(const bfc_ch_t *const *tabs, int n);

int      bfc_ch_get_lpre(const bfc_ch_t *ch);
uint64_t bfc_ch_export_sorted(const bfc_ch_t *ch, uint32_t *sizes, uint64_t *slots);

typedef struct bfcg_trim bfcg_trim_t;
bfcg_trim_t *bfcg_trim_create(int k, const bfc_bf_t *bf, int device, uint64_t max_pos, uint64_t max_reads);
void bfcg_trim_destroy(bfcg_trim_t *t);
int bfcg_trim_batch(bfcg_trim_t *t, const uint8_t *h_seq, const uint8_t *d_seq, uint64_t n_pos, const uint64_t *h_off, uint64_t n_reads,
                    float min_frac, int32_t *start, int32_t *end);
float bfcg_trim_last_ms(bfcg_trim_t *t);
int bfcg_trim_adopted(bfcg_trim_t *t);
void *bfcg_trim_dev_seq(bfcg_trim_t *t);

typedef struct bfcg_kcov bfcg_kcov_t;
bfcg_kcov_t *bfcg_kcov_create(const bfc_ch_t *ch, int device, uint64_t max_pos);
bfcg_kcov_t *bfcg_kcov_attach(bfcg_ctx_t *ctx, uint64_t max_pos);
void bfcg_kcov_destroy(bfcg_kcov_t *t);
int bfcg_kcov_batch(bfcg_kcov_t *t, const uint8_t *h_seq, const uint8_t *d_seq, uint64_t n_pos, int min_occ, uint16_t *out);
float bfcg_kcov_last_ms(bfcg_kcov_t *t);
void *bfcg_kcov_dev_seq(bfcg_kcov_t *t);
void *bfcg_kcov_dev_out(bfcg_kcov_t *t);

typedef struct bfcg_ec bfcg_ec_t;
bfcg_ec_t *bfcg_ec_create(const bfc_ch_t *ch, const bfc_opt_t *opt, int device, uint64_t max_pos, uint64_t max_reads);
bfcg_ec_t *bfcg_ec_attach(bfcg_ctx_t *ctx, const bfc_opt_t *opt, uint64_t max_pos, uint64_t max_reads);
int   bfcg_ec_batch(bfcg_ec_t *e, uint8_t *seq, uint8_t *qual, uint64_t n_pos, const uint64_t *off, uint64_t n_reads, uint32_t *aux, uint32_t *aux2);
void  bfcg_ec_destroy(bfcg_ec_t *e);
float bfcg_ec_last_ms(bfcg_ec_t *e);
uint64_t bfcg_ec_host_reads(bfcg_ec_t *e);
uint64_t bfcg_ec_last_lookups(bfcg_ec_t *e);
uint64_t bfcg_ec_retry_reads(bfcg_ec_t *e);
int   bfcg_ec_adopted(bfcg_ec_t *e);
int   bfcg_ec1_host(const bfc_ch_t *ch, const bfc_opt_t *opt, int mode, char *seq, char *qual, uint32_t *aux, uint32_t *aux2);
int   bfcg_ec_batch_refine(bfcg_ec_t *e, uint8_t *seq, uint8_t *qual, uint64_t n_pos, const uint64_t *off, uint64_t n_reads,
                           const uint32_t *ori_aux, const uint32_t *ori_aux2, uint32_t *aux, uint32_t *aux2);
int   bfcg_ec1_host_refine(const bfc_ch_t *ch, const bfc_opt_t *opt, int mode, char *seq, char *qual, uint32_t ori_aux, uint32_t ori_aux2,
                           uint32_t *aux, uint32_t *aux2);
int   bfcg_ec_parse_stats(const char *comment, uint32_t *aux, uint32_t *aux2);

typedef struct bfcg_kmers bfcg_kmers_t;
bfcg_kmers_t *bfcg_kmers_create(const bfc_ch_t *ch, int device);
bfcg_kmers_t *bfcg_kmers_attach(bfcg_ctx_t *ctx);
void  bfcg_kmers_destroy(bfcg_kmers_t *t);
int   bfcg_kmers_info(bfcg_kmers_t *t, int out[3]);
int   bfcg_kmers_hist(bfcg_kmers_t *t, uint64_t cnt[256], uint64_t high[64]);
int   bfcg_kmers_sub_sizes(bfcg_kmers_t *t, uint32_t *sizes);
int   bfcg_kmers_hist_sizes(bfcg_kmers_t *t, uint64_t cnt[256], uint64_t high[64], uint32_t *sizes);
int   bfcg_kmers_list(bfcg_kmers_t *t, int min_cnt, int min_diff, uint32_t sub_lo, uint32_t sub_hi, uint64_t *y, uint16_t *cnt_high, uint64_t cap, uint64_t *n);
float bfcg_kmers_last_ms(bfcg_kmers_t *t);
int   bfcg_kmer_decode_host(int k, int l_pre, uint32_t sub, uint64_t slot, uint64_t y[2]);
void  bfcg_kmer_2str(int k, const uint64_t y[2], char *buf);
uint64_t bfcg_kmers_format(int k, const uint64_t *y, const uint16_t *cnt_high, uint64_t n, char *buf);
uint64_t bfcg_kmers_format_sizes(const uint32_t *sizes, uint64_t n, char *buf);
int   bfcg_kmers_lookup(bfcg_kmers_t *t, const uint64_t *y, uint64_t n, int16_t *out, uint64_t *n_found);
int   bfcg_kmers_profile(bfcg_kmers_t *t, const uint8_t *h_seq, const uint8_t *d_seq, uint64_t n_pos, int16_t *out);
int   bfcg_kmer_from_str(int k, const char *s, uint64_t y[2]);
int   bfcg_kmer_occ_host(const bfc_ch_t *ch, const uint64_t y[2]);
void  bfcg_kmers_occ_host(const bfc_ch_t *ch, const uint64_t *y, uint64_t n, int16_t *out);
uint64_t bfcg_kmers_parse(int k, const char *text, uint64_t len, uint64_t *y, uint64_t cap, uint64_t *bad_line);
uint64_t bfcg_lookup_format(const char *text, uint64_t len, const int16_t *occ, uint64_t n, char *buf);
uint64_t bfcg_profile_format(const int16_t *occ, uint64_t n, char *buf);
int   bfcg_kmers_read_stats(bfcg_kmers_t *t, const uint8_t *h_seq, const uint8_t *d_seq, uint64_t n_pos, const uint64_t *h_off, uint64_t n_reads,
                            int min_cov, int32_t *out);
int   bfcg_read_stats_host(const bfc_ch_t *ch, const uint8_t *seq, uint64_t n_pos, const uint64_t *off, uint64_t n_reads, int min_cov, int32_t *out);
uint64_t bfcg_read_stats_format(const int32_t *out, uint64_t n_reads, char *buf);
// ... 36 lines not shown
```

Baseline: 41890.

## Split handover log into two halves and optionally commit on a side stream

Splits the per-bucket handover log into two halves so one half can be committed into the segmented table while the next batches write into the other. A new stream stK runs the commit kernel alongside stage B when BFCG_COMMIT_OVERLAP is set, coordinated through events, and the table-growth heuristics account for commits still in flight. The default commit window K rises from 4 to 8, split into two halves of 4. The overlap path is off by default, so the default run mostly sees the halved-buffer bookkeeping and the larger K.

```diff
diff --git a/bfc_amd/_lib.py b/bfc_amd/_lib.py
--- a/bfc_amd/_lib.py
+++ b/bfc_amd/_lib.py
@@ -111,6 +111,7 @@
     "bfcg_stats": (C.c_int, [C.c_void_p, u64p]),
     "bfcg_progress": (C.c_int, [C.c_void_p, u64p, u64p, u64p, C.c_int]),
     "bfcg_partition_info": (C.c_int, [C.c_void_p, u64p]),
+    "bfcg_commit_info": (C.c_int, [C.c_void_p, u64p]),
     "bfcg_s1wc_launches": (C.c_uint64, []),
     "bfcg_table_info": (C.c_int, [C.c_void_p, C.POINTER(C.c_int)]),
     "bfcg_last_batch_ms": (C.c_int, [C.c_void_p, f32p]),
diff --git a/bfc_amd/api.py b/bfc_amd/api.py
--- a/bfc_amd/api.py
+++ b/bfc_amd/api.py
@@ -460,6 +460,17 @@
         out = (C.c_uint64 * 2)()
         self.L.bfcg_partition_info(self.ctx, out)
         return dict(one_pass=bool(out[0] & 1), level2_one_pass=bool(out[0] & 2), replayed_batches=int(out[1]))
+
+    def commit_info(self):
+        out = (C.c_uint64 * 4)()
+        self.L.bfcg_commit_info(self.ctx, out)
+        return dict(halves=int(out[0]), pages_per_half=int(out[1]), beside_bloom=int(out[2]), on_stage_b=int(out[3]))
+
+    def progress(self, n=8):
+        calls, final = C.c_uint64(), C.c_uint64()
+        keys = (C.c_uint64 * n)()
+        self.L.bfcg_progress(self.ctx, C.byref(calls), C.byref(final), keys, n)
+        return int(calls.value), int(final.value), [int(keys[i]) for i in range(min(n, int(final.value)))]
 
     def s1wc_launches(self):
         return int(self.L.bfcg_s1wc_launches())
diff --git a/bfc_amd/csrc/bfcg_bloom3.hip b/bfc_amd/csrc/bfcg_bloom3.hip
--- a/bfc_amd/csrc/bfcg_bloom3.hip
+++ b/bfc_amd/csrc/bfcg_bloom3.hip
@@ -26,7 +26,7 @@
 	unsigned long long *ho_base;
 	if (ho_log) {
 		ho_cur0 = A.ho_cur[f];
-		if (ho_cur0 + n > A.ho_stride) {
+		if (ho_cur0 + n > A.ho_cap) {
 			if (threadIdx.x == 0) { atomicAdd(&A.stats[(size_t)(f & (ST_SLOTS - 1)) * ST_N + ST_ERR_POOL], 1ULL); A.ho_mark[f] = ho_cur0; }
 			return;
 		}
diff --git a/bfc_amd/csrc/bfcg_ctx.hip b/bfc_amd/csrc/bfcg_ctx.hip
--- a/bfc_amd/csrc/bfcg_ctx.hip
+++ b/bfc_amd/csrc/bfcg_ctx.hip
@@ -87,10 +87,18 @@
 	int reused;
 	int seg_no_grow;
 	int seg_cap_shift;
-	unsigned long long *ho, *ho_keys, *h_ho_keys[2]; uint32_t *ho_cur, *ho_mark; uint32_t ho_stride; int ho_K;
+	unsigned long long *ho, *ho_keys, *h_ho_keys[2]; uint32_t *ho_cur, *ho_mark; uint32_t ho_stride, ho_cap; int ho_K, ho_Kh, ho_halves;
+	int ho_half;
 	int ho_pending;
 	uint64_t ho_page_call[HO_MAX_PAGES];
-	int slot_commit[2]; uint64_t slot_page_call[2][HO_MAX_PAGES];
+	int ho_closed; uint64_t ho_closed_call[HO_MAX_PAGES];
+	struct commit_t { int pages, slot, timed; uint64_t call[HO_MAX_PAGES]; } cm[2];
+	int cmq[2], n_cmq;
+	int ho_busy[2];
+	uint64_t n_cm_beside, n_cm_st;
+	int overlap;
+	hipStream_t stK;
+	hipEvent_t evK[2], evKt[2][2];
 	int slot_all_committed[2];
 	uint64_t keys_known;
 	int commit_absorbed;
@@ -344,22 +352,31 @@
 		BFCG_CKN(bfcg_destroy(c), hipMalloc(&B.seg_tab, ((uint64_t)nfine << sh) * 8));
 		{
 			const char *e = getenv("BFCG_COMMIT_K");
-			int K = e ? atoi(e) : 4;
+			int K = e ? atoi(e) : 8;
 			if (K < 1) K = 1;
 			if (K > HO_MAX_PAGES) K = HO_MAX_PAGES;
 			if (!c->cap2) K = 1;
 			size_t free_b = 0, total_b = 0;
 			const uint64_t page = (uint64_t)nfine * (c->cap2 ? c->cap2 : 1) * 8;
 			if (hipMemGetInfo(&free_b, &total_b) == hipSuccess) while (K > 1 && page * (uint64_t)K > (uint64_t)free_b / 3) --K;
+			c->ho_halves = K >= 2 ? 2 : 1; c->ho_Kh = K / c->ho_halves; K = c->ho_Kh * c->ho_halves;
 			c->ho_K = K;
-			c->ho_stride = c->cap2 ? (uint32_t)K * c->cap2 : 0u;
+			c->ho_cap = c->cap2 ? (uint32_t)c->ho_Kh * c->cap2 : 0u;
+			c->ho_stride = c->ho_cap * (uint32_t)c->ho_halves;
 			uint64_t entries = (uint64_t)nfine * c->ho_stride;
 			if (entries < c->recs2_n) entries = c->recs2_n;
 			BFCG_CKN(bfcg_destroy(c), hipMalloc(&c->ho, (entries + 4096) * 8));
-			BFCG_CKN(bfcg_destroy(c), hipMalloc(&c->ho_cur, sizeof(uint32_t) * (size_t)nfine));
-			BFCG_CKN(bfcg_destroy(c), hipMalloc(&c->ho_mark, sizeof(uint32_t) * (size_t)nfine * HO_MAX_PAGES));
-			BFCG_CKN(bfcg_destroy(c), hipMalloc(&c->ho_keys, sizeof(unsigned long long) * ST_SLOTS * HO_MAX_PAGES));
-			for (int b = 0; b < 2; ++b) BFCG_CKN(bfcg_destroy(c), hipHostMalloc(&c->h_ho_keys[b], sizeof(unsigned long long) * ST_SLOTS * HO_MAX_PAGES));
+			BFCG_CKN(bfcg_destroy(c), hipMalloc(&c->ho_cur, sizeof(uint32_t) * (size_t)nfine * 2));
+			BFCG_CKN(bfcg_destroy(c), hipMalloc(&c->ho_mark, sizeof(uint32_t) * (size_t)nfine * HO_MAX_PAGES * 2));
+			BFCG_CKN(bfcg_destroy(c), hipMalloc(&c->ho_keys, sizeof(unsigned long long) * ST_SLOTS * HO_MAX_PAGES * 2));
+			for (int h = 0; h < 2; ++h) BFCG_CKN(bfcg_destroy(c), hipHostMalloc(&c->h_ho_keys[h], sizeof(unsigned long long) * ST_SLOTS * HO_MAX_PAGES));
+			BFCG_CKN(bfcg_destroy(c), hipStreamCreate(&c->stK));
+			for (int h = 0; h < 2; ++h) {
+				BFCG_CKN(bfcg_destroy(c), hipEventCreateWithFlags(&c->evK[h], hipEventDisableTiming));
+				for (int i = 0; i < 2; ++i) BFCG_CKN(bfcg_destroy(c), hipEventCreate(&c->evKt[h][i]));
+			}
+			const char *eo = getenv("BFCG_COMMIT_OVERLAP");
+			c->overlap = c->ho_halves == 2 && n_ranks == 1 && !prm->debug_seen && !getenv("BFCG_SYNC_BATCHES") && eo && atoi(eo) != 0;
 		}
 	}
 	if (P.filter_mode) BFCG_CKN(bfcg_destroy(c), hipMalloc(&B.bloom_hi, c->bloom_bytes));
@@ -409,7 +426,8 @@
 	for (void *h : {(void *)c->h_stats, (void *)c->h_snap[0], (void *)c->h_snap[1]}) if (h) (void)hipHostFree(h); (void)hipFree(c->d_seg); if (c->h_seg) (void)hipHostFree(c->h_seg);
 	for (int b = 0; b < 2; ++b) for (hipEvent_t e : {c->evt[b][0], c->evt[b][1], c->evt[b][2], c->evt[b][3], c->evt[b][4], c->evt[b][5], c->evt[b][6], c->evA[b], c->evB[b]}) if (e) (void)hipEventDestroy(e);
 	if (c->evCopy) (void)hipEventDestroy(c->evCopy);
-	for (hipStream_t st : {c->st, c->stA, c->stC}) if (st) (void)hipStreamDestroy(st);
+	for (int h = 0; h < 2; ++h) for (hipEvent_t e : {c->evK[h], c->evKt[h][0], c->evKt[h][1]}) if (e) (void)hipEventDestroy(e);
+	for (hipStream_t st : {c->st, c->stA, c->stC, c->stK}) if (st) (void)hipStreamDestroy(st);
 	free(c);
 }
 
@@ -425,10 +443,11 @@
 static int enqueue_batch(bfcg_ctx_t *c, const uint8_t *d_seq, const uint8_t *d_qual, uint64_t n_pos, int wait_copy, int no_kstats);
 static int ensure_agg(bfcg_ctx_t *c);
 static int same_block_offset(bfcg_ctx_t *c, int b, const uint8_t *d_seq, const uint8_t **d_qual, uint64_t n_pos, hipStream_t s);
-static int commit_pending_pages(bfcg_ctx_t *c, int b);
-static void absorb_pages(bfcg_ctx_t *c, int b);
-static int handover_begin(bfcg_ctx_t *c, BatchBufs &Bt, int b, int slabs, uint64_t call);
-static int handover_end(bfcg_ctx_t *c, const BatchBufs &Bt, int b);
+static int flush_log(bfcg_ctx_t *c, int b);
+static int absorb_slot(bfcg_ctx_t *c, int b);
+static int absorb_all(bfcg_ctx_t *c);
+static int handover_begin(bfcg_ctx_t *c, BatchBufs &Bt, int b, int slabs, uint64_t call, int overlap);
+static int handover_end(bfcg_ctx_t *c, const BatchBufs &Bt, int b, int overlap);
 
 static void warm_tables(const bfcg_ctx_t *c, KParams &Pt)
 {
@@ -470,8 +489,10 @@
 		}
 		if (c->n_batches) c->reused = 1;
 		c->P.seg = 1; c->P.b3 = c->b3_ok; c->seg_escaped = 0;
-		BFCG_CK(hipMemsetAsync(c->ho_cur, 0, sizeof(uint32_t) * (size_t)nf, c->st));
-		c->ho_pending = 0; c->slot_commit[0] = c->slot_commit[1] = 0; c->slot_all_committed[0] = c->slot_all_committed[1] = 0; c->keys_known = 0; c->commit_absorbed = 0;
+		for (int h = 0; h < 2; ++h) if (c->ho_busy[h]) { BFCG_CK(hipStreamWaitEvent(c->st, c->evK[h], 0)); c->ho_busy[h] = 0; }
+		BFCG_CK(hipMemsetAsync(c->ho_cur, 0, sizeof(uint32_t) * (size_t)nf * 2, c->st));
+		c->ho_pending = 0; c->ho_half = 0; c->ho_closed = 0; c->n_cmq = 0; c->cm[0].pages = c->cm[1].pages = 0;
+		c->slot_all_committed[0] = c->slot_all_committed[1] = 0; c->keys_known = 0; c->commit_absorbed = 0;
 		c->keys_per_batch = 0; c->n_commits = 0; c->ho_window = 1;
 		BFCG_CK(hipMemsetAsync(c->B.seg_tab, 0, (nf << c->P.seg_shift) * 8, c->st));
 	}
@@ -503,16 +524,17 @@
 	fold_slots(c, raw);
 	return 0;
 }
-static void fold_snapshot(bfcg_ctx_t *c, int b)
+static int fold_snapshot(bfcg_ctx_t *c, int b)
 {
 	fold_slots(c, c->h_snap[b]);
-	absorb_pages(c, b);
+	if (absorb_slot(c, b) != 0) return -1;
 	if (c->slot_all_committed[b]) {
 		c->final_call = c->slot_call[b]; c->call_keys[c->slot_call[b] & 63] = c->h_stats[ST_KEYS];
 		if (c->h_stats[ST_KEYS] > c->keys_known && c->h_stats[ST_KEYS] - c->keys_known > c->keys_per_batch) c->keys_per_batch = c->h_stats[ST_KEYS] - c->keys_known;
 		c->keys_known = c->h_stats[ST_KEYS]; c->commit_absorbed = 1;
 	}
 	c->pos_final += c->slot_pos[b]; c->slot_pos[b] = 0;
+	return 0;
 }
 
 static int table_maintain(bfcg_ctx_t *c);
@@ -545,28 +567,31 @@
 	if (!c->pend) return 0;
 	BFCG_CK(hipStreamSynchronize(c->stA));
 	BFCG_CK(hipStreamSynchronize(c->st));
+	if (c->stK) BFCG_CK(hipStreamSynchronize(c->stK));
 	BFCG_CK(hipGetLastError());
 	c->pend = 0;
 	if (batch_times(c, c->cur ^ 1) != 0) return -1;
-	absorb_pages(c, c->cur); absorb_pages(c, c->cur ^ 1);
+	if (absorb_all(c) != 0) return -1;
 	if (c->n_opq) {
 		uint32_t sticky = 0;
 		BFCG_CK(hipMemcpy(&sticky, c->op_flags + OP_STICKY, sizeof(sticky), hipMemcpyDeviceToHost));
 		if (sticky) return replay_poisoned(c);
 		c->n_opq = 0;
 	}
-	if (c->P.seg && c->ho_pending) {
-		if (commit_pending_pages(c, 0) != 0) return -1;
+	if (c->P.seg && (c->ho_pending || c->ho_closed)) {
+		if (flush_log(c, 0) != 0) return -1;
 		BFCG_CK(hipStreamSynchronize(c->st));
 		BFCG_CK(hipGetLastError());
-		absorb_pages(c, 0);
+		if (absorb_all(c) != 0) return -1;
 	}
 	if (fetch_stats(c) != 0) return -1;
 	c->keys_known = c->h_stats[ST_KEYS]; c->commit_absorbed = 1;
 	c->final_call = c->call_no; c->call_keys[c->call_no & 63] = c->h_stats[ST_KEYS];
 	c->pos_final += c->slot_pos[0] + c->slot_pos[1]; c->slot_pos[0] = c->slot_pos[1] = 0;
 	note_growth(c);
-	return check_health(c);
+	if (check_health(c) != 0) return -1;
+	c->keys_known = c->h_stats[ST_KEYS]; c->call_keys[c->call_no & 63] = c->h_stats[ST_KEYS];
+	return 0;
 }
 
 extern "C" int bfcg_sync(bfcg_ctx_t *c) { return drain(c); }
@@ -680,7 +705,10 @@
 {
 	const KParams &P = c->P;
 	const uint64_t nf = nfine(c);
-	const uint64_t need = c->h_stats[ST_KEYS] + c->h_stats[ST_TAB_OVF], g = c->ho_K > 1 ? c->keys_per_batch : c->grow[0] > c->grow[1] ? c->grow[0] : c->grow[1];
+	uint64_t ahead = (uint64_t)c->ho_closed;
+	for (int i = 0; i < c->n_cmq; ++i) if (c->cm[c->cmq[i]].timed) ahead += (uint64_t)c->cm[c->cmq[i]].pages;
+	const uint64_t keys = c->h_stats[ST_KEYS] > c->keys_known || !c->ho_stride ? c->h_stats[ST_KEYS] : c->keys_known;
+	const uint64_t need = keys + c->h_stats[ST_TAB_OVF], g = c->ho_K > 1 ? c->keys_per_batch * (ahead > 1 ? ahead : 1) : c->grow[0] > c->grow[1] ? c->grow[0] : c->grow[1];
 	int t = P.seg_shift;
 	const double full = c->seg_no_grow ? 0.85 : 0.62;
 	while ((double)(need + (c->seg_no_grow ? 0 : g)) > full * (double)(nf << t)) ++t;
@@ -776,6 +804,12 @@
 extern "C" int bfcg_partition_info(bfcg_ctx_t *c, uint64_t out[2]) { out[0] = (uint64_t)((c->onepass ? 1 : 0) | ((c->onepass || (c->mg_op2 && c->mg_op2_allowed)) && c->cap2 ? 2 : 0)); out[1] = c->n_replayed; return 0; }
 extern "C" void bfcg_mg_allow_onepass(bfcg_ctx_t *c, int on) { c->mg_op2_allowed = on != 0; }
 
+extern "C" int bfcg_commit_info(bfcg_ctx_t *c, uint64_t out[4])
+{
+	out[0] = c->ho_stride ? (uint64_t)c->ho_halves : 0; out[1] = c->ho_stride ? (uint64_t)c->ho_Kh : 0; out[2] = c->n_cm_beside; out[3] = c->n_cm_st;
+	return 0;
+}
+
 extern "C" int bfcg_table_info(bfcg_ctx_t *c, int out[4])
 {
 	out[0] = c->P.seg; out[1] = c->P.seg ? c->P.seg_shift : 0; out[2] = c->P.seg ? 0 : c->P.tab_cshift; out[3] = (int)c->n_seg_grow;
@@ -814,6 +848,7 @@
 	const uint8_t *seq, *qual;
 	const void *recv; const uint32_t *sizes; int sizes_slab;
 	int finalise;
+	int overlap;
 };
 
 static int opq_push(bfcg_ctx_t *c, int b, const StageB &w)
@@ -832,9 +867,9 @@
 
 static int enqueue_stage_b(bfcg_ctx_t *c, int b, BatchBufs &Bt, const KParams &Pt, const StageB &w)
 {
-	if (handover_begin(c, Bt, b, w.slabs, w.call) != 0) return -1;
+	if (handover_begin(c, Bt, b, w.slabs, w.call, w.overlap) != 0) return -1;
 	run_stage_b(Pt, Bt, w.in1, w.seg_beg, w.seg_end, w.n_seg, w.segs_per_bucket, w.row_base, w.bucket_start, w.rec_bound, c->st, c->evt[b]);
-	if (handover_end(c, Bt, b) != 0) return -1;
+	if (handover_end(c, Bt, b, w.overlap) != 0) return -1;
 	if (w.queued) {
 		BFCG_CK(hipMemcpyAsync(c->h_flags[b] + 1, c->op_flags + OP_STICKY, sizeof(uint32_t), hipMemcpyDeviceToHost, c->st));
 		if (opq_push(c, b, w) != 0) return -1;
@@ -1069,7 +1104,7 @@
 			for (int i = 1; i < c->n_opq; ++i) c->opq[i - 1] = c->opq[i];
 			--c->n_opq;
 		}
-		fold_snapshot(c, pb);
+		if (fold_snapshot(c, pb) != 0) return -1;
 		note_growth(c);
 		if (c->h_stats[ST_ERR_POOL] || c->h_stats[ST_TAB_OVF] || (c->P.seg ? seg_target_shift(c) != c->P.seg_shift : (c->B.table && table_target_cshift(c) != c->P.tab_cshift))) {
 			c->pend = 1; c->cur = b ^ 1;
@@ -1081,76 +1116,161 @@
 }
 
 
-static int commit_pending_pages(bfcg_ctx_t *c, int b)
-{
-	if (!c->ho_pending) return 0;
-	const uint32_t nf = (uint32_t)nfine(c);
-	BatchBufs Bt = c->B;
-	Bt.ho = c->ho; Bt.ho_stride = c->ho_stride; Bt.ho_cur = c->ho_cur; Bt.ho_mark = c->ho_mark; Bt.ho_mark_stride = nf; Bt.ho_keys = c->ho_keys;
-	BFCG_CK(hipMemsetAsync(c->ho_keys, 0, sizeof(unsigned long long) * ST_SLOTS * (size_t)c->ho_pending, c->st));
-	run_commit_pages(c->P, Bt, nf, (uint32_t)c->ho_pending, c->st);
-	BFCG_CK(hipMemcpyAsync(c->h_ho_keys[b], c->ho_keys, sizeof(unsigned long long) * ST_SLOTS * (size_t)c->ho_pending, hipMemcpyDeviceToHost, c->st));
-	c->slot_commit[b] = c->ho_pending;
-	memcpy(c->slot_page_call[b], c->ho_page_call, sizeof(uint64_t) * (size_t)c->ho_pending);
-	c->ho_pending = 0;
-	return 0;
-}
-static int handover_begin(bfcg_ctx_t *c, BatchBufs &Bt, int b, int slabs, uint64_t call)
-{
-	c->slot_commit[b] = 0; c->slot_all_committed[b] = 1;
-	if (!c->P.seg) return 0;
-	const uint32_t nf = (uint32_t)nfine(c);
-	Bt.stream_out = (uint32_t *)c->ho;
-	Bt.ho = c->ho; Bt.ho_cur = c->ho_cur; Bt.ho_mark = c->ho_mark; Bt.ho_mark_stride = nf; Bt.ho_keys = c->ho_keys;
-	if (!slabs || c->ho_stride == 0 || Bt.seen_out) {
-		if (commit_pending_pages(c, b) != 0) return -1;
-		Bt.ho_stride = 0; Bt.ho_page = 0; Bt.ho_commit = 1; Bt.ho_keys = nullptr;
-		return 0;
-	}
-	if (c->ho_pending == 0) {
-		int w = 1;
-		if (c->ho_K > 1 && c->n_commits > 0) {
-			const double room = 0.85 * (double)((uint64_t)nf << c->P.seg_shift) - (double)c->keys_known, g = 1.1 * (double)(c->keys_per_batch ? c->keys_per_batch : 1);
-			w = room <= g ? 1 : room / g >= (double)c->ho_K ? c->ho_K : (int)(room / g);
-		}
-		c->ho_window = w;
-		if (getenv("BFCG_DEBUG")) fprintf(stderr, "[D::window] %d batches: keys %llu, largest page of the last commit %llu, slots %llu, commits so far %d\n", w,
-			(unsigned long long)c->keys_known, (unsigned long long)c->keys_per_batch, (unsigned long long)((uint64_t)nf << c->P.seg_shift), c->n_commits);
-	}
-	Bt.ho_stride = c->ho_stride; Bt.ho_page = (uint32_t)c->ho_pending;
-	c->ho_page_call[c->ho_pending++] = call;
-	Bt.ho_commit = c->ho_pending >= c->ho_window;
-	if (Bt.ho_commit) BFCG_CK(hipMemsetAsync(c->ho_keys, 0, sizeof(unsigned long long) * ST_SLOTS * (size_t)c->ho_pending, c->st));
-	else c->slot_all_committed[b] = 0;
-	return 0;
-}
-static int handover_end(bfcg_ctx_t *c, const BatchBufs &Bt, int b)
-{
-	if (!c->P.seg || Bt.ho_stride == 0 || !Bt.ho_commit) return 0;
-	BFCG_CK(hipMemcpyAsync(c->h_ho_keys[b], c->ho_keys, sizeof(unsigned long long) * ST_SLOTS * (size_t)c->ho_pending, hipMemcpyDeviceToHost, c->st));
-	c->slot_commit[b] = c->ho_pending;
-	memcpy(c->slot_page_call[b], c->ho_page_call, sizeof(uint64_t) * (size_t)c->ho_pending);
-	c->ho_pending = 0;
-	return 0;
-}
-static void absorb_pages(bfcg_ctx_t *c, int b)
-{
-	const int J = c->slot_commit[b];
-	if (!J) return;
+static void half_bufs(const bfcg_ctx_t *c, BatchBufs &Bt, int h)
+{
+	const size_t nf = (size_t)nfine(c);
+	Bt.ho = c->ho + (size_t)h * c->ho_cap; Bt.ho_stride = c->ho_stride; Bt.ho_cap = c->ho_cap;
+	Bt.ho_cur = c->ho_cur + (size_t)h * nf; Bt.ho_mark = c->ho_mark + (size_t)h * HO_MAX_PAGES * nf; Bt.ho_mark_stride = (uint32_t)nf;
+	Bt.ho_keys = c->ho_keys + (size_t)h * HO_MAX_PAGES * ST_SLOTS;
+}
+static int st_wait_half(bfcg_ctx_t *c, int h)
+{
+	if (c->ho_busy[h]) { BFCG_CK(hipStreamWaitEvent(c->st, c->evK[h], 0)); c->ho_busy[h] = 0; }
+	return 0;
+}
+static int st_wait_commits(bfcg_ctx_t *c) { return st_wait_half(c, 0) != 0 || st_wait_half(c, 1) != 0 ? -1 : 0; }
+static int absorb_commit(bfcg_ctx_t *c, int h)
+{
+	bfcg_ctx::commit_t &m = c->cm[h];
 	uint64_t run = c->keys_known, most = 0;
-	for (int j = 0; j < J; ++j) {
-		const unsigned long long *row = c->h_ho_keys[b] + (size_t)j * ST_SLOTS;
+	for (int j = 0; j < m.pages; ++j) {
+		const unsigned long long *row = c->h_ho_keys[h] + (size_t)j * ST_SLOTS;
 		uint64_t d = 0;
 		for (int i = 0; i < ST_SLOTS; ++i) d += row[i];
 		run += d;
 		if (d > most) most = d;
-		c->call_keys[c->slot_page_call[b][j] & 63] = run;
+		c->call_keys[m.call[j] & 63] = run;
 	}
 	c->keys_per_batch = most; ++c->n_commits;
-	c->final_call = c->slot_page_call[b][J - 1];
+	c->final_call = m.call[m.pages - 1];
 	c->keys_known = run;
-	c->slot_commit[b] = 0;
 	c->commit_absorbed = 1;
+	if (m.timed) {
+		float ms = 0;
+		BFCG_CK(hipEventElapsedTime(&ms, c->evKt[h][0], c->evKt[h][1]));
+		c->last_ms[4] = ms; c->sum_ms[4] += ms; c->sum_ms[5] += ms;
+	}
+	m.pages = 0;
+	return 0;
+}
+static int absorb_front(bfcg_ctx_t *c)
+{
+	const int h = c->cmq[0];
+	BFCG_CK(hipEventSynchronize(c->evK[h]));
+	c->cmq[0] = c->cmq[1]; --c->n_cmq;
+	return absorb_commit(c, h);
+}
+static int absorb_slot(bfcg_ctx_t *c, int b)
+{
+	for (;;) {
+		int last = -1;
+		for (int i = 0; i < c->n_cmq; ++i) if (c->cm[c->cmq[i]].slot == b) last = i;
+		if (last < 0) return 0;
+		if (absorb_front(c) != 0) return -1;
+	}
+}
+static int absorb_all(bfcg_ctx_t *c)
+{
+	while (c->n_cmq) if (absorb_front(c) != 0) return -1;
+	return 0;
+}
+static int enqueue_commit(bfcg_ctx_t *c, int h, int pages, const uint64_t *calls, int b, hipStream_t s)
+{
+	while (c->cm[h].pages) if (absorb_front(c) != 0) return -1;
+	const uint32_t nf = (uint32_t)nfine(c);
+	BatchBufs Bt = c->B;
+	half_bufs(c, Bt, h);
+	const int own = s == c->stK;
+	BFCG_CK(hipMemsetAsync(Bt.ho_keys, 0, sizeof(unsigned long long) * ST_SLOTS * (size_t)pages, s));
+	if (own) BFCG_CK(hipEventRecord(c->evKt[h][0], s));
+	run_commit_pages(c->P, Bt, nf, (uint32_t)pages, s);
+	if (own) BFCG_CK(hipEventRecord(c->evKt[h][1], s));
+	BFCG_CK(hipMemcpyAsync(c->h_ho_keys[h], Bt.ho_keys, sizeof(unsigned long long) * ST_SLOTS * (size_t)pages, hipMemcpyDeviceToHost, s));
+	BFCG_CK(hipEventRecord(c->evK[h], s));
+	c->ho_busy[h] = own;
+	++(own ? c->n_cm_beside : c->n_cm_st);
+	c->cm[h].pages = pages; c->cm[h].slot = b; c->cm[h].timed = own;
+	memcpy(c->cm[h].call, calls, sizeof(uint64_t) * (size_t)pages);
+	c->cmq[c->n_cmq++] = h;
+	return 0;
+}
+static int flush_log(bfcg_ctx_t *c, int b)
+{
+	if (st_wait_commits(c) != 0) return -1;
+	if (c->ho_closed) {
+		if (enqueue_commit(c, c->ho_half ^ 1, c->ho_closed, c->ho_closed_call, b, c->st) != 0) return -1;
+		c->ho_closed = 0;
+	}
+	if (c->ho_pending) {
+		if (enqueue_commit(c, c->ho_half, c->ho_pending, c->ho_page_call, b, c->st) != 0) return -1;
+		c->ho_pending = 0;
+	}
+	return 0;
+}
+static int handover_begin(bfcg_ctx_t *c, BatchBufs &Bt, int b, int slabs, uint64_t call, int overlap)
+{
+	c->slot_all_committed[b] = 1;
+	if (!c->P.seg) return 0;
+	const uint32_t nf = (uint32_t)nfine(c);
+	Bt.stream_out = (uint32_t *)c->ho;
+	if (!slabs || c->ho_stride == 0 || Bt.seen_out) {
+		if (flush_log(c, b) != 0) return -1;
+		half_bufs(c, Bt, 0);
+		Bt.ho_stride = 0; Bt.ho_page = 0; Bt.ho_commit = 1; Bt.ho_keys = nullptr;
+		return 0;
+	}
+	if (c->ho_closed && !overlap) {
+		if (st_wait_commits(c) != 0 || enqueue_commit(c, c->ho_half ^ 1, c->ho_closed, c->ho_closed_call, b, c->st) != 0) return -1;
+		c->ho_closed = 0;
+	}
+	if (c->ho_pending == 0) {
+		int w = 1;
+		if (c->ho_K > 1 && c->n_commits > 0) {
+			int ahead = c->ho_closed;
+			for (int i = 0; i < c->n_cmq; ++i) if (c->cm[c->cmq[i]].timed) ahead += c->cm[c->cmq[i]].pages;
+			const double g = 1.1 * (double)(c->keys_per_batch ? c->keys_per_batch : 1), room = 0.85 * (double)((uint64_t)nf << c->P.seg_shift) - (double)c->keys_known - (double)ahead * g;
+			w = room <= g ? 1 : room / g >= (double)c->ho_Kh ? c->ho_Kh : (int)(room / g);
+		}
+		c->ho_window = w;
+		if (getenv("BFCG_DEBUG")) fprintf(stderr, "[D::window] %d batches into half %d: keys %llu, largest page of the last commit %llu, slots %llu, commits so far %d\n", w, c->ho_half,
+			(unsigned long long)c->keys_known, (unsigned long long)c->keys_per_batch, (unsigned long long)((uint64_t)nf << c->P.seg_shift), c->n_commits);
+		if (st_wait_half(c, c->ho_half) != 0) return -1;
+	}
+	half_bufs(c, Bt, c->ho_half);
+	Bt.ho_page = (uint32_t)c->ho_pending;
+	c->ho_page_call[c->ho_pending++] = call;
+	const int closes = c->ho_pending >= c->ho_window;
+	Bt.ho_commit = closes && !overlap;
+	if (Bt.ho_commit) {
+		if (st_wait_commits(c) != 0) return -1;
+		while (c->cm[c->ho_half].pages) if (absorb_front(c) != 0) return -1;
+		BFCG_CK(hipMemsetAsync(Bt.ho_keys, 0, sizeof(unsigned long long) * ST_SLOTS * (size_t)c->ho_pending, c->st));
+	} else c->slot_all_committed[b] = 0;
+	return 0;
+}
+static int handover_end(bfcg_ctx_t *c, const BatchBufs &Bt, int b, int overlap)
+{
+	if (!c->P.seg || Bt.ho_stride == 0) return 0;
+	const int h = c->ho_half;
+	if (c->ho_closed) {
+		BFCG_CK(hipStreamWaitEvent(c->stK, c->evt[b][3], 0));
+		if (enqueue_commit(c, h ^ 1, c->ho_closed, c->ho_closed_call, b, c->stK) != 0) return -1;
+		c->ho_closed = 0;
+	}
+	if (Bt.ho_commit) {
+		BFCG_CK(hipMemcpyAsync(c->h_ho_keys[h], Bt.ho_keys, sizeof(unsigned long long) * ST_SLOTS * (size_t)c->ho_pending, hipMemcpyDeviceToHost, c->st));
+		BFCG_CK(hipEventRecord(c->evK[h], c->st));
+		c->cm[h].pages = c->ho_pending; c->cm[h].slot = b; c->cm[h].timed = 0;
+		memcpy(c->cm[h].call, c->ho_page_call, sizeof(uint64_t) * (size_t)c->ho_pending);
+		c->cmq[c->n_cmq++] = h; ++c->n_cm_st;
+		c->ho_pending = 0;
+		if (c->ho_halves == 2) c->ho_half ^= 1;
+	} else if (overlap && c->ho_pending >= c->ho_window) {
+		c->ho_closed = c->ho_pending;
+		memcpy(c->ho_closed_call, c->ho_page_call, sizeof(uint64_t) * (size_t)c->ho_pending);
+		c->ho_pending = 0; c->ho_half ^= 1;
+	}
+	return 0;
 }
 
 static int same_block_offset(bfcg_ctx_t *c, int b, const uint8_t *d_seq, const uint8_t **d_qual, uint64_t n_pos, hipStream_t s)
@@ -1199,7 +1319,7 @@
 		const uint32_t *sg = c->op_seg[b];
 		w.seg_beg = sg; w.seg_end = sg + 8 * nb1; w.row_base = sg + 16 * nb1; w.bucket_start = sg + 24 * nb1 + 1; w.rec_bound = (uint64_t)8 * nb1 * c->op_cap;
 	} else { w.seg_beg = Bt.start1; w.seg_end = Bt.start1 + 1; w.row_base = Bt.row_base; w.bucket_start = Bt.start1; w.rec_bound = n_pos; }
-	w.slabs = op && Bt.cap2; w.queued = op_run; w.call = c->call_no; w.pos = n_pos; w.finalise = 1;
+	w.slabs = op && Bt.cap2; w.queued = op_run; w.call = c->call_no; w.pos = n_pos; w.finalise = 1; w.overlap = c->overlap;
 	return enqueue_stage_b(c, b, Bt, Pt, w);
 }
 
diff --git a/bfc_amd/csrc/bfcg_dev.h b/bfc_amd/csrc/bfcg_dev.h
--- a/bfc_amd/csrc/bfcg_dev.h
+++ b/bfc_amd/csrc/bfcg_dev.h
@@ -80,7 +80,7 @@
 	TabOrder ord;
 	unsigned long long batch_hi;
 	const uint32_t *cnt2; uint32_t cap2;
-	unsigned long long *ho; uint32_t ho_stride; uint32_t *ho_cur; uint32_t *ho_mark;
+	unsigned long long *ho; uint32_t ho_stride, ho_cap; uint32_t *ho_cur; uint32_t *ho_mark;
 	uint32_t ho_pages, ho_mark_stride;
 	unsigned long long *ho_keys;
 	const uint32_t *flags;
diff --git a/bfc_amd/csrc/bfcg_internal.h b/bfc_amd/csrc/bfcg_internal.h
--- a/bfc_amd/csrc/bfcg_internal.h
+++ b/bfc_amd/csrc/bfcg_internal.h
@@ -94,7 +94,7 @@
 	uint32_t op_own_lo, op_own_n, op_own_delta;
 	uint32_t *cnt2; uint32_t cap2;
 	uint32_t *cnt_live;
-	unsigned long long *ho; uint32_t ho_stride; uint32_t *ho_cur, *ho_mark; uint32_t ho_mark_stride, ho_page; int ho_commit; unsigned long long *ho_keys;
+	unsigned long long *ho; uint32_t ho_stride, ho_cap; uint32_t *ho_cur, *ho_mark; uint32_t ho_mark_stride, ho_page; int ho_commit; unsigned long long *ho_keys;
 	unsigned long long *seg_tab;
 	unsigned long long *tab_first, *sub_last;
 	unsigned long long batch_hi;
diff --git a/bfc_amd/csrc/bfcg_kernels.hip b/bfc_amd/csrc/bfcg_kernels.hip
--- a/bfc_amd/csrc/bfcg_kernels.hip
+++ b/bfc_amd/csrc/bfcg_kernels.hip
@@ -835,7 +835,7 @@
 	if (SEGOUT) {
 		if (ho_log) {
 			ho_cur0 = A.ho_cur[f];
-			if (ho_cur0 + n > A.ho_stride) {
+			if (ho_cur0 + n > A.ho_cap) {
 				if (threadIdx.x == 0) { atomicAdd(&A.stats[(size_t)(f & (ST_SLOTS - 1)) * ST_N + ST_ERR_POOL], 1ULL); A.ho_mark[f] = ho_cur0; }
 				return;
 			}
@@ -1977,7 +1977,7 @@
 	BloomArgs A;
 	memset(&A, 0, sizeof(A));
 	A.stats = B.stats; A.tab_ovf = B.tab_ovf; A.tab_ovf_cap = B.tab_ovf_cap; A.ovf_cnt = B.stats + (size_t)ST_SLOTS * ST_N; A.seg_tab = B.seg_tab; A.n_fine = n_fine;
-	A.ho = B.ho; A.ho_stride = B.ho_stride; A.ho_cur = B.ho_cur; A.ho_mark = B.ho_mark; A.ho_mark_stride = B.ho_mark_stride; A.ho_pages = pages; A.ho_keys = B.ho_keys;
+	A.ho = B.ho; A.ho_stride = B.ho_stride; A.ho_cap = B.ho_cap; A.ho_cur = B.ho_cur; A.ho_mark = B.ho_mark; A.ho_mark_stride = B.ho_mark_stride; A.ho_pages = pages; A.ho_keys = B.ho_keys;
 	launch_commit_seg(P, A, (int)n_fine, st);
 }
 
@@ -2021,7 +2021,7 @@
 		else launch_bloom<W, RW>(!h4 ? BV_FM_ANYH : P.bloom_bt == 1024 ? BV_FM_1024 : BV_FM, P, A, nfine, st);
 	} else if (P.seg && B.seg_tab && (B.stream_out || B.ho)) {
 		A.stream_out = B.stream_out; A.seg_tab = B.seg_tab; A.table = nullptr; A.agg_out = nullptr;
-		A.ho = B.ho; A.ho_stride = B.ho_stride; A.ho_cur = B.ho_cur; A.ho_mark = B.ho_stride ? B.ho_mark + (size_t)B.ho_page * B.ho_mark_stride : nullptr;
+		A.ho = B.ho; A.ho_stride = B.ho_stride; A.ho_cap = B.ho_cap; A.ho_cur = B.ho_cur; A.ho_mark = B.ho_stride ? B.ho_mark + (size_t)B.ho_page * B.ho_mark_stride : nullptr;
 		if (RW == 3 && P.b3 && (P.b3_cold || !P.dedupe)) run_bloom3(P, A, nfine, (size_t)bloom_lds_bytes(P), st);
 		else launch_bloom<W, RW>(!h4 ? BV_SEG_ANYH : RW == 3 && bloom_fast3(P) ? BV_SEG_F3 : BV_SEG, P, A, nfine, st);
 	} else if (B.stream && B.stream_out && !P.track && h4) {
diff --git a/include/bfc_gpu.h b/include/bfc_gpu.h
--- a/include/bfc_gpu.h
+++ b/include/bfc_gpu.h
@@ -124,6 +124,7 @@
 int bfcg_progress(bfcg_ctx_t *c, uint64_t *calls, uint64_t *final, uint64_t *keys_of, int n);
 int bfcg_table_info(bfcg_ctx_t *c, int out[4]);
 int bfcg_partition_info(bfcg_ctx_t *c, uint64_t out[2]);
+int bfcg_commit_info(bfcg_ctx_t *c, uint64_t out[4]);
 uint64_t bfcg_s1wc_launches(void);
 uint64_t bfcg_stream_batches(bfcg_ctx_t *c);
 
```

Result: slower. 40970 (-2.2%).
